# keunwoochoi/torchaudio-contrib

Hardware: AMD Instinct MI355X
Metric: mel frames/sec (higher is better)
Workload: dtype f32; 1 GPU; Melspectrogram+AmplitudeToDb batch=256/GPU x 1ch x 16000Hz x 10s, fft_len=2048 hop=512 128 mel (BASELINE configs[1]); global_batch=256, parallelism=batch-sharded x1, no data-path collective

## Files before the change

include/tac_amd.h:

```cpp
#ifndef TAC_AMD_H
#define TAC_AMD_H

#include <stdint.h>

#ifdef __cplusplus
extern "C" {
#endif

#define TAC_OK 0
#define TAC_E_INVALID (-1)
#define TAC_E_UNSUPPORTED (-2)
#define TAC_E_SHORT_INPUT (-3)
#define TAC_E_LAUNCH (-4)

#define TAC_PAD_CONSTANT 0
#define TAC_PAD_REFLECT 1
#define TAC_PAD_REPLICATE 2
#define TAC_PAD_CIRCULAR 3

const char* tac_strerror(int code);
int tac_last_hip_error(void);
int tac_abi_version(void);

int64_t tac_num_frames(int64_t L, int n_fft, int hop, int center);
int tac_num_bins(int n_fft, int onesided);

typedef struct tac_stft_desc {
    int64_t rows;
    int64_t length;
    int64_t row_stride;
    int32_t n_fft;
    int32_t hop;
    int32_t win_length;
    int32_t center;
    int32_t pad_mode;
    int32_t normalized;
    int32_t onesided;
    int32_t reserved;
} tac_stft_desc;

int tac_stft_f32(const float* wave, const float* window, const tac_stft_desc* d,
                 float* out, void* stream);

int tac_spectrogram_f32(const float* wave, const float* window, const tac_stft_desc* d,
                        float power, int db, float db_ref, float db_amin,
                        float* out, void* stream);

int tac_melspec_f32(const float* wave, const float* window, const tac_stft_desc* d, float power,
                    const float* fb, const int32_t* fb_plan_host, int32_t n_mels,
                    int db, float db_ref, float db_amin, float* out, void* stream);

#define TAC_PACK_PAIRS_2048 (-2048)
int tac_melbank_pack(const float* fb, int32_t n_freqs, int32_t n_mels, int32_t n_fft, float* wpack,
                     int32_t wpack_cap, int32_t* desc, int32_t desc_cap, int32_t* info_host, void* stream);
int tac_melbank_pack_host(const float* fb_host, int32_t n_freqs, int32_t n_mels, int32_t n_fft, float* wpack_host,
                          int32_t wpack_cap, int32_t* desc_host, int32_t desc_cap, int32_t* info_host);
int tac_melbank_plan_pieces_host(const float* fb_host, int32_t n_freqs, int32_t n_mels, int32_t* seg_steps, int32_t* first,
                                 int32_t* band, int32_t* index, float* weights, int32_t weights_cap);
int tac_melspec_sparse_f32(const float* wave, const float* window, const tac_stft_desc* d, float power,
                           const float* wpack, const int32_t* desc, const int32_t* info_host, int32_t n_mels,
                           int db, float db_ref, float db_amin, float* out, void* stream);

#define TAC_SAMPLES_F32 0
#define TAC_SAMPLES_I16 1
#define TAC_SAMPLES_MULAW_U8 2
#define TAC_SAMPLES_MULAW_I64 3
int tac_melspec_sparse_coded_f32(const void* samples, int32_t sample_format, const float* decode_lut,
                                 const float* window, const tac_stft_desc* d, float power, const float* wpack,
                                 const int32_t* desc, const int32_t* info_host, int32_t n_mels, int db,
                                 float db_ref, float db_amin, float* out, void* stream);
int tac_pcm16_to_f32(const int16_t* x, int64_t n, float* out, void* stream);

int tac_melspec_supported(const tac_stft_desc* d, float power, const int32_t* fb_plan_host,
                          int32_t n_mels);

int tac_filterbank_plan(const float* fb, int32_t n_freqs, int32_t n_mels, int32_t* plan,
                        int32_t* plan_host, void* stream);

int tac_apply_filterbank_f32(const float* spec, int64_t rows, int32_t n_freqs, int64_t n_frames,
                             int64_t stride_r, int64_t stride_f, int64_t stride_t,
                             const float* fb, const int32_t* fb_plan, int32_t n_mels,
                             float* out, void* stream);

int tac_apply_filterbank_sparse_f32(const float* spec, int64_t rows, int32_t n_freqs, int64_t n_frames,
                                    int64_t stride_r, int64_t stride_t, const float* wpack,
                                    const int32_t* desc, const int32_t* info_host, int32_t n_mels,
                                    float* out, void* stream);
int tac_apply_filterbank_sparse_db_f32(const float* spec, int64_t rows, int32_t n_freqs, int64_t n_frames,
                                       int64_t stride_r, int64_t stride_t, const float* wpack, const int32_t* desc,
                                       const int32_t* info_host, int32_t n_mels, int db, float db_ref, float db_amin,
                                       float* out, void* stream);

int tac_complex_norm_f32(const float* x, int64_t n, float power, float* out, void* stream);

int tac_magphase_f32(const float* x, int64_t n, float power, float* mag, float* phase, void* stream);

int tac_phase_vocoder_f32(const float* spec, int64_t rows, int32_t n_freqs, int64_t n_frames,
                          int64_t stride_r, int64_t stride_f, int64_t stride_t,
                          const float* phase_advance, const int32_t* idx0, const int32_t* idx1,
                          const float* alpha, int64_t n_out, float* out, void* stream);
int tac_phase_vocoder_f64(const double* spec, int64_t rows, int32_t n_freqs, int64_t n_frames,
                          int64_t stride_r, int64_t stride_f, int64_t stride_t,
                          const double* phase_advance, const int32_t* idx0, const int32_t* idx1,
                          const double* alpha, int64_t n_out, double* out, void* stream);
int tac_phase_vocoder_backward_f32(const float* spec, int64_t rows, int32_t n_freqs, int64_t n_frames, int64_t stride_r,
                                   int64_t stride_f, int64_t stride_t, const int32_t* idx0, const int32_t* idx1, const float* alpha,
                                   int64_t n_out, const float* grad_out, float* grad_spec, void* stream);

int tac_stretch_norm_f32(const float* mag, int64_t rows, int32_t n_freqs, int64_t n_frames, int64_t stride_r, int64_t stride_t,
                         const int32_t* idx0, const float* alpha, int64_t n_out, float power, int db, float db_ref, float db_amin,
                         float* out, int32_t* flags, void* stream);
int tac_stretch_mel_f32(const float* mag, int64_t rows, int32_t n_freqs, int64_t n_frames, int64_t stride_r, int64_t stride_t,
                        const int32_t* idx0, const float* alpha, int64_t n_out, float power, const float* wpack, const int32_t* desc,
                        const int32_t* info_host, int32_t n_mels, int db, float db_ref, float db_amin, float* out, int32_t* flags,
                        void* stream);
int tac_stretch_norm_backward_f32(const float* mag, int64_t rows, int32_t n_freqs, int64_t n_frames, int64_t stride_r,
                                  int64_t stride_t, const int32_t* idx0, const float* alpha, const int32_t* bounds, int64_t n_out,
                                  float power, const float* grad_out, float* grad_mag, void* stream);

int tac_stft_f64(const double* wave, const double* window, const tac_stft_desc* d, double* out, void* stream);
int tac_spectrogram_f64(const double* wave, const double* window, const tac_stft_desc* d, double power, int db,
                        double db_ref, double db_amin, double* out, void* stream);
int tac_apply_filterbank_f64(const double* spec, int64_t rows, int32_t n_freqs, int64_t n_frames, int64_t stride_r,
                             int64_t stride_f, int64_t stride_t, const double* fb, int32_t n_mels, int db,
                             double db_ref, double db_amin, double* out, void* stream);
int tac_magphase_f64(const double* z, int64_t n, double power, double* mag, double* phase, void* stream);
int tac_amplitude_to_db_f64(const double* x, int64_t n, double ref, double amin, double* out, void* stream);
int tac_db_to_amplitude_f64(const double* x, int64_t n, double ref, double* out, void* stream);

int tac_amplitude_to_db_f32(const float* x, int64_t n, float ref, float amin, float* out,
                            void* stream);

int tac_db_to_amplitude_f32(const float* x, int64_t n, float ref, float* out, void* stream);

int tac_mulaw_encode_f32_i64(const float* x, int64_t n, int32_t n_quantize,
                             const int32_t* thresholds, int32_t n_pos, int32_t n_neg,
                             int32_t zero_code, int64_t* out, void* stream);

int tac_mulaw_decode_i64_f32(const int64_t* codes, int64_t n, int32_t n_quantize,
                             const float* lut, float* out, void* stream);

int tac_mulaw_decode_f32_f32(const float* codes, int64_t n, int32_t n_quantize, const float* lut,
                             float* out, void* stream);
int tac_mulaw_encode_f64_i64(const double* x, int64_t n, int32_t n_quantize, int64_t* out, void* stream);
int tac_mulaw_decode_f64(const void* codes, int32_t codes_are_i64, int64_t n, int32_t n_quantize, double* out, void* stream);

int tac_stft_backward_f32(const float* grad_spec, const float* window, const tac_stft_desc* d,
                          float* grad_frames, void* stream);
int tac_stft_norm_backward_f32(const float* spec, const float* grad_norm, float power, const float* window,
                               const tac_stft_desc* d, float* grad_frames, void* stream);
int tac_spectrogram_backward_f32(const float* wave, const float* window, const tac_stft_desc* d,
                                 const float* grad_norm, float power, float* grad_frames, void* stream);
int64_t tac_spectrogram_backward_ola_workspace(const tac_stft_desc* d);
int tac_spectrogram_backward_ola_f32(const float* wave, const float* window, const tac_stft_desc* d,
                                     const float* grad_norm, float power, void* workspace, int64_t workspace_bytes,
                                     float* grad_wave, int64_t grad_row_stride, void* stream);
int tac_melspectrogram_backward_ola_f32(const float* wave, const float* window, const tac_stft_desc* d,
                                        const float* grad_mel, int32_t n_mels, const void* adjoint_table,
                                        int32_t n_freqs, float power, void* workspace, int64_t workspace_bytes,
                                        float* grad_wave, int64_t grad_row_stride, void* stream);
int tac_melspectrogram_backward_f32(const float* wave, const float* window, const tac_stft_desc* d,
                                    const float* grad_mel, int32_t n_mels, const void* adjoint_table, int32_t n_freqs,
                                    float power, float* grad_frames, void* stream);
int tac_filterbank_adjoint_pack(const float* fb, int32_t n_freqs, int32_t n_mels, void* table,
                                int32_t* max_nonzeros_host, void* stream);
int tac_apply_filterbank_adjoint_f32(const float* grad_mel, int64_t rows_times_frames, int32_t n_mels,
                                     const void* table, int32_t n_freqs, float* grad_spec, void* stream);
int tac_overlap_add_f32(const float* grad_frames, const tac_stft_desc* d, float* grad_wave,
                        int64_t grad_row_stride, void* stream);
int tac_complex_norm_backward_f32(const float* z, const float* grad_out, int64_t n, float power,
                                  float* grad_z, void* stream);
int tac_fold_twosided_f32(const float* grad, int64_t n_frames_total, int32_t n_fft, int32_t width, float* out,
                          void* stream);
int64_t tac_window_grad_partials(const tac_stft_desc* d);
int tac_window_grad_f32(const float* grad_frames_unwindowed, const float* wave, const tac_stft_desc* d,
                        float* partial, int64_t n_partials, void* stream);
int tac_sum_slabs_f32(const float* x, int64_t n_slabs, int64_t slab_elems, float* out, void* stream);
int tac_amplitude_to_db_backward_f32(const float* x, const float* grad_out, int64_t n, float amin,
                                     float* grad_x, void* stream);
int tac_magphase_backward_f32(const float* z, const float* grad_mag, const float* grad_phase, int64_t n, float power,
                              float* grad_z, void* stream);
int tac_db_to_amplitude_backward_f32(const float* x, const float* grad_out, int64_t n, float ref, float* grad_x, void* stream);

int tac_hpss_f32(const float* mag, int64_t rows, int32_t n_freqs, int32_t n_frames, int64_t stride_r,
                 int64_t stride_f, int64_t stride_t, int32_t kernel_f, int32_t kernel_t, float power,
                 int hard, float* harm, float* perc, float* mask_harm, float* mask_perc, void* stream);
int tac_hpss_backward_f32(const float* mag, int64_t rows, int32_t n_freqs, int32_t n_frames, int64_t stride_r, int64_t stride_f,
                          int64_t stride_t, int32_t kernel_f, int32_t kernel_t, float power, int hard, const float* grad_harm,
                          const float* grad_perc, const float* grad_mask_harm, const float* grad_mask_perc, float* grad_mag,
                          void* stream);

const char* tac_last_route(void);
int tac_debug_clock_probe(uint64_t* buf, int32_t capacity_pairs);

int tac_set_fft_pipe(int mode);

int64_t tac_istft_workspace(const tac_stft_desc* d, int64_t n_frames);
int tac_istft_envelope_f32(const float* window, const tac_stft_desc* d, int64_t n_frames, float* inv_env, float* env,
                           void* stream);
int tac_istft_f32(const float* spec, int64_t stride_r, int64_t stride_t, int64_t n_frames, const float* window,
                  const float* inv_env, const tac_stft_desc* d, void* workspace, int64_t workspace_bytes, float* out,
                  void* stream);
int tac_istft_grad_input_f32(const float* grad_out, int64_t grad_stride, const float* inv_env, const tac_stft_desc* d,
                             int64_t n_frames, float* padded, void* stream);
int tac_istft_grad_bins_f32(float* spec, int64_t n_frames_total, int n_fft, int normalized, void* stream);

int tac_dct_rows_f32(const float* x, int64_t rows, int32_t n_in, int64_t n_frames,
                     int64_t stride_r, int64_t stride_m, int64_t stride_t,
                     const float* mat, int32_t n_out, float* out, void* stream);

int tac_polyphase_f32(const float* x, int64_t rows, int64_t l_in, int64_t stride_r, const float* bank, const int32_t* table,
                      int32_t phases, int32_t taps, int32_t taps_min, int32_t step, int32_t off_min, int32_t off_max,
                      int64_t l_out, float* out, void* stream);

int32_t tac_lfilter_chunk(void);
int tac_lfilter_supported(const double* b, const double* a, int32_t n_coeffs);
int tac_lfilter_f32(const float* x, int64_t rows, int64_t length, int64_t stride_r, const double* b, const double* a,
                    int32_t n_coeffs, int clamp, int reverse, float* out, void* stream);

int32_t tac_spectral_mac_tile(int32_t n_parts);
int tac_spectral_mac_f32(const float* X, const float* H, const int32_t* hrow, int64_t rows, int64_t n_frames, int32_t n_bins,
                         int32_t n_parts, int32_t h_rows, int conj, float* Y, void* stream);
int32_t tac_fftconvolve_default_n_fft(int64_t m);
int tac_fftconvolve_supported(int64_t l_in, int64_t m, int32_t n_fft);
int64_t tac_fftconvolve_spectra_workspace(int64_t h_rows, int64_t m, int32_t n_fft);
int tac_fftconvolve_spectra_f32(const float* y, int64_t h_rows, int64_t m, int64_t stride_r, int32_t n_fft, int reverse,
                                void* workspace, int64_t workspace_bytes, float* H, void* stream);
int64_t tac_fftconvolve_workspace(int64_t rows, int64_t l_in, int64_t m, int32_t n_fft, int64_t offset, int64_t l_out);
int tac_fftconvolve_f32(const float* x, int64_t rows, int64_t l_in, int64_t stride_r, const float* H, const int32_t* hrow,
                        int32_t h_rows, int64_t m, int32_t n_fft, int conj, int64_t offset, int64_t l_out, void* workspace,
                        int64_t workspace_bytes, float* out, int64_t out_stride, void* stream);
int tac_fftconvolve_direct_f32(const float* x, int64_t rows, int64_t l_in, int64_t stride_r, const float* bank, const int32_t* table,
                               int64_t m, int64_t offset, int64_t l_out, float* out, void* stream);

#define TAC_KALDI_SNIP_EDGES 1
#define TAC_KALDI_REMOVE_DC 2
#define TAC_KALDI_RAW_ENERGY 4
#define TAC_KALDI_USE_ENERGY 8
#define TAC_KALDI_HTK 16
#define TAC_KALDI_LOG 32
#define TAC_KALDI_POWER 64
int64_t tac_kaldi_num_frames(int64_t length, int32_t win_length, int32_t shift, int snip_edges);
int tac_kaldi_fbank_f32(const float* x, int64_t rows, int64_t length, int64_t stride_r, const float* window, const float* weights,
                        const int32_t* table, int32_t n_fft, int32_t win_length, int32_t shift, int32_t n_mels, int32_t w_total,
                        int32_t flags, float preemph, float energy_floor, float* out, void* stream);

int64_t tac_kaldi_mfcc_table_limit(int32_t n_fft, int32_t n_mels, int32_t w_total);
int tac_kaldi_mfcc_f32(const float* x, int64_t rows, int64_t length, int64_t stride_r, const float* window, const float* weights,
                       const int32_t* table, const float* dct, int32_t n_fft, int32_t win_length, int32_t shift, int32_t n_mels,
                       int32_t w_total, int32_t n_ceps, int32_t flags, float preemph, float energy_floor, float* out, void* stream);
int tac_kaldi_spectrogram_f32(const float* x, int64_t rows, int64_t length, int64_t stride_r, const float* window, int32_t n_fft,
                              int32_t win_length, int32_t shift, int32_t flags, float preemph, float energy_floor, float* out,
                              void* stream);

int64_t tac_sliding_cmn_chunk(int64_t rows, int64_t n_frames, int64_t n_feats, int64_t cmn_window, int64_t min_cmn_window);
int tac_sliding_cmn_f32(const float* x, int64_t rows, int64_t n_frames, int64_t n_feats, int64_t stride_r, int64_t stride_t,
                        int64_t stride_f, int64_t cmn_window, int64_t min_cmn_window, int center, int norm_vars, int adjoint,
                        float* out, void* stream);

#define TAC_DELTAS_REPLICATE 0
#define TAC_DELTAS_CONSTANT 1
#define TAC_DELTAS_REFLECT 2
#define TAC_DELTAS_CIRCULAR 3
int tac_deltas_supported(int64_t n_frames, int32_t win_length, int32_t mode, int adjoint);
int tac_deltas_f32(const float* x, int64_t rows, int64_t n_feats, int64_t n_frames, int64_t stride_r, int64_t stride_f,
                   int64_t stride_t, int32_t win_length, int32_t mode, int adjoint, float* out, void* stream);

#ifdef __cplusplus
}
#endif
#endif
```

torchaudio-contrib_amd/_hip.py:

```python
import ctypes
import itertools
import math
import os
import threading
import weakref

import torch

from . import _kaldi
from . import _native
from . import _resample

_lock = threading.Lock()

launches = {}


def _count(name, *filled):
    launches[name] = launches.get(name, 0) + 1
    check_written(name, *filled)


_epoch = 0
_CACHE_ATTRS = ('_tac_pack', '_tac_plan', '_tac_T', '_tac_adj', '_tac_dft', '_tac_dftT', '_tac_finite', '_tac_istft', '_tac_dct', '_tac_coef', '_tac_conv')
# ... 154 lines not shown
    return g


def _rows_of(wave, g):
    return wave.reshape(-1, g.length).contiguous() if g.flatten else wave


def _dft_matrix(window, n_fft, win_length, onesided, normalized):
    cache = getattr(window, '_tac_dft', None)
    key = (_stamp(window), n_fft, win_length, bool(onesided), bool(normalized))
    if cache is not None and cache[0] == key:
        return cache[1]
    dev = window.device
    w = torch.zeros(n_fft, dtype=torch.float64, device=dev)
    off = (n_fft - win_length) // 2
    w[off:off + win_length] = window.detach().double()
    if normalized:
        w = w / math.sqrt(n_fft)
    n_bins = n_fft // 2 + 1 if onesided else n_fft
    n = torch.arange(n_fft, dtype=torch.int64, device=dev)[:, None]
    k = torch.arange(n_bins, dtype=torch.int64, device=dev)[None, :]
    ang = ((n * k) % n_fft).double() * (2.0 * math.pi / n_fft)
    mat = torch.stack([torch.cos(ang) * w[:, None], -torch.sin(ang) * w[:, None]], dim=-1)
    mat = mat.to(torch.float32).reshape(n_fft, 2 * n_bins).contiguous()
    try:
        window._tac_dft = (key, mat)
    except Exception:
        pass
    return mat


def _stft_dft(wave, window, g):
    x = wave.reshape(-1, g.length)
    if g.center:
        pad = g.n_fft // 2
        x = torch.nn.functional.pad(x.unsqueeze(1), (pad, pad), mode=g.pad_mode).squeeze(1)
    x = x.contiguous()
    mat = _dft_matrix(window, g.n_fft, g.win_length, g.onesided, g.normalized)
    out = _empty(g.stft_shape, device=x.device)
    with _native.on_device(x.device):
        rc = _native.lib().tac_apply_filterbank_f32(
            _native.ptr(x), x.shape[0], g.n_fft, g.n_frames, x.stride(0), 1, g.hop,
            _native.ptr(mat), None, 2 * g.n_bins, _native.ptr(out), _native.stream_ptr(x.device))
    _native.check(rc, 'tac_apply_filterbank_f32 (DFT matrix)')
    _count('tac_apply_filterbank_f32', out)
    return out.transpose(-3, -2)


def stft(wave, window, n_fft, hop, win_length, center, pad_mode, normalized, onesided):
    g = geometry(wave, n_fft, hop, win_length, center, pad_mode, normalized, onesided)
    if not (g.fft_kernel or (g.mixed_radix and g.onesided)):
        return _stft_dft(wave, window, g)
    src = _rows_of(wave, g)
    out = _empty(g.stft_shape, device=wave.device)
    with _native.on_device(wave.device):
        rc = _native.lib().tac_stft_f32(_native.ptr(src), _native.ptr(window), g.desc, _native.ptr(out),
                                        _native.stream_ptr(wave.device))
    _native.check(rc, 'tac_stft_f32')
    _count('tac_stft_f32', out)
    return out.transpose(-3, -2)


def spectrogram(wave, window, n_fft, hop, win_length, center, pad_mode, normalized, onesided, power, db, ref, amin):
    g = geometry(wave, n_fft, hop, win_length, center, pad_mode, normalized, onesided)
    if not (g.fft_kernel or (g.mixed_radix and g.onesided and power in (1.0, 2.0))):
        mag = complex_norm(_stft_dft(wave, window, g), power)
        return amplitude_to_db(mag, ref, amin) if db else mag
    src = _rows_of(wave, g)
    out = _empty(g.spec_shape, device=wave.device)
    with _native.on_device(wave.device):
        rc = _native.lib().tac_spectrogram_f32(
            _native.ptr(src), _native.ptr(window), g.desc, float(power), 1 if db else 0, float(ref), float(amin),
            _native.ptr(out), _native.stream_ptr(wave.device))
    _native.check(rc, 'tac_spectrogram_f32')
    _count('tac_spectrogram_f32', out)
    return out.transpose(-2, -1)


istft_layout = {'in_place': 0, 'copied': 0}


def istft_covers(n_fft):
    return bool(fft_kernel_size(n_fft) or mixed_radix_size(n_fft) or smooth_fft_size(n_fft) or n_fft == 8192)


def istft_full_length(n_frames, n_fft, hop, center):
    return hop * (n_frames - 1) + n_fft - (2 * (n_fft // 2) if center else 0)


def _istft_desc(rows, out_len, row_stride, n_fft, hop, win_length, center, normalized):
    return _native.StftDesc(rows=rows, length=out_len, row_stride=row_stride, n_fft=n_fft, hop=hop, win_length=win_length,
                            center=1 if center else 0, pad_mode=0, normalized=1 if normalized else 0, onesided=1, reserved=0)


def istft_envelope(window, n_fft, hop, win_length, center, n_frames, kept):
    cache = getattr(window, '_tac_istft', None)
    stamp = _stamp(window)
    if cache is None or cache[0] != stamp:
        cache = (stamp, {})
        try:
            window._tac_istft = cache
        except Exception:
            pass
    key = (n_fft, hop, win_length, bool(center), n_frames)
    entry = cache[1].get(key)
    if entry is None:
        n_pos = hop * (n_frames - 1) + n_fft
        with torch.inference_mode(False):
            inv_env = torch.empty(n_pos, dtype=torch.float32, device=window.device)
        desc = _istft_desc(1, 1, 1, n_fft, hop, win_length, center, False)
        with _native.on_device(window.device):
            rc = _native.lib().tac_istft_envelope_f32(_native.ptr(window), desc, n_frames, _native.ptr(inv_env),
                                                      None, _native.stream_ptr(window.device))
        _native.check(rc, 'tac_istft_envelope_f32')
        launches['tac_istft_envelope_f32'] = launches.get('tac_istft_envelope_f32', 0) + 1
        if len(cache[1]) > 64:
            cache[1].clear()
        entry = cache[1][key] = (inv_env, set())
    if kept not in entry[1]:
        pad = n_fft // 2 if center else 0
        peak = float(entry[0][pad:pad + kept].max().item())
        lowest = 1.0 / peak if peak > 0.0 else float('inf')
        if not lowest >= 1e-11:
            raise RuntimeError('istft: window overlap add min: %g is below 1e-11 (fft_length=%d, hop_length=%d, center=%s): '
                               'the window does not satisfy the NOLA condition' % (lowest, n_fft, hop, bool(center)))
        entry[1].add(kept)
    return entry[0]


def _istft_rows(spec):
    sp = spec.transpose(-3, -2)
    if sp.is_contiguous() and sp.data_ptr() % 16 == 0:
        istft_layout['in_place'] += 1
    else:
        istft_layout['copied'] += 1
        sp = sp.contiguous()
    return sp.reshape((-1,) + tuple(sp.shape[-3:]))


def istft(spec, window, n_fft, hop, win_length, center, normalized, length, route=None):
    n_frames = int(spec.shape[-2])
    full = istft_full_length(n_frames, n_fft, hop, center)
    if full <= 0:
        raise RuntimeError('istft: %d frame(s) of fft_length %d leave no samples after removing the centre padding'
                           % (n_frames, n_fft))
    out_len = full if length is None else int(length)
    inv_env = istft_envelope(window, n_fft, hop, win_length, center, n_frames, min(full + (n_fft // 2 if center else 0), out_len))
    lead = tuple(int(s) for s in spec.shape[:-3])
    rows = _istft_rows(spec)
    n_rows = int(rows.shape[0])
    out = _empty(lead + (out_len,), device=spec.device)
    desc = _istft_desc(n_rows, out_len, out_len, n_fft, hop, win_length, center, normalized)
    need = int(_native.lib().tac_istft_workspace(desc, n_frames))
    if need < 0:
        _native.check(need, 'tac_istft_workspace')

    def launch(work, nbytes):
        with _native.on_device(spec.device):
            return _native.lib().tac_istft_f32(_native.ptr(rows), rows.stride(0), rows.stride(1), n_frames, _native.ptr(window),
                                               _native.ptr(inv_env), desc, None if work is None else _native.ptr(work), nbytes,
                                               _native.ptr(out), _native.stream_ptr(spec.device))

    rc = _native.TAC_E_UNSUPPORTED
    if need == 0 and route != 'general':
        rc = launch(None, 0)
    if rc == _native.TAC_E_UNSUPPORTED:
        need = n_rows * n_frames * n_fft * 4
        work = torch.empty(need // 4, dtype=torch.float32, device=spec.device)
        rc = launch(work, need)
    _native.check(rc, 'tac_istft_f32')
    _count('tac_istft_f32', out)
    return out


def istft_backward(grad_out, window, n_fft, hop, win_length, center, normalized, n_frames):
    out_len = int(grad_out.shape[-1])
    full = istft_full_length(n_frames, n_fft, hop, center)
    inv_env = istft_envelope(window, n_fft, hop, win_length, center, n_frames, min(full + (n_fft // 2 if center else 0), out_len))
    lead = tuple(int(s) for s in grad_out.shape[:-1])
    go = grad_out.reshape(-1, out_len)
    go = go if go.is_contiguous() else go.contiguous()
    n_rows, n_pos, n_bins = int(go.shape[0]), hop * (n_frames - 1) + n_fft, n_fft // 2 + 1
    padded = _empty((n_rows, n_pos), device=go.device)
    gspec = _empty(lead + (n_frames, n_bins, 2), device=go.device)
    with _native.on_device(go.device):
        stream = _native.stream_ptr(go.device)
        rc = _native.lib().tac_istft_grad_input_f32(
            _native.ptr(go), out_len, _native.ptr(inv_env),
            _istft_desc(n_rows, out_len, out_len, n_fft, hop, win_length, center, normalized), n_frames, _native.ptr(padded), stream)
        _native.check(rc, 'tac_istft_grad_input_f32')
        _count('tac_istft_grad_input_f32', padded)
        fwd = _native.StftDesc(rows=n_rows, length=n_pos, row_stride=n_pos, n_fft=n_fft, hop=hop, win_length=win_length, center=0,
                               pad_mode=0, normalized=0, onesided=1, reserved=0)
        rc = _native.lib().tac_stft_f32(_native.ptr(padded), _native.ptr(window), fwd, _native.ptr(gspec), stream)
        _native.check(rc, 'tac_stft_f32')
        _count('tac_stft_f32', gspec)
        rc = _native.lib().tac_istft_grad_bins_f32(_native.ptr(gspec), n_rows * n_frames, n_fft, 1 if normalized else 0, stream)
        _native.check(rc, 'tac_istft_grad_bins_f32')
        _count('tac_istft_grad_bins_f32', gspec)
    return gspec.transpose(-3, -2)


POISON_OUTPUTS = False

POISON_BITS = {torch.float32: 0x7FC0DEAD, torch.float64: 0x7FF80000DEADBEEF, torch.int64: -0x21524111DEADBEEF,
               torch.int32: -0x21524111}
_BIT_VIEW = {torch.float32: torch.int32, torch.float64: torch.int64, torch.int64: torch.int64, torch.int32: torch.int32}
_poison_hits = {}


def set_poison_outputs(on):
    global POISON_OUTPUTS
    POISON_OUTPUTS = bool(on)
    ext = _native.ext()
    if ext is not None:
        ext.set_poison(POISON_OUTPUTS)


def poison_fill(t):
    if t.numel():
        t.view(_BIT_VIEW[t.dtype]).fill_(POISON_BITS[t.dtype])
    return t


def poison_count(t):
    if not t.numel():
        return torch.zeros((), dtype=torch.int64, device=t.device)
    return (t.view(_BIT_VIEW[t.dtype]) == POISON_BITS[t.dtype]).sum()


def _poisoning(t):
    return POISON_OUTPUTS and not (t.is_cuda and torch.cuda.is_current_stream_capturing())


def _empty(shape, dtype=torch.float32, device=None):
    out = torch.empty(shape, dtype=dtype, device=device)
    return poison_fill(out) if _poisoning(out) else out


def _empty_strided(shape, stride, dtype=torch.float32, device=None):
    out = torch.empty_strided(shape, stride, dtype=dtype, device=device)
    return poison_fill(out) if _poisoning(out) else out


def _empty_like(x):
    out = torch.empty_like(x)
    return poison_fill(out) if _poisoning(out) else out


def check_written(name, *parts):
    if not POISON_OUTPUTS:
        return
    for t in parts:
        if t is None or not t.numel() or not _poisoning(t):
            continue
        key = (name, t.device.index)
        acc = _poison_hits.get(key)
        if acc is None:
            with torch.inference_mode(False):
                acc = _poison_hits[key] = torch.zeros((), dtype=torch.int64, device=t.device)
        acc += poison_count(t)


def poison_report(reset=True):
    bad = {}
    for (name, _), acc in list(_poison_hits.items()):
        n = int(acc.item())
        if n:
            bad[name] = bad.get(name, 0) + n
    if reset:
        _poison_hits.clear()
    return bad

MEL_PATH = os.environ.get('TAC_MEL_PATH', 'auto')


def _melbank_pack(fb, n_fft):
    cache = getattr(fb, '_tac_pack', None)
    if cache is None or cache[0] != _stamp(fb):
        cache = (_stamp(fb), {})
        try:
            fb._tac_pack = cache
        except Exception:
            pass
    if n_fft in cache[1]:
        return cache[1][n_fft]
    n_freqs, n_mels = fb.shape
    wpack = torch.empty(24576, dtype=torch.float32, device=fb.device)
    desc = torch.empty(8192, dtype=torch.int32, device=fb.device)
    info = (ctypes.c_int32 * 8)()
    with _native.on_device(fb.device):
        rc = _native.lib().tac_melbank_pack(_native.ptr(fb), n_freqs, n_mels, n_fft, _native.ptr(wpack), 24576,
                                            _native.ptr(desc), 8192, ctypes.cast(info, ctypes.c_void_p),
                                            _native.stream_ptr(fb.device))
    if rc == _native.TAC_E_UNSUPPORTED:
        result = None
    else:
        _native.check(rc, 'tac_melbank_pack')
        result = (wpack, desc, info)
    cache[1][n_fft] = result
    return result


PAIR_LAYOUT = True
PACK_PAIRS_2048 = -2048


def _fused_pack(fb, n_fft):
    if PAIR_LAYOUT and n_fft == 2048 and tuple(fb.shape) == (1025, 128):
        pack = _melbank_pack(fb, PACK_PAIRS_2048)
        if pack is not None:
            return pack
    return _melbank_pack(fb, n_fft)


def _filterbank_plan(fb):
    hit = getattr(fb, '_tac_plan', None)
    if hit is not None and hit[0] == _stamp(fb) and hit[1].device == fb.device:
        return hit[1], hit[2]
    n_freqs, n_mels = fb.shape
    n_ints = 2 * ((n_mels + 15) // 16)
    plan = torch.empty(n_ints, dtype=torch.int32, device=fb.device)
    host = (ctypes.c_int32 * n_ints)()
    with _native.on_device(fb.device):
        rc = _native.lib().tac_filterbank_plan(_native.ptr(fb), n_freqs, n_mels, _native.ptr(plan),
                                               ctypes.cast(host, ctypes.c_void_p), _native.stream_ptr(fb.device))
    _native.check(rc, 'tac_filterbank_plan')
    try:
        fb._tac_plan = (_stamp(fb), plan, host)
    except Exception:
        pass
    return plan, host


def _fused_mel_route(g, fb, power):
    if not ((g.pow2_kernel or g.mixed_radix) and g.onesided and g.n_fft <= 4096 and fb.dim() == 2 and
            fb.shape[0] == g.n_bins and 0 < fb.shape[1] <= 512 and fb.is_contiguous()):
        return None
    if g.mixed_radix:
        ok = power in (1.0, 2.0) and MEL_PATH != 'mfma' and _melbank_pack(fb, g.n_fft) is not None
        return 'sparse' if ok else None
    if power in (1.0, 2.0) and MEL_PATH != 'mfma' and _melbank_pack(fb, g.n_fft) is not None:
        return 'sparse'
    if MEL_PATH == 'sparse' or g.n_fft > 2048:
        return None
    _, host = _filterbank_plan(fb)
    rc = _native.lib().tac_melspec_supported(g.desc, float(power), ctypes.cast(host, ctypes.c_void_p), fb.shape[1])
    return 'mfma' if rc == _native.TAC_OK else None


class MelPlan(object):
    __slots__ = ('fn', 'win_ptr', 'desc', 'power', 'wpack', 'dsc', 'info', 'wpack_ptr', 'dsc_ptr', 'info_ptr', 'n_mels',
                 'db', 'ref', 'amin', 'shape', 'device', 'dev_index', 'window', 'fb', 'win_stamp', 'fb_stamp', 'layout', 'cplan',
                 'last_rc')

    def run(self, wave):
        c = self.cplan
        if c is not None:
            v = c.launch(wave)
            if v is not None:
                launches['tac_melspec_sparse_f32'] = launches.get('tac_melspec_sparse_f32', 0) + 1
                if POISON_OUTPUTS:
                    check_written('tac_melspec_sparse_f32', v)
            else:
                self.last_rc = c.last_rc
            return v
        return self.launch(wave) if self.matches(wave) else None

    def launch(self, wave):
        out = _empty(self.shape, device=self.device)
        rc = self.fn(wave.data_ptr(), self.win_ptr, self.desc, self.power, self.wpack_ptr, self.dsc_ptr, self.info_ptr,
                     self.n_mels, self.db, self.ref, self.amin, out.data_ptr(),
                     torch._C._cuda_getCurrentRawStream(self.dev_index))
        if rc != _native.TAC_OK:
            self.last_rc = rc
            return None
        launches['tac_melspec_sparse_f32'] = launches.get('tac_melspec_sparse_f32', 0) + 1
        if POISON_OUTPUTS:
            check_written('tac_melspec_sparse_f32', out)
        return out.transpose(-2, -1)

    def matches(self, wave):
        return (wave.shape, wave.stride(), wave.dtype) == self.layout and torch._C._cuda_getDevice() == self.dev_index \
            and _stamp(self.window) == self.win_stamp and _stamp(self.fb) == self.fb_stamp


def mel_plan(wave, window, fb, n_fft, hop, win_length, center, pad_mode, normalized, onesided, power, db, ref, amin):
    if not (type(wave) is torch.Tensor and wave.dtype == torch.float32 and window.dtype == torch.float32
            and window.is_contiguous() and fb.dtype == torch.float32 and fb.dim() == 2 and wave.is_cuda
            and window.device == wave.device and fb.device == wave.device and not window.is_inference()
            and not fb.is_inference()):
        return None
    g = geometry(wave, n_fft, hop, win_length, center, pad_mode, normalized, onesided)
    if g.flatten or g.desc is None or fb.shape[0] != g.n_bins or _fused_mel_route(g, fb, power) != 'sparse':
        return None
    wpack, dsc, info = _fused_pack(fb, g.n_fft)
    p = MelPlan()
    p.fn = _native.lib().tac_melspec_sparse_f32
    p.window, p.fb, p.win_stamp, p.fb_stamp = window, fb, _stamp(window), _stamp(fb)
    p.win_ptr, p.desc, p.power = window.data_ptr(), g.desc, float(power)
    p.wpack, p.dsc, p.info = wpack, dsc, info
    p.wpack_ptr, p.dsc_ptr, p.info_ptr = wpack.data_ptr(), dsc.data_ptr(), ctypes.cast(info, ctypes.c_void_p)
    p.n_mels, p.db, p.ref, p.amin = int(fb.shape[1]), 1 if db else 0, float(ref), float(amin)
    p.shape = g.lead + (g.n_frames, int(fb.shape[1]))
    p.device, p.dev_index = wave.device, wave.device.index
    p.layout = (wave.shape, wave.stride(), wave.dtype)
    p.cplan = None
    p.last_rc = 0
    ext = _native.ext()
    if ext is not None:
        try:
            p.cplan = ext.MelPlan(ctypes.cast(p.fn, ctypes.c_void_p).value, wave, window, fb, wpack, dsc, bytes(g.desc),
                                  [int(v) for v in info], p.power, p.n_mels, bool(db), p.ref, p.amin, [int(n) for n in p.shape],
                                  _epoch)
        except Exception:
            p.cplan = None
    return p


def melspectrogram(wave, window, fb, n_fft, hop, win_length, center, pad_mode, normalized, onesided, power, db, ref,
                   amin):
    g = geometry(wave, n_fft, hop, win_length, center, pad_mode, normalized, onesided)
    if fb.dim() != 2 or fb.shape[0] != g.n_bins:
        raise RuntimeError('apply_filterbank: size mismatch, spectrogram has %d bins, filterbank %s'
                           % (g.n_bins, tuple(fb.shape)))
    rkey = (id(fb), _stamp(fb), power, MEL_PATH)
    hit = g.routes.get(rkey)
    if hit is not None and hit[0]() is fb:
        route = hit[1]
    else:
        if len(g.routes) > 16:
            g.routes.clear()
        route = _fused_mel_route(g, fb, power)
        g.routes[rkey] = (weakref.ref(fb), route)
    if route is None:
        spec = spectrogram(wave, window, n_fft, hop, win_length, center, pad_mode, normalized, onesided, power,
                           False, 1.0, 1e-7)
        return apply_filterbank(spec, fb, db=(ref, amin) if db else None)
    n_mels = fb.shape[1]
    src = _rows_of(wave, g)
    out = _empty(g.lead + (g.n_frames, n_mels), device=wave.device)
    if route == 'sparse':
        wpack, desc, info = _fused_pack(fb, g.n_fft)
        with _native.on_device(wave.device):
            rc = _native.lib().tac_melspec_sparse_f32(
                _native.ptr(src), _native.ptr(window), g.desc, float(power), _native.ptr(wpack), _native.ptr(desc),
                ctypes.cast(info, ctypes.c_void_p), n_mels, 1 if db else 0, float(ref), float(amin),
                _native.ptr(out), _native.stream_ptr(wave.device))
        if rc == _native.TAC_E_UNSUPPORTED:
            spec = spectrogram(wave, window, n_fft, hop, win_length, center, pad_mode, normalized, onesided, power,
                               False, 1.0, 1e-7)
            return apply_filterbank(spec, fb, db=(ref, amin) if db else None)
        _native.check(rc, 'tac_melspec_sparse_f32')
        _count('tac_melspec_sparse_f32', out)
        return out.transpose(-2, -1)
    _, plan_host = _filterbank_plan(fb)
    with _native.on_device(wave.device):
        rc = _native.lib().tac_melspec_f32(
            _native.ptr(src), _native.ptr(window), g.desc, float(power), _native.ptr(fb),
            ctypes.cast(plan_host, ctypes.c_void_p), n_mels, 1 if db else 0, float(ref), float(amin),
            _native.ptr(out), _native.stream_ptr(wave.device))
    _native.check(rc, 'tac_melspec_f32')
    _count('tac_melspec_f32', out)
    return out.transpose(-2, -1)


def apply_filterbank(spec, fb, allow_sparse=True, db=None):
    fb = fb if fb.is_contiguous() else fb.contiguous()
    n_freqs, n_frames = spec.shape[-2], spec.shape[-1]
    lead = tuple(spec.shape[:-2])
    n_mels = fb.shape[1]
    out = _empty(lead + (n_frames, n_mels), device=spec.device)
    if out.numel():
        rows = spec.reshape(-1, n_freqs, n_frames)
        pack = _melbank_pack(fb, 0) if (allow_sparse and rows.stride(1) == 1 and MEL_PATH != 'mfma') else None
        if pack is not None:
            wpack, desc, info = pack
            with _native.on_device(spec.device):
                if db is None:
                    name = 'tac_apply_filterbank_sparse_f32'
                    rc = _native.lib().tac_apply_filterbank_sparse_f32(
                        _native.ptr(rows), rows.shape[0], n_freqs, n_frames, rows.stride(0) if rows.shape[0] > 1 else 0,
                        rows.stride(2), _native.ptr(wpack), _native.ptr(desc), ctypes.cast(info, ctypes.c_void_p), n_mels,
                        _native.ptr(out), _native.stream_ptr(spec.device))
                else:
                    name = 'tac_apply_filterbank_sparse_db_f32'
                    rc = _native.lib().tac_apply_filterbank_sparse_db_f32(
                        _native.ptr(rows), rows.shape[0], n_freqs, n_frames, rows.stride(0) if rows.shape[0] > 1 else 0,
                        rows.stride(2), _native.ptr(wpack), _native.ptr(desc), ctypes.cast(info, ctypes.c_void_p), n_mels,
                        1, float(db[0]), float(db[1]), _native.ptr(out), _native.stream_ptr(spec.device))
            if rc != _native.TAC_E_UNSUPPORTED:
                _native.check(rc, name)
                _count(name, out)
                return out.transpose(-2, -1)
        plan, _ = _filterbank_plan(fb)
        with _native.on_device(spec.device):
            rc = _native.lib().tac_apply_filterbank_f32(
                _native.ptr(rows), rows.shape[0], n_freqs, n_frames, rows.stride(0), rows.stride(1),
                rows.stride(2), _native.ptr(fb), _native.ptr(plan), n_mels, _native.ptr(out),
                _native.stream_ptr(spec.device))
        _native.check(rc, 'tac_apply_filterbank_f32')
        _count('tac_apply_filterbank_f32', out)
    out = out.transpose(-2, -1)
    return out if db is None else amplitude_to_db(out, db[0], db[1])


DCT_MAX_DIM, DCT_MAX_MATRIX = 256, 32768


def dct_covers(n_in, n_out):
    return 1 <= n_in <= DCT_MAX_DIM and 1 <= n_out <= DCT_MAX_DIM and n_in * n_out <= DCT_MAX_MATRIX


def _dct_matrix(mat, transposed):
    if not transposed and mat.dtype == torch.float32 and mat.is_contiguous():
        return mat.detach()
    hit = getattr(mat, '_tac_dct', None)
    if hit is None or hit[0] != _stamp(mat):
        hit = (_stamp(mat), {})
        try:
            mat._tac_dct = hit
        except Exception:
            pass
    m = hit[1].get(transposed)
    if m is None:
        src = mat.detach().t() if transposed else mat.detach()
        m = hit[1][transposed] = src.to(torch.float32).contiguous()
    return m


def dct_rows(x, mat, transposed=False):
    m = _dct_matrix(mat, transposed)
    n_in, n_out = m.shape
    n_frames = x.shape[-1]
    lead = tuple(x.shape[:-2])
    out = _empty(lead + (n_frames, n_out), device=x.device)
    if out.numel():
        rows = x.reshape(-1, n_in, n_frames)
        if any(st <= 0 for st, n in zip(rows.stride(), rows.shape) if n > 1):
            rows = rows.contiguous()
        with _native.on_device(x.device):
            rc = _native.lib().tac_dct_rows_f32(
                _native.ptr(rows), rows.shape[0], n_in, n_frames, rows.stride(0), rows.stride(1), rows.stride(2),
                _native.ptr(m), n_out, _native.ptr(out), _native.stream_ptr(x.device))
        _native.check(rc, 'tac_dct_rows_f32')
        _count('tac_dct_rows_f32', out)
    return out.transpose(-2, -1)


RESAMPLE_MAX_BANK = 20480
RESAMPLE_MAX_PHASES = 2048
RESAMPLE_TILE = 1024
_RS_SPAN_WIDE, _RS_SPAN_MAX = 8192, 14336


def _rs_span_cap(b, tile, off_min, off_max):
    return (3 + ((b.phases - 1 + tile - 1) // b.phases) * b.step + (off_max - off_min) + b.K + 3) & ~3


def resample_tile(b):
    if b.phases > RESAMPLE_MAX_PHASES or b.phases * b.K > RESAMPLE_MAX_BANK:
        return None
    off_min, off_max = min(b.off), max(b.off)
    for tile in (1024, 512, 256):
        if _rs_span_cap(b, tile, off_min, off_max) <= (_RS_SPAN_MAX if tile == 256 else _RS_SPAN_WIDE):
            return tile
    return None


def resample_covers(orig, new, lpw, rolloff, method, beta):
    return resample_tile(_resample.bank(orig, new, lpw, rolloff, method, beta)) is not None and \
        resample_tile(_resample.adjoint_bank(orig, new, lpw, rolloff, method, beta)) is not None


_resample_tables = {}


def _resample_device_bank(key, adjoint, device):
    hit = _resample_tables.get((key, adjoint, device))
    if hit is None:
        b = (_resample.adjoint_bank if adjoint else _resample.bank)(*key)
        taps = b.taps.t().contiguous().to(torch.float32).to(device)
        table = torch.tensor([b.off, b.run], dtype=torch.int32).to(device)
        if len(_resample_tables) > 64:
            _resample_tables.clear()
        hit = _resample_tables[(key, adjoint, device)] = (b, taps, table, min(b.off), max(b.off), min(b.run))
    return hit


def polyphase(x, key, n_out, adjoint=False):
    b, taps, table, off_min, off_max, run_min = _resample_device_bank(key, adjoint, x.device)
    length = x.shape[-1]
    out = _empty(tuple(x.shape[:-1]) + (n_out,), device=x.device)
    if out.numel():
        if length == 0:
            return out.zero_()
        rows = x.reshape(-1, length)
        if (length > 1 and rows.stride(1) != 1) or (rows.shape[0] > 1 and rows.stride(0) <= 0):
            rows = rows.contiguous()
        with _native.on_device(x.device):
            rc = _native.lib().tac_polyphase_f32(
                _native.ptr(rows), rows.shape[0], length, rows.stride(0), _native.ptr(taps), _native.ptr(table), b.phases, b.K,
                run_min, b.step, off_min, off_max, n_out, _native.ptr(out), _native.stream_ptr(x.device))
        _native.check(rc, 'tac_polyphase_f32')
        _count('tac_polyphase_f32', out)
    return out


LFILTER_C = 16
LFILTER_TILE = 1024 * LFILTER_C
LFILTER_MAX_COEFFS = 3

_lfilter_ok = {}
_lfilter_chunk_checked = False

# ... 1187 lines not shown
```

torchaudio-contrib_amd/csrc/lane_placement.hpp:

```cpp
#pragma once
#include <algorithm>
#include <functional>
#include <vector>

namespace tac {

inline std::vector<int> place_band_starts(int nslot, const int* steps, const std::vector<int>& lo, const std::vector<int>& len) {
    std::vector<int> start(lo);
    static const int kGroup[2][16] = {{0, 1, 2, 3, 12, 13, 14, 15, 20, 21, 22, 23, 24, 25, 26, 27},
                                      {4, 5, 6, 7, 8, 9, 10, 11, 16, 17, 18, 19, 28, 29, 30, 31}};
    for (int s = 0; s < nslot; ++s)
        for (int gi = 0; gi < 4; ++gi) {
            int lanes[16];
            for (int i = 0; i < 16; ++i) lanes[i] = kGroup[gi & 1][i] + 32 * (gi >> 1);
            std::vector<int> cand[16];
            for (int i = 0; i < 16; ++i) {
                const int m = s * 64 + lanes[i];
                const int slack = std::max(0, std::min(steps[s] - (len[m] + 3) / 4, lo[m] / 4));
                for (int d = 0; d <= slack; ++d) cand[i].push_back(lo[m] - 4 * d);
            }
            for (int cap = 1; cap <= 16; ++cap) {
                std::vector<int> load[16];
                int choice[16];
                unsigned seen = 0;
                std::function<bool(int)> place = [&](int i) -> bool {
                    for (int c : cand[i]) {
                        const int r = (c / 4) & 15;
                        if (seen & (1u << r)) continue;
                        seen |= 1u << r;
                        if ((int)load[r].size() < cap) { load[r].push_back(i); choice[i] = c; return true; }
                        for (size_t q = 0; q < load[r].size(); ++q) {
                            const int other = load[r][q];
                            if (place(other)) {
                                load[r].erase(std::find(load[r].begin(), load[r].end(), other));
                                load[r].push_back(i);
                                choice[i] = c;
                                return true;
                            }
                        }
                    }
                    return false;
                };
                bool ok = true;
                for (int i = 0; i < 16 && ok; ++i) {
                    seen = 0;
                    ok = place(i);
                }
                if (ok) {
                    for (int i = 0; i < 16; ++i) start[s * 64 + lanes[i]] = choice[i];
                    break;
                }
            }
        }
    return start;
}

inline int row_read_cycles(int nslot, const int* steps, const std::vector<int>& first) {
    static const int kGroup[2][16] = {{0, 1, 2, 3, 12, 13, 14, 15, 20, 21, 22, 23, 24, 25, 26, 27},
                                      {4, 5, 6, 7, 8, 9, 10, 11, 16, 17, 18, 19, 28, 29, 30, 31}};
    int total = 0;
    for (int s = 0; s < nslot; ++s)
        for (int gi = 0; gi < 4; ++gi) {
            std::vector<int> quads[16];
            int worst = 1;
            for (int i = 0; i < 16; ++i) {
                const int q = first[s * 64 + kGroup[gi & 1][i] + 32 * (gi >> 1)] / 4;
                std::vector<int>& v = quads[q & 15];
                if (std::find(v.begin(), v.end(), q) == v.end()) v.push_back(q);
                worst = std::max(worst, (int)v.size());
            }
            total += steps[s] * worst;
        }
    return total;
}

}
```

torchaudio-contrib_amd/csrc/melspec_sparse.hip:

```cpp
#include "mel_common.hpp"
#include "mel_lanes.hpp"
#include "fb_lanes.hpp"

#include <algorithm>
#include <cstdlib>
#include <functional>
#include <atomic>
#include <vector>


#include "sparse_phase.hpp"
#include "melspec_stream.hpp"
#include "melspec_stream3.hpp"
#include "melspec_mfma.hpp"
#include "mel_pieces.hpp"
#include "lane_placement.hpp"

namespace tac {

int launch_n400_mel(const FrameGeom& g, float power, const float* wpack, const int* desc, const int32_t* info_host,
                    int n_mels, int db, float amin, float log10_ref, float* out, hipStream_t stream, int fmt = FMT_F32,
                    const void* samples = nullptr, const float* lut = nullptr);
int pack_n400(const std::vector<float>& h, int n_freqs, int n_mels, float* wpack, int wpack_cap, int32_t* desc,
              int desc_cap, int32_t* info_host, hipStream_t stream, bool to_host = false);
int launch_small_mel_entry(int n_fft, const FrameGeom& g, const Tables& tb, float power, const float* wpack, const int* desc,
                           const int32_t* info_host, int n_mels, int db, float amin, float log10_ref, float* out,
                           hipStream_t stream, int fmt = FMT_F32, const void* samples = nullptr, const float* lut = nullptr);
int pack_small(int n_fft, const std::vector<float>& h, int n_freqs, int n_mels, float* wpack, int wpack_cap, int32_t* desc,
               int desc_cap, int32_t* info_host, hipStream_t stream, bool to_host = false);
int launch_n4096_mel(const FrameGeom& g, float power, const float* wpack, const int32_t* desc, const int32_t* info_host, int n_mels,
                     int db, float amin, float log10_ref, float* out, hipStream_t stream);
int pack_n4096_mel(const std::vector<float>& h, int n_freqs, int n_mels, float* wpack, int wpack_cap, int32_t* desc, int desc_cap,
                   int32_t* info_host, hipStream_t stream, bool to_host = false);

constexpr int SP_TILE = 16;
constexpr int SP_MAX_W = 3072;

struct SparseArgs {
    const float* wpack;
    const int* desc;
    int wtot;
    int dstride;
    int n_mels;
    int db;
    float amin;
    float log10_ref;
    float* out;
    int out_vec4;
};

__host__ __device__ inline int sparse_ostr(int n_mels, int out_vec4) { return out_vec4 ? n_mels + 4 : (n_mels | 1); }


template <int NT>
__device__ __forceinline__ void sparse_phase_c(const float* otile, int ostr, int th, int tile_frames, const SparseArgs& m,
                                               const FrameGeom& g, int row, long long f0) {
    if (m.out_vec4) {
        typedef float f4 __attribute__((ext_vector_type(4)));
        const int q4 = m.n_mels >> 2;
        const int c4_df = NT / q4, c4_db = NT % q4;
        int fo = th / q4, b4 = th % q4;
        for (int idx = th; idx < tile_frames * q4; idx += NT) {
            f4 v = *reinterpret_cast<const f4*>(otile + fo * ostr + 4 * b4);
            if (m.db) {
                v.x = amp_to_db(v.x, m.amin, m.log10_ref);
                v.y = amp_to_db(v.y, m.amin, m.log10_ref);
                v.z = amp_to_db(v.z, m.amin, m.log10_ref);
                v.w = amp_to_db(v.w, m.amin, m.log10_ref);
            }
            const long long frame = f0 + fo;
            if (frame < g.n_frames)
                *reinterpret_cast<f4*>(m.out + (row * g.n_frames + frame) * m.n_mels + 4 * b4) = v;
            b4 += c4_db;
            fo += c4_df;
            if (b4 >= q4) { b4 -= q4; ++fo; }
        }
    } else {
        const int c_df = NT / m.n_mels, c_dband = NT % m.n_mels;
        int fo = th / m.n_mels, band = th % m.n_mels;
        for (int idx = th; idx < tile_frames * m.n_mels; idx += NT) {
            float v = otile[fo * ostr + band];
            if (m.db) v = amp_to_db(v, m.amin, m.log10_ref);
            const long long frame = f0 + fo;
            if (frame < g.n_frames) m.out[(row * g.n_frames + frame) * m.n_mels + band] = v;
            band += c_dband;
            fo += c_df;
            if (band >= m.n_mels) { band -= m.n_mels; ++fo; }
        }
    }
}

template <int NC, int E, bool POW2>
__global__ void __launch_bounds__((MelCfg<NC, E, SP_TILE>::WAVES * 64), (MelCfg<NC, E, SP_TILE>::WAVES / 4))
melspec_sparse_kernel(FrameGeom g, Tables tb, SparseArgs m) {
    using C = MelCfg<NC, E, SP_TILE>;
    using F = typename C::F;
    constexpr int WAVES = C::WAVES, PROW = C::PROW, TILE = SP_TILE;
    extern __shared__ __attribute__((aligned(16))) unsigned char smem_raw[];
    cf* bufs = reinterpret_cast<cf*>(smem_raw);
    float* wlds = reinterpret_cast<float*>(bufs + C::NBUF * F::PADDED);
    const int ostr = sparse_ostr(m.n_mels, m.out_vec4);
    float* otile = wlds + m.wtot;
    int* dlds = reinterpret_cast<int*>(otile + ((TILE * ostr + 3) & ~3));

    const int tid = threadIdx.x;
    const int lane = tid & 63;
    const int w = __builtin_amdgcn_readfirstlane(tid >> 6);
    const int sub = lane / F::LPF;
    const int t = lane % F::LPF;

    for (int i = tid; i < m.wtot; i += WAVES * 64) wlds[i] = m.wpack[i];
    for (int i = tid; i < WAVES * 4 * m.dstride; i += WAVES * 64) dlds[i] = m.desc[i];

    MelFftConsts<F, true, true> fftk;
    fftk.load(tb, g, t);
    __syncthreads();

    const int tiles_per_row = (int)((g.n_frames + TILE - 1) / TILE);
    const int total_tiles = (int)g.rows * tiles_per_row;
    const int chunk = (total_tiles + (int)gridDim.x - 1) / (int)gridDim.x;
    const int begin = (int)blockIdx.x * chunk;
    const int end = begin + chunk < total_tiles ? begin + chunk : total_tiles;

    const int fr = tid & 15;
    const int* dg = dlds + (tid >> 4) * m.dstride;
    const float* prow = reinterpret_cast<const float*>(bufs) + fr * PROW;
    const int c_f0 = tid / m.n_mels, c_band0 = tid % m.n_mels;
    const int c_df = (WAVES * 64) / m.n_mels, c_dband = (WAVES * 64) % m.n_mels;
    const int q4 = m.n_mels >> 2;
    const int c4_f0 = q4 ? tid / q4 : 0, c4_b0 = q4 ? tid % q4 : 0;
    const int c4_df = q4 ? (WAVES * 64) / q4 : 0, c4_db = q4 ? (WAVES * 64) % q4 : 0;

    cf raw[F::E];
    bool pre_ok = false;
    if (begin < end) {
        const int r0 = begin / tiles_per_row;
        const long long fr0 = (long long)(begin - r0 * tiles_per_row) * TILE + (long long)w * C::GPW * F::G + sub;
        pre_ok = prefetch_frame_raw_x<F>(raw, g, r0, fr0, t);
    }
    __builtin_amdgcn_s_waitcnt(0x0F70);

    NoStamp st;
    for (int tile = begin; tile < end; ++tile) {
        const int row = tile / tiles_per_row;
        const long long f0 = (long long)(tile - row * tiles_per_row) * TILE;
        st.mark(0);

        {
            const int nt = tile + 1;
            const int nr = nt / tiles_per_row;
            const long long nf0 = nt < end ? (long long)(nt - nr * tiles_per_row) * TILE : -1;
            mel_phase_a<C, POW2, true, decltype(st), true>(g, bufs, fftk, w, sub, t, row, f0, raw, &pre_ok, &st, nr, nf0);
        }
        __syncthreads();
        st.mark(1);

        sparse_phase_b(dg, prow, wlds, otile + fr * ostr);
        st.mark(7);
        __syncthreads();
        st.mark(11);

        sparse_phase_c<WAVES * 64>(otile, ostr, tid, TILE, m, g, row, f0);
    }
}

constexpr int FBS_WAVES = 8, FBS_TILE = 16, FBS_CHUNKS = 9;

__global__ void __launch_bounds__(FBS_WAVES * 64, 2)
fb_sparse_kernel(const float* __restrict__ spec, long long rows, int n_freqs, long long n_frames, long long stride_r,
                 long long stride_t, int prow_stride, SparseArgs m) {
    extern __shared__ __attribute__((aligned(16))) unsigned char smem_raw[];
    float* ptile = reinterpret_cast<float*>(smem_raw);
    float* wlds = ptile + FBS_TILE * prow_stride;
    const int ostr = sparse_ostr(m.n_mels, m.out_vec4);
    float* otile = wlds + m.wtot;
    int* dlds = reinterpret_cast<int*>(otile + ((FBS_TILE * ostr + 3) & ~3));
    const int tid = threadIdx.x;
    for (int i = tid; i < m.wtot; i += FBS_WAVES * 64) wlds[i] = m.wpack[i];
    for (int i = tid; i < FBS_WAVES * 4 * m.dstride; i += FBS_WAVES * 64) dlds[i] = m.desc[i];

    FrameGeom g{};
    g.n_frames = n_frames;
    const int tiles_per_row = (int)((n_frames + FBS_TILE - 1) / FBS_TILE);
    const int total_tiles = (int)rows * tiles_per_row;
    const int chunk = (total_tiles + (int)gridDim.x - 1) / (int)gridDim.x;
    const int begin = (int)blockIdx.x * chunk;
    const int end = begin + chunk < total_tiles ? begin + chunk : total_tiles;
    const int fr = tid & 15;
    const int* dg = dlds + (tid >> 4) * m.dstride;
    const float* prow = ptile + fr * prow_stride;

    const bool packed = (stride_t == n_freqs);
    typedef float fbs_f4 __attribute__((ext_vector_type(4)));
    fbs_f4 nxt[FBS_CHUNKS];
    auto request = [&](int tile) {
        const int row = tile / tiles_per_row;
        const long long f0 = (long long)(tile - row * tiles_per_row) * FBS_TILE;
        const float* base = spec + row * stride_r;
        const long long row_floats = packed ? n_frames * n_freqs : 0;
#pragma unroll
        for (int j = 0; j < FBS_CHUNKS; ++j) {
            const int c = tid + FBS_WAVES * 64 * j;
            if (packed) {
                const long long e = f0 * n_freqs + 4LL * c;
                if (e + 4 <= row_floats) {
                    nxt[j] = *reinterpret_cast<const fbs_f4*>(base + e);
                } else {
                    fbs_f4 v;
                    const long long lastel = row_floats - 1;
                    v.x = base[e < lastel ? e : lastel];
                    v.y = base[e + 1 < lastel ? e + 1 : lastel];
                    v.z = base[e + 2 < lastel ? e + 2 : lastel];
                    v.w = base[e + 3 < lastel ? e + 3 : lastel];
                    nxt[j] = v;
                }
            } else {
                const int q4r = (n_freqs + 3) >> 2;
                const int fi = c / q4r, b0 = 4 * (c - fi * q4r);
                long long frame = f0 + fi;
                frame = frame < n_frames ? frame : n_frames - 1;
                const float* src = base + frame * stride_t;
                fbs_f4 v;
                v.x = src[b0 < n_freqs ? b0 : n_freqs - 1];
                v.y = src[b0 + 1 < n_freqs ? b0 + 1 : n_freqs - 1];
                v.z = src[b0 + 2 < n_freqs ? b0 + 2 : n_freqs - 1];
                v.w = src[b0 + 3 < n_freqs ? b0 + 3 : n_freqs - 1];
                nxt[j] = v;
            }
        }
    };
    auto deposit = [&](int tile) {
        const int row = tile / tiles_per_row;
        const long long f0 = (long long)(tile - row * tiles_per_row) * FBS_TILE;
        const int live = (int)((n_frames - f0) < FBS_TILE ? (n_frames - f0) : FBS_TILE);
#pragma unroll
        for (int j = 0; j < FBS_CHUNKS; ++j) {
            const int c = tid + FBS_WAVES * 64 * j;
            int fi, bin;
            if (packed) {
                fi = (4 * c) / n_freqs;
                bin = 4 * c - fi * n_freqs;
            } else {
                const int q4r = (n_freqs + 3) >> 2;
                fi = c / q4r;
                bin = 4 * (c - fi * q4r);
            }
            const float vals[4] = {nxt[j].x, nxt[j].y, nxt[j].z, nxt[j].w};
#pragma unroll
            for (int i = 0; i < 4; ++i) {
                if (packed && bin >= n_freqs) { bin -= n_freqs; ++fi; }
                if (fi < FBS_TILE && bin < n_freqs) ptile[fi * prow_stride + bin] = fi < live ? vals[i] : 0.0f;
                ++bin;
            }
        }
    };
    for (int i = tid; i < FBS_TILE * 8; i += FBS_WAVES * 64) {
        const int col = n_freqs + (i & 7);
        if (col < prow_stride) ptile[(i >> 3) * prow_stride + col] = 0.0f;
    }
    if (begin < end) request(begin);
    for (int tile = begin; tile < end; ++tile) {
        const int row = tile / tiles_per_row;
        const long long f0 = (long long)(tile - row * tiles_per_row) * FBS_TILE;
        deposit(tile);
        __syncthreads();
        if (tile + 1 < end) request(tile + 1);
        sparse_phase_b(dg, prow, wlds, otile + fr * ostr);
        __syncthreads();
        sparse_phase_c<FBS_WAVES * 64>(otile, ostr, tid, FBS_TILE, m, g, row, f0);
    }
}

template <int NC, int E>
static int sparse_groups() { return MelCfg<NC, E, SP_TILE>::WAVES * 4; }

static int sparse_groups_for(int n_fft) {
    switch (n_fft) {
        case 32: return sparse_groups<16, 16>();
        case 64: return sparse_groups<32, 16>();
        case 128: return sparse_groups<64, 16>();
        case 256: return sparse_groups<128, 16>();
        case 512: return sparse_groups<256, 16>();
        case 1024: return sparse_groups<512, 16>();
        case 2048: return 64;
        case 400: return LM_MARK + 8;
        case 4096: return LM_MARK + 4096;
        default: return 0;
    }
}

template <int NC, int E>
static int launch_sparse(const FrameGeom& g, const Tables& tb, const SparseArgs& m, float power, hipStream_t stream) {
    using C = MelCfg<NC, E, SP_TILE>;
    const int ostr = sparse_ostr(m.n_mels, m.out_vec4);
    const size_t lds_bytes = (size_t)C::NBUF * C::F::PADDED * sizeof(cf) + (size_t)m.wtot * 4 +
                             (size_t)((SP_TILE * ostr + 3) & ~3) * 4 + (size_t)C::WAVES * 4 * m.dstride * 4;
    if (lds_bytes > 160 * 1024) return TAC_E_UNSUPPORTED;
    const long long tiles = g.rows * ((g.n_frames + SP_TILE - 1) / SP_TILE);
    if (tiles >= 0x7fffffffLL) return TAC_E_UNSUPPORTED;
    int per_cu = (int)(160 * 1024 / lds_bytes);
    if (per_cu > 2) per_cu = 2;
    if (per_cu < 1) per_cu = 1;
    const bool pow2 = (power == 2.0f);
    return launch_kernel(pow2 ? melspec_sparse_kernel<NC, E, true> : melspec_sparse_kernel<NC, E, false>,
                         persistent_blocks(tiles, 1, (long long)device_cu_count() * per_cu), C::WAVES * 64, lds_bytes, stream, g, tb, m);
}

template <int NC, int E, int FMT>
static int launch_stream(FrameGeom g, const Tables& tb, const SparseArgs& sm, const int32_t* info_host, float power,
                         hipStream_t stream, const void* samples, const float* lut) {
    const long long total = g.rows * g.n_frames;
    if (total >= 0x7fffffffLL) return TAC_E_UNSUPPORTED;
    if (g.length < 2 * NC) return TAC_E_UNSUPPORTED;
    if (info_host[2] & ST_PAIR_MARK) {
        int shape = -1;
        for (int i = 0; i < ST_PAIR_SHAPES; ++i)
            if (info_host[4] == ST_PAIR_SHAPE[i][0] && info_host[5] == ST_PAIR_SHAPE[i][1] && info_host[6] == ST_PAIR_SHAPE[i][2]) shape = i;
        const int c1 = info_host[7];
        if (FMT != FMT_F32 || NC != 1024 || shape < 0 || info_host[1] != 3 || sm.n_mels != 128 || info_host[0] != 256 * info_host[3] ||
            (c1 != ST_FAST_STEPS1 && c1 != ST_FAST_STEPS1_SHORT))
            return TAC_E_INVALID;
        if constexpr (FMT == FMT_F32 && NC == 1024) {
            static const bool rotation = getenv("TAC_STREAM2") != nullptr;
            if (fft_pipe_mfma() || rotation) {
                const int32_t classic[8] = {256 * (ST_FAST_STEPS0 + c1), 2, 64, ST_FAST_STEPS0 + c1, ST_FAST_STEPS0, c1, 0, 0};
                SparseArgs cm = sm;
                cm.wpack = sm.wpack + info_host[0];
                cm.desc = sm.desc + 192;
                cm.wtot = classic[0];
                cm.dstride = classic[1];
                return launch_stream<NC, E, FMT>(g, tb, cm, classic, power, stream, samples, lut);
            }
            const size_t ldsp = stream3_lds_bytes<NC, E>(sm.wtot, S3_WAVES, false) + S3_TW2L_BYTES;
            StreamArgs m{sm.wpack, sm.desc, 3, {info_host[4], info_host[5], info_host[6], 0}, sm.wtot,
                         sm.n_mels, sm.db, sm.amin, sm.log10_ref, sm.out, total, samples, lut, 0, nullptr, 0};
            const bool pow2 = (power == 2.0f);
            void (*kp)(FrameGeom, Tables, StreamArgs);
#define TAC_S3_PAIR(I) (pow2 ? melspec_stream3_kernel<NC, E, true, FMT, ST_PAIR_SHAPE[I][1] + ST_PAIR_SHAPE[I][2], S3_WAVES, ST_PAIR_SHAPE[I][0], ST_PAIR_SHAPE[I][2]> \
                             : melspec_stream3_kernel<NC, E, false, FMT, ST_PAIR_SHAPE[I][1] + ST_PAIR_SHAPE[I][2], S3_WAVES, ST_PAIR_SHAPE[I][0], ST_PAIR_SHAPE[I][2]>)
            kp = shape == 0 ? TAC_S3_PAIR(0) : (shape == 1 ? TAC_S3_PAIR(1) : TAC_S3_PAIR(2));
#undef TAC_S3_PAIR
            static_assert(ST_PAIR_SHAPES == 3, "one instantiation per shape");
            const long long bp = persistent_blocks(total, S3_WAVES, device_cu_count());
            m.chunk = (total + bp - 1) / bp;
            m.probe = (g_clock_probe && g_clock_probe_pairs >= bp) ? g_clock_probe : nullptr;
            set_last_route("melspec_stream3_kernel<%d, %d, %s, %d, %d, %d, %d, %d>", NC, E, pow2 ? "true" : "false", FMT,
                           info_host[5] + info_host[6], S3_WAVES, info_host[4], info_host[6]);
            return launch_kernel(kp, bp, S3_WAVES * 64, ldsp, stream, g, tb, m);
        }
    }
    const size_t lds_bytes = stream_lds_bytes<NC, E>(sm.wtot);
    if (info_host[1] < 1 || info_host[1] > ST_MAX_SLOTS) return TAC_E_UNSUPPORTED;
    if (FMT != FMT_F32) g.vec2_ok = coded_pairs_aligned(g, samples, FMT);
    StreamArgs m{sm.wpack, sm.desc, info_host[1], {info_host[4], info_host[5], info_host[6], info_host[7]}, sm.wtot,
                 sm.n_mels, sm.db, sm.amin, sm.log10_ref, sm.out, total, samples, lut, 0, nullptr, (info_host[2] & ST_REV_MARK) ? 1 : 0};
    const bool pow2 = (power == 2.0f);
    const bool fullm = FMT == FMT_F32 && (sm.n_mels % 64) == 0;
    const bool fast2 = fullm && info_host[1] == 2 && info_host[4] == ST_FAST_STEPS0 &&
                       (info_host[5] == ST_FAST_STEPS1 || info_host[5] == ST_FAST_STEPS1_SHORT);
    const bool fshort = info_host[5] == ST_FAST_STEPS1_SHORT;
    static const bool two_waves = getenv("TAC_STREAM2") != nullptr;
    constexpr bool coded = FMT != FMT_F32;
    constexpr int waves3 = S3_WAVES;
    if constexpr (FMT == FMT_F32 && NC == 1024) {
        const bool use_mfma = fft_pipe_mfma();
        constexpr int WM = 12;
        const size_t ldsm = mfma_lds_bytes<NC, E>(sm.wtot, WM);
        if (use_mfma && !two_waves && ldsm <= 160 * 1024) {
            void (*km)(FrameGeom, Tables, StreamArgs);
            if (fast2 && fshort) km = pow2 ? melspec_mfma_kernel<true, ST_FAST_STEPS1_SHORT, WM> : melspec_mfma_kernel<false, ST_FAST_STEPS1_SHORT, WM>;
            else if (fast2) km = pow2 ? melspec_mfma_kernel<true, ST_FAST_STEPS1, WM> : melspec_mfma_kernel<false, ST_FAST_STEPS1, WM>;
            else km = pow2 ? melspec_mfma_kernel<true, 0, WM> : melspec_mfma_kernel<false, 0, WM>;
            const long long bm = persistent_blocks(total, WM, device_cu_count());
            m.chunk = (total + bm - 1) / bm;
            m.probe = (g_clock_probe && g_clock_probe_pairs >= bm) ? g_clock_probe : nullptr;
            set_last_route("melspec_mfma_kernel<%s, %d, %d>", pow2 ? "true" : "false", fast2 ? (fshort ? ST_FAST_STEPS1_SHORT : ST_FAST_STEPS1) : 0, WM);
            return launch_kernel(km, bm, WM * 64, ldsm, stream, g, tb, m);
        }
    }
    const size_t lds3 = stream3_lds_bytes<NC, E>(sm.wtot, waves3, coded) + ((FMT == FMT_F32 && fast2) ? S3_TW2L_BYTES : 0);
    if (!two_waves && lds3 <= 160 * 1024) {
        void (*k3)(FrameGeom, Tables, StreamArgs);
        if constexpr (FMT == FMT_F32) {
            {
                constexpr int W = S3_WAVES;
                if (fast2 && fshort) k3 = pow2 ? melspec_stream3_kernel<NC, E, true, FMT, ST_FAST_STEPS1_SHORT, W> : melspec_stream3_kernel<NC, E, false, FMT, ST_FAST_STEPS1_SHORT, W>;
                else if (fast2) k3 = pow2 ? melspec_stream3_kernel<NC, E, true, FMT, ST_FAST_STEPS1, W> : melspec_stream3_kernel<NC, E, false, FMT, ST_FAST_STEPS1, W>;
                else k3 = pow2 ? melspec_stream3_kernel<NC, E, true, FMT, 0, W> : melspec_stream3_kernel<NC, E, false, FMT, 0, W>;
            }
        } else {
            k3 = pow2 ? melspec_stream3_kernel<NC, E, true, FMT, 0, S3_WAVES> : melspec_stream3_kernel<NC, E, false, FMT, 0, S3_WAVES>;
        }
        const long long b3 = persistent_blocks(total, waves3, device_cu_count());
        m.chunk = (total + b3 - 1) / b3;
        m.probe = (g_clock_probe && g_clock_probe_pairs >= b3) ? g_clock_probe : nullptr;
        {
            const int fast1 = (FMT == FMT_F32 && fast2) ? (fshort ? ST_FAST_STEPS1_SHORT : ST_FAST_STEPS1) : 0;
            set_last_route("melspec_stream3_kernel<%d, %d, %s, %d, %d, %d>", NC, E, pow2 ? "true" : "false", FMT, fast1, waves3);
        }
        return launch_kernel(k3, b3, waves3 * 64, lds3, stream, g, tb, m);
    }
    void (*kern)(FrameGeom, Tables, StreamArgs);
    if constexpr (FMT == FMT_F32) {
        if (fast2 && fshort)
            kern = pow2 ? melspec_stream_kernel<NC, E, true, true, FMT, ST_FAST_STEPS1_SHORT> : melspec_stream_kernel<NC, E, false, true, FMT, ST_FAST_STEPS1_SHORT>;
        else if (fast2)
            kern = pow2 ? melspec_stream_kernel<NC, E, true, true, FMT, ST_FAST_STEPS1> : melspec_stream_kernel<NC, E, false, true, FMT, ST_FAST_STEPS1>;
        else
            kern = pow2 ? (fullm ? melspec_stream_kernel<NC, E, true, true, FMT, 0> : melspec_stream_kernel<NC, E, true, false, FMT, 0>)
                        : (fullm ? melspec_stream_kernel<NC, E, false, true, FMT, 0> : melspec_stream_kernel<NC, E, false, false, FMT, 0>);
    } else {
        kern = pow2 ? melspec_stream_kernel<NC, E, true, false, FMT, 0> : melspec_stream_kernel<NC, E, false, false, FMT, 0>;
    }
    if (lds_bytes > 160 * 1024) return TAC_E_UNSUPPORTED;
    return launch_kernel(kern, persistent_blocks(total, 2 * ST_WAVES, device_cu_count()), ST_WAVES * 64, lds_bytes, stream, g, tb, m);
}


template <int S, int CHUNKS, int FBL_WAVES, int FBL_FLY>
__global__ void __launch_bounds__(FBL_WAVES * 64, FBL_WAVES / 4)
fb_lanes_kernel(const float* __restrict__ spec, long long rows, int n_freqs, long long n_frames, long long stride_r,
                long long stride_t, LaneMel mel) {
    typedef float f4 __attribute__((ext_vector_type(4)));
    extern __shared__ __attribute__((aligned(16))) unsigned char smem_raw[];
    const int lane = threadIdx.x & 63;
    const int w = __builtin_amdgcn_readfirstlane(threadIdx.x >> 6);
    const int pitch = fbl_pitch(n_freqs);
    float* const srow = reinterpret_cast<float*>(smem_raw) + (size_t)w * (pitch + LM_MAX_MELS + 4);
    float* const mbuf = srow + pitch;
    unsigned* const next_frame = reinterpret_cast<unsigned*>(reinterpret_cast<float*>(smem_raw) +
                                                             (size_t)FBL_WAVES * (pitch + LM_MAX_MELS + 4));
    int* const mlo = reinterpret_cast<int*>(next_frame + 4);
    float* const mwl = reinterpret_cast<float*>(mlo + lm_desc_ints(64));
    lane_mel_load_tables<S, 64, FBL_FLY>(mlo, mwl, mel, threadIdx.x, FBL_WAVES * 64);

    const long long total = rows * n_frames;
    const long long chunk = (total + gridDim.x - 1) / gridDim.x;
    const long long begin = (long long)blockIdx.x * chunk;
    const long long endl = begin + chunk < total ? begin + chunk : total;
    const int nloc = endl > begin ? (int)(endl - begin) : 0;
    if (threadIdx.x == 0) *next_frame = FBL_WAVES;
    __syncthreads();
    auto grab = [&]() -> int {
        unsigned v = 0;
        if (lane == 0) v = __hip_atomic_fetch_add(next_frame, 1u, __ATOMIC_RELAXED, __HIP_MEMORY_SCOPE_WORKGROUP);
        return (int)__builtin_amdgcn_readfirstlane(v);
    };
    const int nch = (n_freqs + 3) >> 2, lastc = (n_freqs >> 2) - 1;
    f4 nxt[CHUNKS];
    float tail[3];
    auto request = [&](int i) {
        const long long gf = begin + i;
        const long long r = gf / n_frames;
        const float* src = spec + r * stride_r + (gf - r * n_frames) * stride_t;
#pragma unroll
        for (int u = 0; u < CHUNKS; ++u) {
            const int c = lane + 64 * u;
            nxt[u] = *reinterpret_cast<const f4*>(src + 4 * (c < lastc ? c : lastc));
        }
#pragma unroll
        for (int u = 0; u < 3; ++u) tail[u] = src[n_freqs - 1 - u];
    };
    auto deposit = [&]() {
#pragma unroll
        for (int u = 0; u < CHUNKS; ++u) {
            const int c = lane + 64 * u;
            if (c <= lastc) *reinterpret_cast<f4*>(srow + 4 * c) = nxt[u];
        }
        if (lane < 3 && n_freqs - 1 - lane > 4 * lastc + 3) srow[n_freqs - 1 - lane] = tail[lane == 0 ? 0 : (lane == 1 ? 1 : 2)];
    };
    int i = w;
    if (i < nloc) request(i);
    while (i < nloc) {
        const int nx = grab();
        wave_lds_fence();
        deposit();
        wave_lds_fence();
        if (nx < nloc) request(nx);
        const long long g0 = (begin + i) * (long long)mel.n_mels;
        const int am = (int)(g0 & 3);
        lane_mel_contract<S, 64, FBL_FLY>(srow, n_freqs, mlo, mwl, lane, mel, mbuf + am);
        wave_lds_fence();
        lane_mel_store<1>(mbuf + am, am, mel.n_mels, mel.out + g0, lane);
        i = nx;
    }
}

template <int S, int CHUNKS>
static int launch_fb_lanes(const float* spec, long long rows, int n_freqs, long long n_frames, long long stride_r,
                           long long stride_t, const LaneMel& mel, hipStream_t stream) {
    constexpr int FBL_WAVES = CHUNKS == FBL_CHUNKS_WIDE ? 8 : 16, FBL_FLY = CHUNKS == FBL_CHUNKS_WIDE ? 16 : 8;
    const size_t bytes = fbl_base_lds(n_freqs) + lm_lds_bytes(64, mel.wtot);
    if (bytes > 160 * 1024) return TAC_E_UNSUPPORTED;
    const long long total = rows * n_frames;
    if (total >= 0x7fffffffLL) return TAC_E_UNSUPPORTED;
    return launch_kernel(fb_lanes_kernel<S, CHUNKS, FBL_WAVES, FBL_FLY>, persistent_blocks(total, FBL_WAVES, device_cu_count()),
                         FBL_WAVES * 64, bytes, stream, spec, rows, n_freqs, n_frames, stride_r, stride_t, mel);
}

static int pack_lanes(const std::vector<float>& h, int n_freqs, int n_mels, float* wpack, int wpack_cap, int32_t* desc,
                      int desc_cap, int32_t* info_host, hipStream_t stream, bool to_host = false) {
    const int nslot = (n_mels + 63) / 64;
    if (nslot > ST_MAX_SLOTS || nslot * 64 > desc_cap) return TAC_E_UNSUPPORTED;
    const int limit = StreamCfg<1024, 16>::PROW;
    std::vector<int> blo(n_mels, 0), blen(n_mels, 0);
    for (int m = 0; m < n_mels; ++m) {
        int l0 = n_freqs, h0 = 0;
        for (int f = 0; f < n_freqs; ++f)
            if (h[(size_t)f * n_mels + m] != 0.0f) { l0 = f < l0 ? f : l0; h0 = f + 1; }
        if (h0 > l0) {
            blo[m] = l0 & ~3;
            blen[m] = h0 - blo[m];
        }
    }
    const bool rev = (n_mels % 64) != 0 && blen[n_mels - 1] > blen[0];
    auto band_of = [&](int c) { return rev ? n_mels - 1 - c : c; };
    std::vector<int> lo(nslot * 64, 0), len(nslot * 64, 0);
    int steps[ST_MAX_SLOTS] = {0, 0, 0, 0};
    for (int c = 0; c < n_mels; ++c) {
        lo[c] = blo[band_of(c)];
        len[c] = blen[band_of(c)];
        steps[c / 64] = std::max(steps[c / 64], (len[c] + 3) / 4);
    }
    const bool fast_shape = nslot == 2 && (n_mels % 64) == 0 && steps[0] <= ST_FAST_STEPS0 && steps[1] <= ST_FAST_STEPS1;
    if (fast_shape) {
        steps[0] = ST_FAST_STEPS0;
        steps[1] = steps[1] <= ST_FAST_STEPS1_SHORT ? ST_FAST_STEPS1_SHORT : ST_FAST_STEPS1;
    }
    int total_steps = 0;
    for (int s = 0; s < nslot; ++s) {
        if (!fast_shape) steps[s] = std::max(4, (steps[s] + 3) & ~3);
        if (4 * steps[s] > limit) return TAC_E_UNSUPPORTED;
        total_steps += steps[s];
    }
    const long long wtot = 256LL * total_steps;
    if (wtot > wpack_cap || stream3_lds_bytes<1024, 16>((int)wtot, S3_WAVES, true) > 160 * 1024) return TAC_E_UNSUPPORTED;
    std::vector<float> wp((size_t)wtot, 0.0f);
    const std::vector<int> start = place_band_starts(nslot, steps, lo, len);
    int base = 0;
    for (int s = 0; s < nslot; ++s) {
        for (int l = 0; l < 64; ++l) {
            const int c = s * 64 + l, m = c < n_mels ? band_of(c) : 0;
            int first = start[c];
            if (first + 4 * steps[s] > limit) first = (limit - 4 * steps[s]) & ~3;
            for (int j = 0; j < steps[s]; ++j)
                for (int u = 0; u < 4; ++u) {
                    const int bin = first + 4 * j + u;
                    const bool live = c < n_mels && bin >= lo[c] && bin < lo[c] + len[c] && bin < n_freqs;
                    wp[((size_t)(base + j) * 64 + l) * 4 + u] = live ? h[(size_t)bin * n_mels + m] : 0.0f;
                }
            lo[c] = first;
        }
        base += steps[s];
    }
    if (to_host) {
        std::copy(wp.begin(), wp.end(), wpack);
        std::copy(lo.begin(), lo.end(), desc);
    } else {
        TAC_HIP(hipMemcpyAsync(wpack, wp.data(), wp.size() * sizeof(float), hipMemcpyHostToDevice, stream));
        TAC_HIP(hipMemcpyAsync(desc, lo.data(), lo.size() * sizeof(int32_t), hipMemcpyHostToDevice, stream));
        TAC_HIP(hipStreamSynchronize(stream));
    }
    info_host[0] = (int32_t)wtot;
    info_host[1] = nslot;
    info_host[2] = 64 + (rev ? ST_REV_MARK : 0);
    info_host[3] = total_steps;
    for (int s = 0; s < ST_MAX_SLOTS; ++s) info_host[4 + s] = steps[s];
    return TAC_OK;
}

static int pack_pairs(const std::vector<float>& h, int n_freqs, int n_mels, float* wpack, int wpack_cap, int32_t* desc,
                      int desc_cap, int32_t* info_host, hipStream_t stream, bool to_host = false) {
    if (n_mels != 128 || n_freqs != 1025 || desc_cap < 192 + 128) return TAC_E_UNSUPPORTED;
    const int limit = StreamCfg<1024, 16>::PROW;
    std::vector<int> blo(n_mels, 0), bq(n_mels, 0), bend(n_mels, 0);
    for (int m = 0; m < n_mels; ++m) {
        int l0 = n_freqs, h0 = 0;
        for (int f = 0; f < n_freqs; ++f)
            if (h[(size_t)f * n_mels + m] != 0.0f) { l0 = f < l0 ? f : l0; h0 = f + 1; }
        if (h0 > l0) {
            blo[m] = l0 & ~3;
            bend[m] = h0;
            bq[m] = (h0 - blo[m] + 3) / 4;
        }
    }
    int need_a = 0, need_b = 0, need_w = 0;
    for (int m = 0; m < 64; ++m) need_a = std::max(need_a, bq[m]);
    for (int m = 64; m < 96; ++m) need_b = std::max(need_b, bq[m]);
    for (int m = 96; m < 128; ++m) need_w = std::max(need_w, bq[m]);
    int steps[3] = {0, 0, 0}, best_cycles = 0;
    std::vector<int> best_first, best_lo, best_hi, best_band;
    for (int i = 0; i < ST_PAIR_SHAPES; ++i) {
        const int* shp = ST_PAIR_SHAPE[i];
        if (need_a > shp[0] || need_b > shp[1] || need_w > shp[1] + 2 * shp[2]) continue;
        if (!best_first.empty() && shp[0] + shp[1] + shp[2] > steps[0] + steps[1] + steps[2]) continue;
        const int keep[3] = {steps[0], steps[1], steps[2]};
        steps[0] = shp[0]; steps[1] = shp[1]; steps[2] = shp[2];
        const int B = steps[1], C = steps[2];
        std::vector<int> band(192, 0), lo(192, 0), len(192, 0), first(192, 0);
        std::vector<int> live_lo(192, 0), live_hi(192, 0);
        auto must = [&](int c, int m, int q0, int q1) {
            band[c] = m;
            lo[c] = blo[m] + 4 * q0;
            len[c] = q1 > q0 ? std::min(bend[m], blo[m] + 4 * q1) - lo[c] : 0;
            if (len[c] < 0) len[c] = 0;
        };
        auto place = [&](int c0, int c1) {
            const std::vector<int> st = place_band_starts(3, steps, lo, len);
            for (int c = c0; c < c1; ++c) {
                first[c] = st[c];
                const int n = steps[c / 64];
                if (first[c] + 4 * n > limit) first[c] = (limit - 4 * n) & ~3;
            }
        };
        auto end_quad = [&](int c) { return (first[c] + 4 * steps[c / 64] - blo[band[c]]) / 4; };
        for (int l = 0; l < 64; ++l) {
            must(l, l, 0, bq[l]);
            if (l < 32) must(64 + l, 64 + l, 0, bq[64 + l]);
            else must(64 + l, 64 + l, 0, std::max(1, bq[64 + l] - 2 * C));
            band[128 + l] = l >= 32 ? 64 + l : 96 + l;
        }
        place(0, 128);
        for (int l = 32; l < 64; ++l) {
            const int e1 = std::min(end_quad(64 + l), bq[64 + l]);
            must(128 + l, 64 + l, e1, std::max(e1, bq[64 + l] - C));
        }
        place(160, 192);
        for (int l = 0; l < 32; ++l) {
            const int m = 96 + l, e2 = std::min(std::max(end_quad(64 + 32 + l), end_quad(128 + 32 + l)), bq[m]);
            must(128 + l, m, e2, bq[m]);
        }
        place(128, 160);
        for (int l = 0; l < 64; ++l) {
            live_lo[l] = blo[l];
            live_hi[l] = bend[l];
            live_lo[64 + l] = blo[64 + l];
            live_hi[64 + l] = l < 32 ? bend[64 + l] : std::min(bend[64 + l], first[64 + l] + 4 * B);
            if (l >= 32) {
                const int up = 128 + l, down = 128 + l - 32;
                live_lo[up] = live_hi[64 + l];
                live_hi[up] = std::max(live_lo[up], std::min(bend[64 + l], first[up] + 4 * C));
                live_lo[down] = live_hi[up];
                live_hi[down] = std::max(live_lo[down], bend[64 + l]);
            }
        }
        const int cycles = row_read_cycles(3, steps, first);
        if (best_first.empty() || cycles < best_cycles) {
            best_cycles = cycles; best_first = first; best_lo = live_lo; best_hi = live_hi; best_band = band;
        } else {
            steps[0] = keep[0]; steps[1] = keep[1]; steps[2] = keep[2];
        }
    }
    if (best_first.empty()) return TAC_E_UNSUPPORTED;
    const int A = steps[0], B = steps[1], C = steps[2], total_steps = A + B + C;
    const int wtot = 256 * total_steps;
    std::vector<int> first = best_first, live_lo = best_lo, live_hi = best_hi, band = best_band, lo;
    std::vector<float> wp((size_t)wtot, 0.0f);
    int base = 0;
    for (int s = 0; s < 3; ++s) {
        for (int l = 0; l < 64; ++l) {
            const int c = s * 64 + l;
            if (live_hi[c] > first[c] + 4 * steps[s] || (live_hi[c] > live_lo[c] && live_lo[c] < first[c])) return TAC_E_UNSUPPORTED;
            for (int j = 0; j < steps[s]; ++j)
                for (int u = 0; u < 4; ++u) {
                    const int bin = first[c] + 4 * j + u;
                    const bool live = bin >= live_lo[c] && bin < live_hi[c];
                    wp[((size_t)(base + j) * 64 + l) * 4 + u] = live ? h[(size_t)bin * n_mels + band[c]] : 0.0f;
                }
        }
        base += steps[s];
    }
    lo = first;
    int32_t classic[8] = {0, 0, 0, 0, 0, 0, 0, 0};
    if (wtot >= wpack_cap) return TAC_E_UNSUPPORTED;
    const int rc = pack_lanes(h, n_freqs, n_mels, wpack + wtot, wpack_cap - wtot, desc + 192, desc_cap - 192, classic, stream, to_host);
    if (rc != TAC_OK) return rc;
    if (classic[1] != 2 || classic[2] != 64 || classic[4] != ST_FAST_STEPS0 ||
        (classic[5] != ST_FAST_STEPS1 && classic[5] != ST_FAST_STEPS1_SHORT))
        return TAC_E_UNSUPPORTED;
    if (to_host) {
        std::copy(wp.begin(), wp.end(), wpack);
        std::copy(lo.begin(), lo.end(), desc);
    } else {
        TAC_HIP(hipMemcpyAsync(wpack, wp.data(), wp.size() * sizeof(float), hipMemcpyHostToDevice, stream));
        TAC_HIP(hipMemcpyAsync(desc, lo.data(), lo.size() * sizeof(int32_t), hipMemcpyHostToDevice, stream));
        TAC_HIP(hipStreamSynchronize(stream));
    }
    info_host[0] = wtot;
    info_host[1] = 3;
    info_host[2] = 64 + ST_PAIR_MARK;
    info_host[3] = total_steps;
    info_host[4] = A;
    info_host[5] = B;
    info_host[6] = C;
    info_host[7] = classic[5];
    return TAC_OK;
}

}

extern "C" {

int tac_melbank_plan_pieces_host(const float* fb_host, int32_t n_freqs, int32_t n_mels, int32_t* seg_steps, int32_t* first,
                                 int32_t* band, int32_t* index, float* weights, int32_t weights_cap) {
    using namespace tac;
    if (!fb_host || !seg_steps || !first || !band || !index || !weights || n_freqs <= 0 || n_mels <= 0) return TAC_E_INVALID;
    PiecePlan p;
    if (!plan_pieces(fb_host, n_freqs, n_mels, StreamCfg<1024, 16>::PROW, &p)) return TAC_E_UNSUPPORTED;
    if ((long long)p.w.size() > weights_cap) return TAC_E_INVALID;
    for (int s = 0; s < MP_SEGS; ++s) seg_steps[s] = p.L[s];
    for (int e = 0; e < MP_SEGS * 64; ++e) {
        first[e] = p.first[e];
        band[e] = p.band[e];
        index[e] = p.index[e];
    }
    std::copy(p.w.begin(), p.w.end(), weights);
    return TAC_OK;
}

int tac_melbank_pack_host(const float* fb_host, int32_t n_freqs, int32_t n_mels, int32_t n_fft, float* wpack_host, int32_t wpack_cap,
                          int32_t* desc_host, int32_t desc_cap, int32_t* info_host) {
    using namespace tac;
    if (!fb_host || !wpack_host || !desc_host || !info_host || n_freqs <= 0 || n_mels <= 0) return TAC_E_INVALID;
    const bool lanes = n_fft == 256 || n_fft == 400 || n_fft == 512 || n_fft == 1024;
    if (n_fft == TAC_PACK_PAIRS_2048) {
        if (n_freqs != 1025) return TAC_E_UNSUPPORTED;
        const std::vector<float> hp(fb_host, fb_host + (size_t)n_freqs * n_mels);
        return pack_pairs(hp, n_freqs, n_mels, wpack_host, wpack_cap, desc_host, desc_cap, info_host, nullptr, true);
    }
    if ((n_fft != 2048 && n_fft != 4096 && !lanes) || n_freqs != n_fft / 2 + 1) return TAC_E_UNSUPPORTED;
    const std::vector<float> h(fb_host, fb_host + (size_t)n_freqs * n_mels);
    if (n_fft == 400) return pack_n400(h, n_freqs, n_mels, wpack_host, wpack_cap, desc_host, desc_cap, info_host, nullptr, true);
    if (lanes) return pack_small(n_fft, h, n_freqs, n_mels, wpack_host, wpack_cap, desc_host, desc_cap, info_host, nullptr, true);
    return n_fft == 2048 ? pack_lanes(h, n_freqs, n_mels, wpack_host, wpack_cap, desc_host, desc_cap, info_host, nullptr, true)
                         : pack_n4096_mel(h, n_freqs, n_mels, wpack_host, wpack_cap, desc_host, desc_cap, info_host, nullptr, true);
}

int tac_melbank_pack(const float* fb, int32_t n_freqs, int32_t n_mels, int32_t n_fft, float* wpack,
                     int32_t wpack_cap, int32_t* desc, int32_t desc_cap, int32_t* info_host, void* stream) {
    using namespace tac;
    if (!fb || !wpack || !desc || !info_host || n_freqs <= 0 || n_mels <= 0) return TAC_E_INVALID;
    if (n_fft == TAC_PACK_PAIRS_2048) {
        if (n_freqs != 1025) return TAC_E_UNSUPPORTED;
        std::vector<float> hp((size_t)n_freqs * n_mels);
        TAC_HIP(hipMemcpyAsync(hp.data(), fb, hp.size() * sizeof(float), hipMemcpyDeviceToHost, (hipStream_t)stream));
        TAC_HIP(hipStreamSynchronize((hipStream_t)stream));
        return pack_pairs(hp, n_freqs, n_mels, wpack, wpack_cap, desc, desc_cap, info_host, (hipStream_t)stream);
    }
    if (n_fft < 0) return TAC_E_UNSUPPORTED;
    const int groups = n_fft == 0 ? FBS_WAVES * 4 : sparse_groups_for(n_fft);
    if (groups == 0 || (n_fft != 0 && n_freqs != n_fft / 2 + 1)) return TAC_E_UNSUPPORTED;
    std::vector<float> h((size_t)n_freqs * n_mels);
    TAC_HIP(hipMemcpyAsync(h.data(), fb, h.size() * sizeof(float), hipMemcpyDeviceToHost, (hipStream_t)stream));
    TAC_HIP(hipStreamSynchronize((hipStream_t)stream));
    if (n_fft == 2048)
        return pack_lanes(h, n_freqs, n_mels, wpack, wpack_cap, desc, desc_cap, info_host, (hipStream_t)stream);
    if (n_fft == 4096)
        return pack_n4096_mel(h, n_freqs, n_mels, wpack, wpack_cap, desc, desc_cap, info_host, (hipStream_t)stream);
    if (n_fft == 0 && n_freqs >= 8 && (n_freqs + 3) / 4 <= FBL_CHUNKS_WIDE * 64) {
        const int rc = pack_lane_mel(h, n_freqs, n_mels, 64, fbl_pitch(n_freqs), 2, fbl_fly(n_freqs), LM_MAX_STEPS_WAVE, fbl_base_lds(n_freqs),
                                     wpack, wpack_cap, desc, desc_cap, info_host, (hipStream_t)stream);
        if (rc != TAC_E_UNSUPPORTED) return rc;
    }
    if (n_fft == 400) return pack_n400(h, n_freqs, n_mels, wpack, wpack_cap, desc, desc_cap, info_host, (hipStream_t)stream);
    if (n_fft == 256 || n_fft == 512 || n_fft == 1024) {
        const int rc = pack_small(n_fft, h, n_freqs, n_mels, wpack, wpack_cap, desc, desc_cap, info_host, (hipStream_t)stream);
        if (rc != TAC_E_UNSUPPORTED) return rc;
    }
    struct Band { int m, lo, len; };
    std::vector<Band> bands(n_mels);
    long long total = 0;
    for (int m = 0; m < n_mels; ++m) {
        int lo = n_freqs, hi = 0;
        for (int f = 0; f < n_freqs; ++f)
            if (h[(size_t)f * n_mels + m] != 0.0f) { lo = f < lo ? f : lo; hi = f + 1; }
        lo &= ~1;
        bands[m] = {m, hi > lo ? lo : 0, hi > lo ? hi - lo : 0};
        total += (bands[m].len + 7) & ~7;
    }
    if (total > SP_MAX_W || total > wpack_cap) return TAC_E_UNSUPPORTED;
    std::stable_sort(bands.begin(), bands.end(), [](const Band& a, const Band& b) { return a.len > b.len; });
    std::vector<std::vector<Band>> per(groups);
    std::vector<int> load(groups, 0);
    for (const Band& b : bands) {
        int best = 0;
        for (int gI = 1; gI < groups; ++gI)
            if (load[gI] < load[best] || (load[gI] == load[best] && per[gI].size() < per[best].size())) best = gI;
        per[best].push_back(b);
        load[best] += ((b.len + 7) & ~7) + 4;
    }
    size_t maxnb = 0;
    for (auto& v : per) maxnb = std::max(maxnb, v.size());
    const int dstride = 4 + 4 * (int)maxnb;
    if ((long long)groups * dstride > desc_cap) return TAC_E_UNSUPPORTED;
    std::vector<float> wp((size_t)total, 0.0f);
    std::vector<int32_t> dd((size_t)groups * dstride, 0);
    int woff = 0, maxload = 0;
    for (int gI = 0; gI < groups; ++gI) {
        dd[(size_t)gI * dstride] = (int)per[gI].size();
        int gl = 0;
        for (size_t bI = 0; bI < per[gI].size(); ++bI) {
            const Band& b = per[gI][bI];
            const int n8 = (b.len + 7) / 8;
            int32_t* e = &dd[(size_t)gI * dstride + 4 + 4 * bI];
            e[0] = b.m; e[1] = b.lo; e[2] = n8; e[3] = woff;
            for (int j = 0; j < b.len; ++j) wp[woff + j] = h[(size_t)(b.lo + j) * n_mels + b.m];
            woff += 8 * n8;
            gl += 8 * n8;
        }
        maxload = std::max(maxload, gl);
    }
    TAC_HIP(hipMemcpyAsync(wpack, wp.data(), wp.size() * sizeof(float), hipMemcpyHostToDevice, (hipStream_t)stream));
    TAC_HIP(hipMemcpyAsync(desc, dd.data(), dd.size() * sizeof(int32_t), hipMemcpyHostToDevice, (hipStream_t)stream));
    TAC_HIP(hipStreamSynchronize((hipStream_t)stream));
    info_host[0] = (int32_t)total;
    info_host[1] = dstride;
    info_host[2] = groups;
    info_host[3] = maxload;
    return TAC_OK;
}

int tac_melspec_sparse_f32(const float* wave, const float* window, const tac_stft_desc* d, float power,
                           const float* wpack, const int32_t* desc, const int32_t* info_host, int32_t n_mels,
                           int db, float db_ref, float db_amin, float* out, void* stream) {
    using namespace tac;
    if (!wpack || !desc || !info_host || !out || !d || n_mels <= 0) return TAC_E_INVALID;
    if (!d->onesided || d->n_fft > 4096) return TAC_E_UNSUPPORTED;
    if (power != 2.0f && power != 1.0f) return TAC_E_UNSUPPORTED;
    if (d->n_fft == 4096) {
        FrameGeom g4;
        int64_t T4 = 0;
        const int rc4 = make_geometry(wave, window, d, &g4, &T4);
        if (rc4 != TAC_OK) return rc4;
        return launch_n4096_mel(g4, power, wpack, desc, info_host, n_mels, db ? 1 : 0, db_amin, db ? log10f(db_ref) : 0.0f, out,
                                (hipStream_t)stream);
    }
    const bool lanes_pack = info_host[2] >= LM_MARK;
    if (!lanes_pack && (info_host[2] & ~(d->n_fft == 2048 ? (ST_REV_MARK | ST_PAIR_MARK) : 0)) != sparse_groups_for(d->n_fft)) return TAC_E_INVALID;
    FrameGeom g;
    int64_t T = 0;
    int rc = make_geometry(wave, window, d, &g, &T);
    if (rc != TAC_OK) return rc;
    if (lanes_pack && (d->n_fft == 256 || d->n_fft == 512 || d->n_fft == 1024)) {
        Tables tbs;
        rc = get_tables(d->n_fft, &tbs);
        if (rc != TAC_OK) return rc;
        return launch_small_mel_entry(d->n_fft, g, tbs, power, wpack, desc, info_host, n_mels, db ? 1 : 0, db_amin,
                                      db ? log10f(db_ref) : 0.0f, out, (hipStream_t)stream);
    }
    if (lanes_pack && d->n_fft != 400) return TAC_E_INVALID;
    if (d->n_fft == 400)
        return launch_n400_mel(g, power, wpack, desc, info_host, n_mels, db ? 1 : 0, db_amin, db ? log10f(db_ref) : 0.0f, out,
                               (hipStream_t)stream);
    Tables tb;
    rc = get_tables(d->n_fft, &tb);
    if (rc != TAC_OK) return rc;
    const int out_vec4 = ((n_mels & 3) == 0) && ((reinterpret_cast<uintptr_t>(out) & 15u) == 0);
    SparseArgs m{wpack, desc, info_host[0], info_host[1], n_mels, db ? 1 : 0, db_amin, db ? log10f(db_ref) : 0.0f, out, out_vec4};
    hipStream_t s = (hipStream_t)stream;
    switch (d->n_fft) {
        case 32: return launch_sparse<16, 16>(g, tb, m, power, s);
        case 64: return launch_sparse<32, 16>(g, tb, m, power, s);
        case 128: return launch_sparse<64, 16>(g, tb, m, power, s);
        case 256: return launch_sparse<128, 16>(g, tb, m, power, s);
        case 512: return launch_sparse<256, 16>(g, tb, m, power, s);
        case 1024: return launch_sparse<512, 16>(g, tb, m, power, s);
        case 2048: return launch_stream<1024, 16, FMT_F32>(g, tb, m, info_host, power, s, wave, nullptr);
        default: return TAC_E_UNSUPPORTED;
    }
}

int tac_melspec_sparse_coded_f32(const void* samples, int32_t sample_format, const float* decode_lut, const float* window,
                                 const tac_stft_desc* d, float power, const float* wpack, const int32_t* desc,
                                 const int32_t* info_host, int32_t n_mels, int db, float db_ref, float db_amin, float* out,
                                 void* stream) {
    using namespace tac;
    if (!samples || !wpack || !desc || !info_host || !out || !d || n_mels <= 0) return TAC_E_INVALID;
    if (sample_format < TAC_SAMPLES_F32 || sample_format > TAC_SAMPLES_MULAW_I64) return TAC_E_INVALID;
    if (sample_format >= TAC_SAMPLES_MULAW_U8 && !decode_lut) return TAC_E_INVALID;
    const bool small = d->n_fft == 256 || d->n_fft == 512 || d->n_fft == 1024 || d->n_fft == 400;
    if (!d->onesided || (d->n_fft != 2048 && !small)) return TAC_E_UNSUPPORTED;
    if (power != 2.0f && power != 1.0f) return TAC_E_UNSUPPORTED;
    if (small ? info_host[2] < LM_MARK : (info_host[2] & ~ST_REV_MARK) != sparse_groups_for(d->n_fft)) return small ? TAC_E_UNSUPPORTED : TAC_E_INVALID;
    FrameGeom g;
    int64_t T = 0;
    int rc = make_geometry(static_cast<const float*>(samples), window, d, &g, &T);
    if (rc != TAC_OK) return rc;
    Tables tb;
    rc = get_tables(d->n_fft, &tb);
    if (rc != TAC_OK) return rc;
    if (small) {
        if (sample_format == TAC_SAMPLES_F32) return TAC_E_UNSUPPORTED;
        if (d->n_fft == 400)
            return launch_n400_mel(g, power, wpack, desc, info_host, n_mels, db ? 1 : 0, db_amin, db ? log10f(db_ref) : 0.0f, out,
                                   (hipStream_t)stream, sample_format, samples, decode_lut);
        return launch_small_mel_entry(d->n_fft, g, tb, power, wpack, desc, info_host, n_mels, db ? 1 : 0, db_amin,
                                      db ? log10f(db_ref) : 0.0f, out, (hipStream_t)stream, sample_format, samples, decode_lut);
    }
    SparseArgs m{wpack, desc, info_host[0], info_host[1], n_mels, db ? 1 : 0, db_amin, db ? log10f(db_ref) : 0.0f, out, 0};
    hipStream_t s = (hipStream_t)stream;
    switch (sample_format) {
        case TAC_SAMPLES_F32: return launch_stream<1024, 16, FMT_F32>(g, tb, m, info_host, power, s, samples, nullptr);
        case TAC_SAMPLES_I16: return launch_stream<1024, 16, FMT_I16>(g, tb, m, info_host, power, s, samples, nullptr);
        case TAC_SAMPLES_MULAW_U8: return launch_stream<1024, 16, FMT_MULAW_U8>(g, tb, m, info_host, power, s, samples, decode_lut);
        default: return launch_stream<1024, 16, FMT_MULAW_I64>(g, tb, m, info_host, power, s, samples, decode_lut);
    }
}

int tac_apply_filterbank_sparse_f32(const float* spec, int64_t rows, int32_t n_freqs, int64_t n_frames,
                                    int64_t stride_r, int64_t stride_t, const float* wpack, const int32_t* desc,
                                    const int32_t* info_host, int32_t n_mels, float* out, void* stream) {
    return tac_apply_filterbank_sparse_db_f32(spec, rows, n_freqs, n_frames, stride_r, stride_t, wpack, desc, info_host, n_mels, 0,
                                              1.0f, 1e-7f, out, stream);
}

int tac_apply_filterbank_sparse_db_f32(const float* spec, int64_t rows, int32_t n_freqs, int64_t n_frames,
                                       int64_t stride_r, int64_t stride_t, const float* wpack, const int32_t* desc,
                                       const int32_t* info_host, int32_t n_mels, int db, float db_ref, float db_amin,
                                       float* out, void* stream) {
    using namespace tac;
    if (rows == 0 || n_frames == 0) return TAC_OK;
    if (!spec || !wpack || !desc || !info_host || !out) return TAC_E_INVALID;
    if (rows < 0 || n_freqs <= 0 || n_frames < 0 || n_mels <= 0) return TAC_E_INVALID;
    if (db && !(db_ref > 0.0f)) return TAC_E_INVALID;
    const float log10_ref = db ? log10f(db_ref) : 0.0f;
    if (info_host[2] == LM_MARK + 64) {
        if (!lane_mel_info_ok(info_host, 64, fbl_fly(n_freqs), LM_MAX_STEPS_WAVE)) return TAC_E_INVALID;
        const int chunks = (n_freqs + 3) / 4;
        if (n_mels < LM_MIN_MELS || n_mels > LM_MAX_MELS || chunks > FBL_CHUNKS_WIDE * 64) return TAC_E_UNSUPPORTED;
        const LaneMel lm{wpack, desc, info_host[1], info_host[0], n_mels, db ? 1 : 0, db_amin, log10_ref, out, info_host[5] ? 1 : 0};
        const long long sr = rows > 1 ? stride_r : 0;
        const bool wide = chunks > FBL_CHUNKS * 64;
        switch (info_host[4]) {
#define TAC_FBL_CASE(SS)                                                                                                    \
    case SS:                                                                                                               \
        return wide ? launch_fb_lanes<SS, FBL_CHUNKS_WIDE>(spec, rows, n_freqs, n_frames, sr, stride_t, lm, (hipStream_t)stream) \
                    : launch_fb_lanes<SS, FBL_CHUNKS>(spec, rows, n_freqs, n_frames, sr, stride_t, lm, (hipStream_t)stream);
            TAC_FBL_CASE(2) TAC_FBL_CASE(4) TAC_FBL_CASE(6) TAC_FBL_CASE(8) TAC_FBL_CASE(10) TAC_FBL_CASE(12) TAC_FBL_CASE(14)
            TAC_FBL_CASE(16) TAC_FBL_CASE(18) TAC_FBL_CASE(20) TAC_FBL_CASE(22) TAC_FBL_CASE(24) TAC_FBL_CASE(26) TAC_FBL_CASE(28)
            TAC_FBL_CASE(30) TAC_FBL_CASE(32) TAC_FBL_CASE(34) TAC_FBL_CASE(36)
#undef TAC_FBL_CASE
            default: return TAC_E_INVALID;
        }
    }
    if (info_host[2] != FBS_WAVES * 4) return TAC_E_INVALID;
    if ((long long)FBS_TILE * ((n_freqs + 3) / 4) > (long long)FBS_CHUNKS * FBS_WAVES * 64) return TAC_E_UNSUPPORTED;
    int prow = n_freqs + 7;
    prow += (34 - (prow & 31)) & 31;
    const int out_vec4 = ((n_mels & 3) == 0) && ((reinterpret_cast<uintptr_t>(out) & 15u) == 0);
    SparseArgs m{wpack, desc, info_host[0], info_host[1], n_mels, db ? 1 : 0, db_amin, log10_ref, out, out_vec4};
    const int ostr = sparse_ostr(n_mels, out_vec4);
    const size_t lds_bytes = (size_t)FBS_TILE * prow * 4 + (size_t)m.wtot * 4 + (size_t)((FBS_TILE * ostr + 3) & ~3) * 4 +
                             (size_t)FBS_WAVES * 4 * m.dstride * 4;
    if (lds_bytes > 160 * 1024) return TAC_E_UNSUPPORTED;
    const long long tiles = rows * ((n_frames + FBS_TILE - 1) / FBS_TILE);
    if (tiles >= 0x7fffffffLL) return TAC_E_UNSUPPORTED;
    int per_cu = (int)(160 * 1024 / lds_bytes);
    if (per_cu > 2) per_cu = 2;
    return launch_kernel(fb_sparse_kernel, persistent_blocks(tiles, 1, (long long)device_cu_count() * per_cu), FBS_WAVES * 64, lds_bytes,
                         (hipStream_t)stream, spec, (long long)rows, (int)n_freqs, (long long)n_frames, (long long)stride_r,
                         (long long)stride_t, prow, m);
}

}
```

torchaudio-contrib_amd/csrc/melspec_stream.hpp:

```cpp
#pragma once
#include "mel_common.hpp"


namespace tac {

#ifndef TAC_ST_WAVES
#define TAC_ST_WAVES 8
#endif
constexpr int ST_WAVES = TAC_ST_WAVES;
constexpr int ST_MAX_SLOTS = 4;
constexpr int ST_TW_STRIDE = 36;
constexpr int ST_TW_BYTES = 16 * ST_TW_STRIDE * 4;
constexpr int ST_FAST_STEPS0 = 4, ST_FAST_STEPS1 = 16;
constexpr int ST_FAST_STEPS1_SHORT = 14;
constexpr int ST_RIDE1 = 6;
constexpr int ST_BATCH = 4;
constexpr int ST_RIDE = ST_FAST_STEPS0 + ST_RIDE1;

struct StreamArgs {
    const float* wl;
    const int* lo;
    int nslot;
    int steps[ST_MAX_SLOTS];
    int wtot;
    int n_mels;
    int db;
    float amin;
    float log10_ref;
    float* out;
    long long total;
    const void* samples;
    const float* lut;
    long long chunk;
    unsigned long long* probe;
    int rev;
};
constexpr int ST_REV_MARK = 256;
constexpr int ST_PAIR_MARK = 512;
constexpr int ST_PAIR_SHAPES = 3;
constexpr int ST_PAIR_SHAPE[ST_PAIR_SHAPES][3] = {{4, 6, 4}, {4, 7, 3}, {3, 7, 5}};


template <int NC, int E>
struct StreamCfg {
    using F = WaveFft<NC, E>;
    static constexpr int NBINS = NC + 1;
    static constexpr int PROW0 = NBINS + 7;
    static constexpr int PROW = (PROW0 + 3) & ~3;
    static_assert(F::G == 1, "one frame per wave-pass");
};

template <int NC, int E>
__host__ __device__ inline size_t stream_lds_bytes(int wtot) {
    using C = StreamCfg<NC, E>;
    size_t b = (size_t)ST_WAVES * ((C::F::PADDED * sizeof(cf) + 15) & ~(size_t)15);
    b += (size_t)ST_WAVES * 2 * C::PROW * 4;
    b += ((size_t)wtot * 4 + 15) & ~(size_t)15;
    return b + 1024 + ST_TW_BYTES + 16;
}

template <int NC, int E, bool POW2, bool FULLM, int FMT, int FAST2>
__global__ void __launch_bounds__(ST_WAVES * 64, 2)
melspec_stream_kernel(FrameGeom g, Tables tb, StreamArgs m) {
    using C = StreamCfg<NC, E>;
    using F = typename C::F;
    constexpr int PROW = C::PROW, NBINS = C::NBINS, SLOTS = 2 * ST_WAVES;
    constexpr int XA_BYTES = (F::PADDED * sizeof(cf) + 15) & ~15;
    extern __shared__ __attribute__((aligned(16))) unsigned char smem_raw[];
    const int tid = threadIdx.x;
    const int lane = tid & 63;
    const int w = __builtin_amdgcn_readfirstlane(tid >> 6);
    cf* xa = reinterpret_cast<cf*>(smem_raw + (size_t)w * XA_BYTES);
    float* const rows_all = reinterpret_cast<float*>(smem_raw + (size_t)ST_WAVES * XA_BYTES);
    float* rowA = rows_all + (size_t)(2 * w) * PROW;
    float* rowB = rowA + PROW;
    float* wlds = rows_all + (size_t)ST_WAVES * 2 * PROW;

    float* lutlds = wlds + ((m.wtot + 3) & ~3);
    for (int i = tid; i < m.wtot; i += ST_WAVES * 64) wlds[i] = m.wl[i];
    if (FMT >= FMT_MULAW_U8 && tid < 256) lutlds[tid] = m.lut[tid];
    float* twlds = lutlds + 256;
    if (FAST2 && tid < 16 * 16) {
        const int js = tid >> 4, q = tid & 15;
        const cf wv = q ? tb.w_nc[js * q * (NC / 256)] : mkc(1.0f, 0.0f);
        twlds[js * ST_TW_STRIDE + 2 * (q ? q - 1 : 15)] = wv.x;
        twlds[js * ST_TW_STRIDE + 2 * (q ? q - 1 : 15) + 1] = wv.y;
    }
    unsigned* const next_frame = reinterpret_cast<unsigned*>(twlds + ST_TW_BYTES / 4);
    if (tid == 0) *next_frame = SLOTS;
    for (int i = tid; i < ST_WAVES * 2 * (PROW - NBINS); i += ST_WAVES * 64) {
        const int r = i / (PROW - NBINS), c2 = i - r * (PROW - NBINS);
        rows_all[(size_t)r * PROW + NBINS + c2] = 0.0f;
    }

    const long long chunk = (m.total + gridDim.x - 1) / gridDim.x;
    const long long begin = (long long)blockIdx.x * chunk;
    const long long endl = begin + chunk < m.total ? begin + chunk : m.total;
    const int nloc = endl > begin ? (int)(endl - begin) : 0;
    const unsigned T = (unsigned)g.n_frames;

    const int t = lane;
    cf tw[FAST2 ? 3 : F::NTW];
    if constexpr (FAST2) {
        cf all[F::NTW];
        F::load_twiddles(all, tb.w_nc, t);
#pragma unroll
        for (int q = 0; q < 3; ++q) tw[q] = all[twiddles_before(NC, E, 2) + q];
    } else {
        F::load_twiddles(tw, tb.w_nc, t);
    }
    const cf w0 = tb.w_n[t];
    constexpr bool FULLPTW = FAST2 != 0;
    cf ptw[FULLPTW ? F::NPAIR : 1];
    if constexpr (FULLPTW) {
#pragma unroll
        for (int p = 0; p < F::NPAIR; ++p) ptw[p] = tb.w_n[t + p * F::LPF];
    }
    cf win[E];
    load_window_regs<F>(win, g, t);
    const float half = 0.5f * g.scale;
    const float win_scale = FMT == FMT_I16 ? half * (1.0f / 32768.0f) : half;
#pragma unroll
    for (int e = 0; e < E; ++e) win[e] = cscale(win[e], win_scale);
    int lo_s[ST_MAX_SLOTS];
#pragma unroll
    for (int s = 0; s < ST_MAX_SLOTS; ++s) lo_s[s] = s < m.nslot ? m.lo[s * 64 + lane] : 0;
    __syncthreads();

#define ST_MARK(k) do { } while (0)
    cf vA[E], vB[E];
    cf zmA[F::NPAIR], zmB[F::NPAIR], zmidA = mkc(0.f, 0.f), zmidB = mkc(0.f, 0.f);

    auto grab_ask = [&]() -> unsigned {
        unsigned v = 0;
        if (lane == 0) v = __hip_atomic_fetch_add(next_frame, 1u, __ATOMIC_RELAXED, __HIP_MEMORY_SCOPE_WORKGROUP);
        return v;
    };
    auto grab = [&]() -> int { return (int)__builtin_amdgcn_readfirstlane(grab_ask()); };
    auto request = [&](cf (&raw)[E], int i, int& mode, int& row, long long& fr) {
        i = i < nloc ? i : nloc - 1;
        const unsigned gf = (unsigned)(begin + i);
        const unsigned r = gf / T;
        row = (int)r;
        fr = (long long)(gf - r * T);
        const long long start = fr * (long long)g.hop - g.center_pad;
        const bool ok = g.vec2_ok && start >= 0 && start + F::N <= g.length;
        mode = ok ? 1 : 2;
        long long cs = start < 0 ? 0 : start;
        cs = cs + F::N <= g.length ? cs : g.length - F::N;
        const long long off = (long long)row * g.row_stride + cs;
        {
            if constexpr (FMT == FMT_F32) {
                const cf* src = reinterpret_cast<const cf*>(static_cast<const float*>(m.samples) + off);
#pragma unroll
                for (int q = 0; q < E; ++q) raw[q] = src[t + q * F::LPF];
            } else if constexpr (FMT == FMT_I16) {
                const unsigned* src = reinterpret_cast<const unsigned*>(static_cast<const short*>(m.samples) + off);
#pragma unroll
                for (int q = 0; q < E; ++q) raw[q].x = __uint_as_float(src[t + q * F::LPF]);
            } else if constexpr (FMT == FMT_MULAW_U8) {
                const unsigned short* src =
                    reinterpret_cast<const unsigned short*>(static_cast<const unsigned char*>(m.samples) + off);
#pragma unroll
                for (int q = 0; q < E; ++q) raw[q].x = __uint_as_float((unsigned)src[t + q * F::LPF]);
            } else {
                const int* src = reinterpret_cast<const int*>(static_cast<const long long*>(m.samples) + off);
#pragma unroll
                for (int q = 0; q < E; ++q) {
                    raw[q].x = __int_as_float(src[4 * (t + q * F::LPF)]);
                    raw[q].y = __int_as_float(src[4 * (t + q * F::LPF) + 2]);
                }
            }
        }
    };
    auto decode = [&](cf (&v)[E]) {
        if constexpr (FMT == FMT_I16) {
#pragma unroll
            for (int q = 0; q < E; ++q) {
                const int bits = __float_as_int(v[q].x);
                v[q] = mkc((float)(short)(bits & 0xffff), (float)(bits >> 16));
            }
        } else if constexpr (FMT == FMT_MULAW_U8) {
#pragma unroll
            for (int q = 0; q < E; ++q) {
                const unsigned bits = __float_as_uint(v[q].x);
                v[q] = mkc(lutlds[bits & 0xffu], lutlds[(bits >> 8) & 0xffu]);
            }
        } else if constexpr (FMT == FMT_MULAW_I64) {
#pragma unroll
            for (int q = 0; q < E; ++q) v[q] = mkc(lutlds[__float_as_uint(v[q].x) & 0xffu], lutlds[__float_as_uint(v[q].y) & 0xffu]);
        }
    };
    struct Fetch {
        const void* base;
        const float* lut;
        __device__ __forceinline__ float operator()(long long row_offset, int j) const {
            if constexpr (FMT == FMT_F32) return static_cast<const float*>(base)[row_offset + j];
            else if constexpr (FMT == FMT_I16) return (float)static_cast<const short*>(base)[row_offset + j];
            else if constexpr (FMT == FMT_MULAW_U8) return lut[static_cast<const unsigned char*>(base)[row_offset + j]];
            else return lut[(unsigned)static_cast<const long long*>(base)[row_offset + j] & 0xffu];
        }
    };
    auto s0 = [&](cf (&v)[E], int mode, int row, long long fr) {
        if (mode == 1) {
            decode(v);
        } else {
            int tz;
            asm volatile("v_mov_b32 %0, %1" : "=v"(tz) : "v"(t));
            load_frame<F, true, true>(v, g, win, xa, row, fr, tz, Fetch{m.samples, lutlds});
#pragma unroll
            for (int e = 0; e < E; ++e) v[e] = cscale(v[e], win_scale);
        }
    };
    typedef float f4 __attribute__((ext_vector_type(4)));
    auto s0b = [&](cf (&v)[E], int mode, auto&& before_writes) {
        if (mode == 1) Dft<16>::run_windowed(v, win);
        else F::template pass_butterflies<0>(v);
        wave_lds_fence();
        before_writes();
        F::template pass_write<0, true>(v, xa, t, t);
        wave_lds_fence();
        F::template pass_readback<1>(v, xa, t);
    };
    auto tw1_issue = [&](cf (&tw1)[16]) {
        if constexpr (FAST2) {
            const f4* tl = reinterpret_cast<const f4*>(twlds + (t & 15) * ST_TW_STRIDE);
#pragma unroll
            for (int u = 0; u < 8; ++u) {
                const f4 x = tl[u];
                tw1[2 * u] = mkc(x.x, x.y);
                tw1[2 * u + 1] = mkc(x.z, x.w);
            }
        }
    };
    auto s12 = [&](cf (&v)[E], cf (&zm)[F::NPAIR], cf& zmid, cf (&tw1)[16], bool reload_tw1) {
        if constexpr (FAST2) F::template pass_twiddle<1, true>(v, tw1);
        else F::template pass_twiddle<1>(v, tw);
        F::template pass_butterflies<1>(v);
        F::exchange_1_2_in_registers(v);
        if constexpr (FAST2) F::template pass_twiddle<2, true>(v, tw);
        else F::template pass_twiddle<2>(v, tw);
        F::template pass_butterflies<2>(v);
        wave_lds_fence();
        F::template pass_write<2, true>(v, xa, t, t);
        wave_lds_fence();
        const cf* const pb = xa + lds_pad(NC - t);
#pragma unroll
        for (int p = 0; p < F::NPAIR; ++p) {
            const cf z = pb[-lds_pad_c(p * F::LPF)];
            zm[p] = (p == 0 && t == 0) ? v[F::reg_of_spectrum(0)] : z;
        }
        zmid = xa[lds_pad(NC / 2)];
    };
    auto s3 = [&](cf (&v)[E], cf (&zm)[F::NPAIR], cf zmid, float* prow) {
        wave_lds_fence();
        static_assert(F::NPAIR % 2 == 0, "R2C pairs are processed two at a time");
#pragma unroll
        for (int p = 0; p < F::NPAIR; p += 2) {
            const int kk = t + p * F::LPF, kk2 = kk + F::LPF;
            cf pw, pw2;
            if constexpr (FULLPTW) {
                r2c_power_pair_x2(v[F::reg_of_spectrum(p)], zm[p], ptw[p], v[F::reg_of_spectrum(p + 1)], zm[p + 1], ptw[p + 1], pw, pw2);
            } else {
                pw = F::r2c_power_factored_x2(v[F::reg_of_spectrum(p)], zm[p], w0, p);
                pw2 = F::r2c_power_factored_x2(v[F::reg_of_spectrum(p + 1)], zm[p + 1], w0, p + 1);
            }
            prow[kk] = POW2 ? pw.x : __builtin_amdgcn_sqrtf(pw.x);
            prow[NC - kk] = POW2 ? pw.y : __builtin_amdgcn_sqrtf(pw.y);
            prow[kk2] = POW2 ? pw2.x : __builtin_amdgcn_sqrtf(pw2.x);
            prow[NC - kk2] = POW2 ? pw2.y : __builtin_amdgcn_sqrtf(pw2.y);
        }
        if (t == 0) {
            const float pm = 4.0f * cnorm2(zmid);
            prow[NC / 2] = POW2 ? pm : __builtin_amdgcn_sqrtf(pm);
        }
        wave_lds_fence();
    };
    auto s3_issue = [&](const float* prow, f4 (&cw)[ST_RIDE], f4 (&cp)[ST_RIDE], bool with_weights) {
        const f4* wp = reinterpret_cast<const f4*>(wlds) + lane;
        const f4* p0 = reinterpret_cast<const f4*>(prow + lo_s[0]);
        const f4* p1 = reinterpret_cast<const f4*>(prow + lo_s[1]);
#pragma unroll
        for (int u = 0; u < ST_FAST_STEPS0; ++u) {
            if (with_weights) cw[u] = wp[u * 64];
            cp[u] = p0[u];
        }
#pragma unroll
        for (int u = 0; u < ST_RIDE1; ++u) {
            if (with_weights) cw[ST_FAST_STEPS0 + u] = wp[(ST_FAST_STEPS0 + u) * 64];
            cp[ST_FAST_STEPS0 + u] = p1[u];
        }
    };
    auto fma4 = [](f4 wv, f4 pv, cf& a0, cf& a1) {
        a0 = __builtin_elementwise_fma(mkc(wv.x, wv.y), mkc(pv.x, pv.y), a0);
        a1 = __builtin_elementwise_fma(mkc(wv.z, wv.w), mkc(pv.z, pv.w), a1);
    };
    const bool fast_db = m.amin >= 1.1754944e-38f;
    const float ten_log10_ref = 10.0f * m.log10_ref;
    auto s4_fast = [&](const float* prow, int i, const f4 (&cw)[ST_RIDE], const f4 (&cp)[ST_RIDE], auto&& after_ride) {
        i = i < nloc ? i : nloc - 1;
        constexpr int REST = (FAST2 ? FAST2 : ST_FAST_STEPS1) - ST_RIDE1;
        constexpr int NB = (REST + ST_BATCH - 1) / ST_BATCH;
        const f4* wp = reinterpret_cast<const f4*>(wlds) + lane + ST_RIDE * 64;
        const f4* p1 = reinterpret_cast<const f4*>(prow + lo_s[1]) + ST_RIDE1;
        cf a0 = mkc(0.f, 0.f), a1 = mkc(0.f, 0.f), b0 = mkc(0.f, 0.f), b1 = mkc(0.f, 0.f);
        f4 w2[ST_BATCH], q2[ST_BATCH];
        auto issue_batch = [&](int c0) {
#pragma unroll
            for (int u = 0; u < ST_BATCH; ++u) {
                if (c0 + u < REST) {
                    w2[u] = wp[(c0 + u) * 64];
                    q2[u] = p1[c0 + u];
                }
            }
        };
        if constexpr (NB > 0) issue_batch(0);
        __builtin_amdgcn_sched_barrier(0);
#pragma unroll
        for (int u = 0; u < ST_FAST_STEPS0; ++u) fma4(cw[u], cp[u], a0, a1);
#pragma unroll
        for (int u = 0; u < ST_RIDE1; ++u) fma4(cw[ST_FAST_STEPS0 + u], cp[ST_FAST_STEPS0 + u], b0, b1);
        asm volatile("" : "+v"(a0), "+v"(a1), "+v"(b0), "+v"(b1) : : "memory");
        __builtin_amdgcn_sched_barrier(0);
        after_ride();
        __builtin_amdgcn_sched_barrier(0);
#pragma unroll
        for (int c = 0; c < NB; ++c) {
#pragma unroll
            for (int u = 0; u < ST_BATCH; ++u)
                if (c * ST_BATCH + u < REST) fma4(w2[u], q2[u], b0, b1);
            __builtin_amdgcn_sched_barrier(0);
            if (c + 1 < NB) issue_batch((c + 1) * ST_BATCH);
            __builtin_amdgcn_sched_barrier(0);
        }
        float v0 = (a0.x + a0.y) + (a1.x + a1.y), v1 = (b0.x + b0.y) + (b1.x + b1.y);
        if (m.db) {
            v0 = fast_db ? amp_to_db_fast(v0, m.amin, ten_log10_ref) : amp_to_db(v0, m.amin, m.log10_ref);
            v1 = fast_db ? amp_to_db_fast(v1, m.amin, ten_log10_ref) : amp_to_db(v1, m.amin, m.log10_ref);
        }
        float* orow = m.out + (begin + i) * (long long)m.n_mels + lane;
        orow[0] = v0;
        orow[64] = v1;
    };
// ... 121 lines not shown
```

torchaudio-contrib_amd/csrc/melspec_stream3.hpp:

```cpp
#pragma once
#include <type_traits>

#include "melspec_stream.hpp"

namespace tac {

constexpr int S3_WAVES = 12;
constexpr int S3_TW2L_BYTES = 64 * 12 * 8;

template <class F>
__host__ __device__ constexpr int s3_xa_bytes() {
    return ((F::NC + F::NC / 16 - 1) * (int)sizeof(cf) + 127) & ~127;
}

template <int NC, int E>
__host__ __device__ inline size_t stream3_lds_bytes(int wtot, int waves, bool coded) {
    using C = StreamCfg<NC, E>;
    size_t xa = (size_t)s3_xa_bytes<typename C::F>();
    return (size_t)waves * xa + (((size_t)wtot * 4 + 15) & ~(size_t)15) + ST_TW_BYTES + 16 + 64 * (C::F::NPAIR + E) * sizeof(cf) + (coded ? 1024 : 0);
}

__device__ __forceinline__ unsigned lds_offset_of(const void* p) { return (unsigned)reinterpret_cast<unsigned long long>(p); }
template <int BYTE_OFF>
__device__ __forceinline__ cf lds_read_b64_single(unsigned addr) {
    cf r;
    asm volatile("ds_read_b64 %0, %1 offset:%2" : "=v"(r) : "v"(addr), "n"(BYTE_OFF) : "memory");
    return r;
}
__device__ __forceinline__ void lds_wait_all(cf (&a)[16]) {
    asm volatile("s_waitcnt lgkmcnt(0)"
                 : "+v"(a[0]), "+v"(a[1]), "+v"(a[2]), "+v"(a[3]), "+v"(a[4]), "+v"(a[5]), "+v"(a[6]), "+v"(a[7]), "+v"(a[8]),
                   "+v"(a[9]), "+v"(a[10]), "+v"(a[11]), "+v"(a[12]), "+v"(a[13]), "+v"(a[14]), "+v"(a[15])
                 :: "memory");
}
__device__ __forceinline__ void lds_wait_all8(cf* a) {
    asm volatile("s_waitcnt lgkmcnt(0)"
                 : "+v"(a[0]), "+v"(a[1]), "+v"(a[2]), "+v"(a[3]), "+v"(a[4]), "+v"(a[5]), "+v"(a[6]), "+v"(a[7])
                 :: "memory");
}
__device__ __forceinline__ void lds_wait_all(cf (&a)[8], cf& b) {
    asm volatile("s_waitcnt lgkmcnt(0)"
                 : "+v"(a[0]), "+v"(a[1]), "+v"(a[2]), "+v"(a[3]), "+v"(a[4]), "+v"(a[5]), "+v"(a[6]), "+v"(a[7]), "+v"(b)
                 :: "memory");
}

struct S3Swz {
    unsigned w0;
    unsigned r[4];
    __device__ __forceinline__ void init(const cf* xa, int t) {
        const unsigned base = lds_offset_of(xa);
        w0 = base + 128u * (unsigned)t + 8u * (unsigned)(t & 15);
        const unsigned a = (unsigned)t >> 4, k0 = (unsigned)t & 15u;
#pragma unroll
        for (unsigned j = 0; j < 4; ++j) r[j] = base + 8u * (16u * a + (k0 ^ (a + 4u * j)));
    }
};
__device__ __forceinline__ void s3_write_pass0_swz(const cf (&v)[16], const S3Swz& z) {
#pragma unroll
    for (int k = 0; k < 16; ++k) {
        const unsigned addr = z.w0 ^ (8u * (unsigned)k);
        asm volatile("ds_write_b64 %0, %1" :: "v"(addr), "v"(v[k]) : "memory");
    }
}
__device__ __forceinline__ void s3_readback_pass1_swz(cf (&v)[16], const S3Swz& z) {
    auto rd = [&](auto qc) { constexpr int q = decltype(qc)::value; v[q] = lds_read_b64_single<512 * q>(z.r[q & 3]); };
    rd(std::integral_constant<int, 0>{}); rd(std::integral_constant<int, 1>{}); rd(std::integral_constant<int, 2>{}); rd(std::integral_constant<int, 3>{});
    rd(std::integral_constant<int, 4>{}); rd(std::integral_constant<int, 5>{}); rd(std::integral_constant<int, 6>{}); rd(std::integral_constant<int, 7>{});
    rd(std::integral_constant<int, 8>{}); rd(std::integral_constant<int, 9>{}); rd(std::integral_constant<int, 10>{}); rd(std::integral_constant<int, 11>{});
    rd(std::integral_constant<int, 12>{}); rd(std::integral_constant<int, 13>{}); rd(std::integral_constant<int, 14>{}); rd(std::integral_constant<int, 15>{});
    lds_wait_all(v);
}
template <class F>
__device__ __forceinline__ void s3_r2c_partners_dense(const cf (&v)[16], cf* xa, cf (&zm)[8], cf& zmid, int t) {
    constexpr int NC = F::NC;
    static_assert(NC == 1024 && F::E == 16 && radix_at(NC, 2) == 4, "16 . 16 . 4 plan");
    wave_lds_fence();
#pragma unroll
    for (int b = 0; b < 4; ++b)
#pragma unroll
        for (int k = 2; k < 4; ++k) xa[t + 64 * b + 256 * k] = v[b * 4 + k];
    wave_lds_fence();
    const unsigned pa = lds_offset_of(xa + (NC - t - 7 * 64));
    auto rd = [&](auto pc) { constexpr int p = decltype(pc)::value; zm[p] = lds_read_b64_single<(7 - p) * 64 * 8>(pa); };
    rd(std::integral_constant<int, 0>{}); rd(std::integral_constant<int, 1>{}); rd(std::integral_constant<int, 2>{}); rd(std::integral_constant<int, 3>{});
    rd(std::integral_constant<int, 4>{}); rd(std::integral_constant<int, 5>{}); rd(std::integral_constant<int, 6>{}); rd(std::integral_constant<int, 7>{});
    zmid = lds_read_b64_single<0>(lds_offset_of(xa + NC / 2));
    lds_wait_all(zm, zmid);
    if (t == 0) zm[0] = v[F::reg_of_spectrum(0)];
}

template <class F>
__device__ __forceinline__ void s3_readback_pass1(cf (&v)[16], const cf* xa, int t) {
    const unsigned ra = lds_offset_of(xa + lds_pad(t));
    auto rd = [&](auto qc) { constexpr int q = decltype(qc)::value; v[q] = lds_read_b64_single<lds_pad_c(q * (F::NC / 16)) * 8>(ra); };
    rd(std::integral_constant<int, 0>{}); rd(std::integral_constant<int, 1>{}); rd(std::integral_constant<int, 2>{}); rd(std::integral_constant<int, 3>{});
    rd(std::integral_constant<int, 4>{}); rd(std::integral_constant<int, 5>{}); rd(std::integral_constant<int, 6>{}); rd(std::integral_constant<int, 7>{});
    rd(std::integral_constant<int, 8>{}); rd(std::integral_constant<int, 9>{}); rd(std::integral_constant<int, 10>{}); rd(std::integral_constant<int, 11>{});
    rd(std::integral_constant<int, 12>{}); rd(std::integral_constant<int, 13>{}); rd(std::integral_constant<int, 14>{}); rd(std::integral_constant<int, 15>{});
    lds_wait_all(v);
}
template <class F>
__device__ __forceinline__ void s3_read_partners(const cf (&v)[16], const cf* xa, cf (&zm)[8], cf& zmid, int t) {
    constexpr int NC = F::NC;
    static_assert(F::NPAIR == 8, "eight partners per lane");
    const unsigned pa = lds_offset_of(xa + lds_pad(NC - t) - lds_pad_c(7 * F::LPF));
    auto rd = [&](auto pc) { constexpr int p = decltype(pc)::value; zm[p] = lds_read_b64_single<lds_pad_c((7 - p) * F::LPF) * 8>(pa); };
    rd(std::integral_constant<int, 0>{}); rd(std::integral_constant<int, 1>{}); rd(std::integral_constant<int, 2>{}); rd(std::integral_constant<int, 3>{});
    rd(std::integral_constant<int, 4>{}); rd(std::integral_constant<int, 5>{}); rd(std::integral_constant<int, 6>{}); rd(std::integral_constant<int, 7>{});
    zmid = lds_read_b64_single<0>(lds_offset_of(xa + lds_pad(NC / 2)));
    lds_wait_all(zm, zmid);
    if (t == 0) zm[0] = v[F::reg_of_spectrum(0)];
}
template <class F>
__device__ __forceinline__ void s3_r2c_partners(const cf (&v)[16], cf* xa, cf (&zm)[8], cf& zmid, int t) {
    s3_r2c_partners_dense<F>(v, xa, zm, zmid, t);
}
template <int N0, int CNT>
__device__ __forceinline__ void s3_read_strided(cf* dst, const cf* first) {
    static_assert(CNT == 8 || CNT == 16, "eight or sixteen values");
    const unsigned ra = lds_offset_of(first);
    auto rd = [&](auto qc) { constexpr int q = decltype(qc)::value; if constexpr (q < CNT) dst[q] = lds_read_b64_single<lds_pad_c((N0 + q) * 64) * 8>(ra); };
    rd(std::integral_constant<int, 0>{}); rd(std::integral_constant<int, 1>{}); rd(std::integral_constant<int, 2>{}); rd(std::integral_constant<int, 3>{});
    rd(std::integral_constant<int, 4>{}); rd(std::integral_constant<int, 5>{}); rd(std::integral_constant<int, 6>{}); rd(std::integral_constant<int, 7>{});
    rd(std::integral_constant<int, 8>{}); rd(std::integral_constant<int, 9>{}); rd(std::integral_constant<int, 10>{}); rd(std::integral_constant<int, 11>{});
    rd(std::integral_constant<int, 12>{}); rd(std::integral_constant<int, 13>{}); rd(std::integral_constant<int, 14>{}); rd(std::integral_constant<int, 15>{});
    if constexpr (CNT == 16) lds_wait_all(*reinterpret_cast<cf(*)[16]>(dst));
    else lds_wait_all8(dst);
}

typedef float pf4 __attribute__((ext_vector_type(4)));
template <class F, int THREADS>
struct S3Setup {
    static constexpr int TOT = S3_IMG_TW1_F4 + S3_IMG_PTW_F4;
    static constexpr int NIMG = (TOT + THREADS - 1) / THREADS;
    static constexpr int NWIN = (64 * F::E + THREADS - 1) / THREADS;
    static_assert(F::N == 2048 && F::E == 16 && F::NPAIR == 8 && S3_IMG_TW_STRIDE == ST_TW_STRIDE, "image layout of get_tables()");
    pf4 img[NIMG];
    cf win[NWIN];
    __device__ __forceinline__ void issue(const FrameGeom& g, const Tables& tb, int tid) {
#pragma unroll
        for (int u = 0; u < NIMG; ++u) {
            const int c = tid + u * THREADS;
            img[u] = reinterpret_cast<const pf4*>(tb.s3img)[c < TOT ? c : TOT - 1];
        }
        if (g.win_length == F::N) {
            const cf* w2 = reinterpret_cast<const cf*>(g.window);
#pragma unroll
            for (int u = 0; u < NWIN; ++u) {
                const int idx = tid + u * THREADS;
                win[u] = w2[idx < 64 * F::E ? idx : 0];
            }
        } else {
#pragma unroll
            for (int u = 0; u < NWIN; ++u) {
                const int idx = tid + u * THREADS;
                win[u] = window_pair(g, idx < 64 * F::E ? idx : 0);
            }
        }
    }
    __device__ __forceinline__ void store(float* twlds, cf* ptwl, cf* winl, float half, int tid) const {
#pragma unroll
        for (int u = 0; u < NIMG; ++u) {
            const int c = tid + u * THREADS;
            if (c < S3_IMG_TW1_F4) reinterpret_cast<pf4*>(twlds)[c] = img[u];
            else if (c < TOT) reinterpret_cast<pf4*>(ptwl)[c - S3_IMG_TW1_F4] = img[u];
        }
#pragma unroll
        for (int u = 0; u < NWIN; ++u) {
            const int idx = tid + u * THREADS;
            const int q = idx >> 6, tt = idx & 63;
            if (idx < 64 * F::E) winl[((q >> 1) * 64 + tt) * 2 + (q & 1)] = cscale(win[u], half);
        }
    }
};

template <int NC, int E, bool POW2, int FMT, int FAST1, int WAVES, int PA = 0, int PC = 0>
__global__ void __launch_bounds__(WAVES * 64, (WAVES + 3) / 4)
melspec_stream3_kernel(FrameGeom g, Tables tb, StreamArgs m) {
    using C = StreamCfg<NC, E>;
    using F = typename C::F;
    constexpr int NBINS = C::NBINS;
    constexpr int XA_BYTES = s3_xa_bytes<F>();
    static_assert(XA_BYTES >= (int)(C::PROW * 4), "the power row fits the exchange area");
    extern __shared__ __attribute__((aligned(16))) unsigned char smem_raw[];
    const int tid = threadIdx.x;
    const int lane = tid & 63;
    const int w = __builtin_amdgcn_readfirstlane(tid >> 6);
    cf* const xa = reinterpret_cast<cf*>(smem_raw + (size_t)w * XA_BYTES);
    float* const prow = reinterpret_cast<float*>(xa);
    const long long chunk = m.chunk;
    const long long begin = (long long)blockIdx.x * chunk;
    const long long endl = begin + chunk < m.total ? begin + chunk : m.total;
    const int nloc = endl > begin ? (int)(endl - begin) : 0;
    const unsigned T = (unsigned)g.n_frames;
    const int t = lane;

    const int deal_shift = nloc >> 1;
    auto place = [&](int i) { const int j = i + deal_shift; return j < nloc ? j : j - nloc; };
    cf v[E];
    int mode = 0, row = 0;
    long long fr = 0;
    auto request = [&](int i) {
        i = i < nloc ? i : nloc - 1;
        const unsigned gf = (unsigned)(begin + place(i));
        const unsigned r = gf / T;
        row = (int)r;
        fr = (long long)(gf - r * T);
        const long long start = fr * (long long)g.hop - g.center_pad;
        const bool ok = g.vec2_ok && start >= 0 && start + F::N <= g.length;
        mode = ok ? 1 : 2;
        long long cs = start < 0 ? 0 : start;
        cs = cs + F::N <= g.length ? cs : g.length - F::N;
        const long long off = (long long)row * g.row_stride + cs;
        if constexpr (FMT == FMT_F32) {
            const cf* src = reinterpret_cast<const cf*>(static_cast<const float*>(m.samples) + off);
#pragma unroll
            for (int q = 0; q < E; ++q) v[q] = src[t + q * F::LPF];
        } else if constexpr (FMT == FMT_I16) {
            const unsigned* src = reinterpret_cast<const unsigned*>(static_cast<const short*>(m.samples) + off);
#pragma unroll
            for (int q = 0; q < E; ++q) v[q].x = __uint_as_float(src[t + q * F::LPF]);
        } else if constexpr (FMT == FMT_MULAW_U8) {
            const unsigned short* src = reinterpret_cast<const unsigned short*>(static_cast<const unsigned char*>(m.samples) + off);
#pragma unroll
            for (int q = 0; q < E; ++q) v[q].x = __uint_as_float((unsigned)src[t + q * F::LPF]);
        } else {
            const int* src = reinterpret_cast<const int*>(static_cast<const long long*>(m.samples) + off);
#pragma unroll
            for (int q = 0; q < E; ++q) {
                v[q].x = __int_as_float(src[4 * (t + q * F::LPF)]);
                v[q].y = __int_as_float(src[4 * (t + q * F::LPF) + 2]);
            }
        }
    };
    float* const wlds = reinterpret_cast<float*>(smem_raw + (size_t)WAVES * XA_BYTES);
    float* const twlds = wlds + ((m.wtot + 3) & ~3);
    unsigned* const next_frame = reinterpret_cast<unsigned*>(twlds + ST_TW_BYTES / 4);
    cf* const ptwl = reinterpret_cast<cf*>(next_frame + 4);
    cf* const winl = ptwl + 64 * F::NPAIR;
    const float half = 0.5f * g.scale * (FMT == FMT_I16 ? (1.0f / 32768.0f) : 1.0f);
    constexpr int WCH = 4;
    const int n4 = (m.wtot + 3) >> 2;
    pf4 wreg[WCH];
#pragma unroll
    for (int u = 0; u < WCH; ++u) {
        const int c = tid + u * WAVES * 64;
        wreg[u] = reinterpret_cast<const pf4*>(m.wl)[c < n4 ? c : n4 - 1];
    }
    S3Setup<F, WAVES * 64> setup;
    setup.issue(g, tb, tid);
    cf tw2[3];
    {
        cf all[F::NTW];
        F::load_twiddles(all, tb.w_nc, t);
#pragma unroll
        for (int q = 0; q < 3; ++q) tw2[q] = all[twiddles_before(NC, E, 2) + q];
    }
    int lo_s[ST_MAX_SLOTS];
#pragma unroll
    for (int s = 0; s < ST_MAX_SLOTS; ++s) lo_s[s] = s < m.nslot ? m.lo[s * 64 + lane] : 0;
    float lutv = 0.0f;
    if (FMT >= FMT_MULAW_U8) lutv = m.lut[tid & 255];
    __builtin_amdgcn_sched_barrier(0);
    if (nloc > 0) request(w);
    __builtin_amdgcn_sched_barrier(0);
#pragma unroll
    for (int u = 0; u < WCH; ++u) {
        const int c = tid + u * WAVES * 64;
        if (c < n4) reinterpret_cast<pf4*>(wlds)[c] = wreg[u];
    }
    for (int c = tid + WCH * WAVES * 64; c < n4; c += WAVES * 64)
        reinterpret_cast<pf4*>(wlds)[c] = reinterpret_cast<const pf4*>(m.wl)[c];
    if (tid == 0) *next_frame = WAVES;
    setup.store(twlds, ptwl, winl, half, tid);
    cf ptw_regs[F::NPAIR];
#pragma unroll
    for (int p = 0; p < F::NPAIR; ++p) ptw_regs[p] = tb.w_n[t + p * F::LPF];
    float* const lutlds = reinterpret_cast<float*>(winl + 64 * E);
    constexpr bool TW2L = FAST1 > 0;
    cf* const tw2l = reinterpret_cast<cf*>(lutlds);
    if constexpr (TW2L) {
        for (int i = tid; i < 64 * 12; i += WAVES * 64) {
            const int tt = i & 63, e = i >> 6, b = e / 3, q = e % 3 + 1;
            tw2l[((e >> 1) * 64 + tt) * 2 + (e & 1)] = tb.w_nc[((tt + 64 * b) * q) & 1023];
        }
    }
    if (FMT >= FMT_MULAW_U8 && tid < 256) lutlds[tid] = lutv;
    __syncthreads();
    if (nloc <= 0) return;

    typedef float f4 __attribute__((ext_vector_type(4)));
    const bool fast_db = m.amin >= 1.1754944e-38f;
    const float ten_log10_ref = 10.0f * m.log10_ref;
    auto decode = [&]() {
        if constexpr (FMT == FMT_I16) {
#pragma unroll
            for (int q = 0; q < E; ++q) {
                const int bits = __float_as_int(v[q].x);
                v[q] = mkc((float)(short)(bits & 0xffff), (float)(bits >> 16));
            }
        } else if constexpr (FMT == FMT_MULAW_U8) {
#pragma unroll
            for (int q = 0; q < E; ++q) {
                const unsigned bits = __float_as_uint(v[q].x);
                v[q] = mkc(lutlds[bits & 0xffu], lutlds[(bits >> 8) & 0xffu]);
            }
        } else if constexpr (FMT == FMT_MULAW_I64) {
#pragma unroll
            for (int q = 0; q < E; ++q) v[q] = mkc(lutlds[__float_as_uint(v[q].x) & 0xffu], lutlds[__float_as_uint(v[q].y) & 0xffu]);
        }
    };
    struct Fetch {
        const void* base;
        const float* lut;
        __device__ __forceinline__ float operator()(long long row_offset, int j) const {
            if constexpr (FMT == FMT_F32) return static_cast<const float*>(base)[row_offset + j];
            else if constexpr (FMT == FMT_I16) return (float)static_cast<const short*>(base)[row_offset + j];
            else if constexpr (FMT == FMT_MULAW_U8) return lut[static_cast<const unsigned char*>(base)[row_offset + j]];
            else return lut[(unsigned)static_cast<const long long*>(base)[row_offset + j] & 0xffu];
        }
    };
    auto fma4 = [](f4 wv, f4 pv, cf& a0, cf& a1) {
        a0 = __builtin_elementwise_fma(mkc(wv.x, wv.y), mkc(pv.x, pv.y), a0);
        a1 = __builtin_elementwise_fma(mkc(wv.z, wv.w), mkc(pv.z, pv.w), a1);
    };
    S3Swz swz;
    swz.init(xa, t);
    int i = w;
    unsigned long long probe_c = 0, probe_w = 0;
    if (m.probe && w == 0) {
        probe_c = __builtin_readcyclecounter();
        probe_w = wall_clock64();
    }
    while (i < nloc) {
        unsigned ask = 0;
        if (lane == 0) ask = __hip_atomic_fetch_add(next_frame, 1u, __ATOMIC_RELAXED, __HIP_MEMORY_SCOPE_WORKGROUP);
        if (mode == 1) {
            decode();
        } else {
            int tz;
            asm volatile("v_mov_b32 %0, %1" : "=v"(tz) : "v"(t));
            load_frame<F, false, true, true>(v, g, nullptr, xa, row, fr, tz, Fetch{m.samples, lutlds});
        }
        {
            cf win[E];
            const f4* wl = reinterpret_cast<const f4*>(winl) + t;
#pragma unroll
            for (int u = 0; u < E / 2; ++u) {
                const f4 x = wl[u * 64];
                win[2 * u] = mkc(x.x, x.y);
                win[2 * u + 1] = mkc(x.z, x.w);
            }
            Dft<16>::run_windowed(v, win);
        }
        wave_lds_fence();
        cf tw1[16];
        {
            const f4* tl = reinterpret_cast<const f4*>(twlds + (t & 15) * ST_TW_STRIDE);
#pragma unroll
            for (int u = 0; u < 8; ++u) {
                const f4 x = tl[u];
                tw1[2 * u] = mkc(x.x, x.y);
                tw1[2 * u + 1] = mkc(x.z, x.w);
            }
        }
        s3_write_pass0_swz(v, swz);
        wave_lds_fence();
        s3_readback_pass1_swz(v, swz);
        F::template pass_twiddle<1, true>(v, tw1);
        F::template pass_butterflies<1>(v);
        F::exchange_1_2_in_registers(v);
        if constexpr (TW2L) {
            const f4* tl2 = reinterpret_cast<const f4*>(tw2l) + t;
            cf w2[12];
#pragma unroll
            for (int u = 0; u < 6; ++u) {
                const f4 x = tl2[u * 64];
                w2[2 * u] = mkc(x.x, x.y);
                w2[2 * u + 1] = mkc(x.z, x.w);
            }
#pragma unroll
            for (int b = 0; b < 4; ++b) {
                cmul_x2(v[4 * b + 1], w2[3 * b], v[4 * b + 2], w2[3 * b + 1]);
                v[4 * b + 3] = cmul(v[4 * b + 3], w2[3 * b + 2]);
            }
        } else {
            F::template pass_twiddle<2, true>(v, tw2);
        }
        F::template pass_butterflies<2>(v);
        cf zm[F::NPAIR], zmid;
        s3_r2c_partners<F>(v, xa, zm, zmid, t);
        cf pw[F::NPAIR];
        const cf (&ptw)[F::NPAIR] = ptw_regs;
#pragma unroll
        for (int p = 0; p < F::NPAIR; p += 2)
            r2c_power_pair_x2(v[F::reg_of_spectrum(p)], zm[p], ptw[p], v[F::reg_of_spectrum(p + 1)], zm[p + 1], ptw[p + 1], pw[p], pw[p + 1]);
        const float pmid = 4.0f * cnorm2(zmid);
        wave_lds_fence();
        {
            float lo[F::NPAIR], hi[F::NPAIR];
#pragma unroll
            for (int p = 0; p < F::NPAIR; ++p) {
                lo[p] = POW2 ? pw[p].x : __builtin_amdgcn_sqrtf(pw[p].x);
                hi[p] = POW2 ? pw[p].y : __builtin_amdgcn_sqrtf(pw[p].y);
            }
            const unsigned alo = lds_offset_of(prow + t), ahi = lds_offset_of(prow + (NC - t - 7 * F::LPF));
            asm volatile("ds_write2st64_b32 %8, %0, %1 offset0:0 offset1:1\n\t"
                         "ds_write2st64_b32 %8, %2, %3 offset0:2 offset1:3\n\t"
                         "ds_write2st64_b32 %8, %4, %5 offset0:4 offset1:5\n\t"
                         "ds_write2st64_b32 %8, %6, %7 offset0:6 offset1:7"
                         :: "v"(lo[0]), "v"(lo[1]), "v"(lo[2]), "v"(lo[3]), "v"(lo[4]), "v"(lo[5]), "v"(lo[6]), "v"(lo[7]), "v"(alo)
                         : "memory");
            asm volatile("ds_write2st64_b32 %8, %0, %1 offset0:7 offset1:6\n\t"
                         "ds_write2st64_b32 %8, %2, %3 offset0:5 offset1:4\n\t"
                         "ds_write2st64_b32 %8, %4, %5 offset0:3 offset1:2\n\t"
                         "ds_write2st64_b32 %8, %6, %7 offset0:1 offset1:0"
                         :: "v"(hi[0]), "v"(hi[1]), "v"(hi[2]), "v"(hi[3]), "v"(hi[4]), "v"(hi[5]), "v"(hi[6]), "v"(hi[7]), "v"(ahi)
                         : "memory");
        }
        if (t == 0) prow[NC / 2] = POW2 ? pmid : __builtin_amdgcn_sqrtf(pmid);
        if (t < C::PROW - NBINS) prow[NBINS + t] = 0.0f;
        wave_lds_fence();
        const int cur = i;
        i = (int)__builtin_amdgcn_readfirstlane(ask);
        request(i);
        if constexpr (FAST1 > 0 && PC > 0) {
            constexpr int SA = PA, SB = FAST1 - PC, SC = PC;
            static_assert(SA > 0 && SB > 0 && FMT == FMT_F32, "three segments, float32 samples");
            const int ci = cur < nloc ? cur : nloc - 1;
            const f4* wp = reinterpret_cast<const f4*>(wlds) + lane;
            const f4* p0 = reinterpret_cast<const f4*>(prow + lo_s[0]);
            const f4* p1 = reinterpret_cast<const f4*>(prow + lo_s[1]);
            const f4* p2 = reinterpret_cast<const f4*>(prow + lo_s[2]);
            cf a0 = mkc(0.f, 0.f), a1 = mkc(0.f, 0.f), b0 = mkc(0.f, 0.f), b1 = mkc(0.f, 0.f), c0 = mkc(0.f, 0.f), c1 = mkc(0.f, 0.f);
            f4 wa[SA], qa[SA], wb[SB], qb[SB];
#pragma unroll
            for (int u = 0; u < SA; ++u) {
                wa[u] = wp[u * 64];
                qa[u] = p0[u];
            }
#pragma unroll
            for (int u = 0; u < SB; ++u) {
                wb[u] = wp[(SA + u) * 64];
                qb[u] = p1[u];
            }
#pragma unroll
            for (int u = 0; u < SA; ++u) fma4(wa[u], qa[u], a0, a1);
            f4 wc[SC], qc[SC];
#pragma unroll
            for (int u = 0; u < SC; ++u) {
                wc[u] = wp[(SA + SB + u) * 64];
                qc[u] = p2[u];
            }
#pragma unroll
            for (int u = 0; u < SB; ++u) fma4(wb[u], qb[u], b0, b1);
#pragma unroll
            for (int u = 0; u < SC; ++u) fma4(wc[u], qc[u], c0, c1);
            float v0 = (a0.x + a0.y) + (a1.x + a1.y);
            const float sb = (b0.x + b0.y) + (b1.x + b1.y), sc = (c0.x + c0.y) + (c1.x + c1.y);
            const auto got = __builtin_amdgcn_permlane32_swap(0u, __float_as_uint(sc), false, false);
            float v1 = (sb + (lane >= 32 ? sc : 0.0f)) + __uint_as_float(got[0]);
            if (m.db) {
                v0 = fast_db ? amp_to_db_fast(v0, m.amin, ten_log10_ref) : amp_to_db(v0, m.amin, m.log10_ref);
                v1 = fast_db ? amp_to_db_fast(v1, m.amin, ten_log10_ref) : amp_to_db(v1, m.amin, m.log10_ref);
            }
            float* orow = m.out + (begin + place(ci)) * (long long)m.n_mels + lane;
            orow[0] = v0;
            orow[64] = v1;
        } else if constexpr (FAST1 > 0) {
            const int ci = cur < nloc ? cur : nloc - 1;
            const f4* wp = reinterpret_cast<const f4*>(wlds) + lane;
            const f4* p0 = reinterpret_cast<const f4*>(prow + lo_s[0]);
            const f4* p1 = reinterpret_cast<const f4*>(prow + lo_s[1]);
            cf a0 = mkc(0.f, 0.f), a1 = mkc(0.f, 0.f), b0 = mkc(0.f, 0.f), b1 = mkc(0.f, 0.f);
            constexpr int B1 = (FAST1 + 1) / 2, B2 = FAST1 - B1;
            f4 w0[ST_FAST_STEPS0], q0[ST_FAST_STEPS0], wa[B1], qa[B1];
#pragma unroll
            for (int u = 0; u < ST_FAST_STEPS0; ++u) {
                w0[u] = wp[u * 64];
                q0[u] = p0[u];
            }
#pragma unroll
            for (int u = 0; u < B1; ++u) {
                wa[u] = wp[(ST_FAST_STEPS0 + u) * 64];
                qa[u] = p1[u];
            }
#pragma unroll
            for (int u = 0; u < ST_FAST_STEPS0; ++u) fma4(w0[u], q0[u], a0, a1);
            f4 wb[B2], qb[B2];
#pragma unroll
            for (int u = 0; u < B2; ++u) {
                wb[u] = wp[(ST_FAST_STEPS0 + B1 + u) * 64];
                qb[u] = p1[B1 + u];
            }
#pragma unroll
            for (int u = 0; u < B1; ++u) fma4(wa[u], qa[u], b0, b1);
#pragma unroll
            for (int u = 0; u < B2; ++u) fma4(wb[u], qb[u], b0, b1);
            float v0 = (a0.x + a0.y) + (a1.x + a1.y), v1 = (b0.x + b0.y) + (b1.x + b1.y);
            if (m.db) {
                v0 = fast_db ? amp_to_db_fast(v0, m.amin, ten_log10_ref) : amp_to_db(v0, m.amin, m.log10_ref);
                v1 = fast_db ? amp_to_db_fast(v1, m.amin, ten_log10_ref) : amp_to_db(v1, m.amin, m.log10_ref);
            }
            float* orow = m.out + (begin + place(ci)) * (long long)m.n_mels + lane;
            orow[0] = v0;
            orow[64] = v1;
        } else {
            const int ci = cur < nloc ? cur : nloc - 1;
            const f4* wp = reinterpret_cast<const f4*>(wlds) + lane;
            float* orow = m.out + (begin + place(ci)) * (long long)m.n_mels + (m.rev ? m.n_mels - 1 - lane : lane);
            const int ostep = m.rev ? -64 : 64;
#pragma unroll
            for (int s = 0; s < ST_MAX_SLOTS; ++s) {
                if (s < m.nslot) {
                    const f4* pp = reinterpret_cast<const f4*>(prow + lo_s[s]);
                    const int n = m.steps[s];
                    cf acc0 = mkc(0.f, 0.f), acc1 = mkc(0.f, 0.f);
                    int j = 0;
#pragma unroll 1
                    for (; j + 8 <= n; j += 8, wp += 512) {
                        f4 wv[8], pv[8];
#pragma unroll
                        for (int u = 0; u < 8; ++u) {
                            wv[u] = wp[u * 64];
                            pv[u] = pp[j + u];
                        }
#pragma unroll
                        for (int u = 0; u < 8; ++u) fma4(wv[u], pv[u], acc0, acc1);
                    }
                    if (j + 4 <= n) {
                        f4 wv[4], pv[4];
#pragma unroll
                        for (int u = 0; u < 4; ++u) {
                            wv[u] = wp[u * 64];
                            pv[u] = pp[j + u];
                        }
#pragma unroll
                        for (int u = 0; u < 4; ++u) fma4(wv[u], pv[u], acc0, acc1);
                        wp += 256;
                        j += 4;
                    }
#pragma unroll 1
                    for (; j < n; ++j, wp += 64) fma4(wp[0], pp[j], acc0, acc1);
                    float val = (acc0.x + acc0.y) + (acc1.x + acc1.y);
                    if (m.db) val = fast_db ? amp_to_db_fast(val, m.amin, ten_log10_ref) : amp_to_db(val, m.amin, m.log10_ref);
                    if (s * 64 + lane < m.n_mels) orow[s * ostep] = val;
                }
            }
        }
        wave_lds_fence();
    }
    if (m.probe && w == 0) {
        const unsigned long long dc = __builtin_readcyclecounter() - probe_c, dw = wall_clock64() - probe_w;
        if (lane == 0) {
            m.probe[2 * blockIdx.x] = dc;
            m.probe[2 * blockIdx.x + 1] = dw;
        }
    }
}

}
```

Measured before the change: 709.5 million frames/s.

## Deal mel bands to lanes with a permuted layout to shorten fused mel-reduction steps

Adds a 'dealt' pack mode for the fused 2048/128-mel stream kernel. Mel bands are assigned to lanes through a searched permutation instead of lane==band, which allows a shorter step shape (3,6,4) and placement with fewer LDS bank conflicts. Each lane's band indices and a swap flag are packed into a descriptor word, and the kernel scatters its two outputs to the permuted mel columns. The cost is scattered output stores and more host-side packing search. The dealt pack is used only when it beats the pair pack on steps or modeled read cycles; otherwise the pair pack is kept.

```diff
diff --git a/include/tac_amd.h b/include/tac_amd.h
--- a/include/tac_amd.h
+++ b/include/tac_amd.h
@@ -51,6 +51,7 @@
                     int db, float db_ref, float db_amin, float* out, void* stream);
 
 #define TAC_PACK_PAIRS_2048 (-2048)
+#define TAC_PACK_DEALT_2048 (-2049)
 int tac_melbank_pack(const float* fb, int32_t n_freqs, int32_t n_mels, int32_t n_fft, float* wpack,
                      int32_t wpack_cap, int32_t* desc, int32_t desc_cap, int32_t* info_host, void* stream);
 int tac_melbank_pack_host(const float* fb_host, int32_t n_freqs, int32_t n_mels, int32_t n_fft, float* wpack_host,
diff --git a/torchaudio-contrib_amd/_hip.py b/torchaudio-contrib_amd/_hip.py
--- a/torchaudio-contrib_amd/_hip.py
+++ b/torchaudio-contrib_amd/_hip.py
@@ -480,15 +480,17 @@
     return result
 
 
-PAIR_LAYOUT = True
+PAIR_LAYOUT = 'dealt'
 PACK_PAIRS_2048 = -2048
+PACK_DEALT_2048 = -2049
 
 
 def _fused_pack(fb, n_fft):
     if PAIR_LAYOUT and n_fft == 2048 and tuple(fb.shape) == (1025, 128):
-        pack = _melbank_pack(fb, PACK_PAIRS_2048)
-        if pack is not None:
-            return pack
+        for selector in ((PACK_DEALT_2048, PACK_PAIRS_2048) if PAIR_LAYOUT == 'dealt' else (PACK_PAIRS_2048,)):
+            pack = _melbank_pack(fb, selector)
+            if pack is not None:
+                return pack
     return _melbank_pack(fb, n_fft)
 
 
diff --git a/torchaudio-contrib_amd/csrc/lane_placement.hpp b/torchaudio-contrib_amd/csrc/lane_placement.hpp
--- a/torchaudio-contrib_amd/csrc/lane_placement.hpp
+++ b/torchaudio-contrib_amd/csrc/lane_placement.hpp
@@ -4,6 +4,95 @@
 #include <vector>
 
 namespace tac {
+
+inline int place_group(const std::vector<int> (&cand)[16], int (&choice)[16], int max_cap = 16) {
+    struct Search {
+        const std::vector<int> (&cand)[16];
+        int (&choice)[16];
+        int cap;
+        int load[16][16], n[16];
+        unsigned seen;
+        bool place(int i) {
+            for (int c : cand[i]) {
+                const int r = (c / 4) & 15;
+                if (seen & (1u << r)) continue;
+                seen |= 1u << r;
+                if (n[r] < cap) { load[r][n[r]++] = i; choice[i] = c; return true; }
+                for (int q = 0; q < n[r]; ++q) {
+                    const int other = load[r][q];
+                    if (place(other)) {
+                        int* at = std::find(load[r], load[r] + n[r], other);
+                        std::copy(at + 1, load[r] + n[r], at);
+                        load[r][n[r] - 1] = i;
+                        choice[i] = c;
+                        return true;
+                    }
+                }
+            }
+            return false;
+        }
+    };
+    for (int cap = 1; cap <= max_cap; ++cap) {
+        Search s{cand, choice, cap, {}, {}, 0};
+        bool ok = true;
+        for (int i = 0; i < 16 && ok; ++i) {
+            s.seen = 0;
+            ok = s.place(i);
+        }
+        if (ok) return cap;
+    }
+    return 0;
+}
+
+inline int read_group_lane(int gi, int i) {
+    static const int kGroup[2][16] = {{0, 1, 2, 3, 12, 13, 14, 15, 20, 21, 22, 23, 24, 25, 26, 27},
+                                      {4, 5, 6, 7, 8, 9, 10, 11, 16, 17, 18, 19, 28, 29, 30, 31}};
+    return kGroup[gi & 1][i] + 32 * (gi >> 1);
+}
+
+inline int group_distance(int steps, int limit, const int* lo, const int* len) {
+    unsigned mask[16];
+    int slack[16], top = 0;
+    for (int i = 0; i < 16; ++i) {
+        slack[i] = std::max(0, std::min(steps - (len[i] + 3) / 4, lo[i] / 4));
+        mask[i] = 0;
+        for (int d = 0; d <= slack[i] && d < 16; ++d) mask[i] |= 1u << ((lo[i] / 4 - d) & 15);
+        top = std::max(top, lo[i]);
+    }
+    int owner[16], unseated = 0;
+    std::fill(owner, owner + 16, -1);
+    struct Seat {
+        const unsigned* mask;
+        int* owner;
+        unsigned seen;
+        bool operator()(int i) {
+            for (unsigned todo = mask[i] & ~seen; todo; todo = mask[i] & ~seen) {
+                const int r = __builtin_ctz(todo);
+                seen |= 1u << r;
+                if (owner[r] < 0 || (*this)(owner[r])) { owner[r] = i; return true; }
+            }
+            return false;
+        }
+    } seat{mask, owner, 0};
+    for (int i = 0; i < 16; ++i) {
+        seat.seen = 0;
+        if (!seat(i)) ++unseated;
+    }
+    if (unseated == 0 && top + 4 * steps <= limit) return 0;
+    std::vector<int> cand[16];
+    for (int i = 0; i < 16; ++i)
+        for (int d = 0; d <= slack[i]; ++d) cand[i].push_back(lo[i] - 4 * d);
+    int choice[16], worst = 1, quads[16][16], n[16] = {};
+    place_group(cand, choice);
+    for (int i = 0; i < 16; ++i) {
+        int f = choice[i];
+        if (f + 4 * steps > limit) f = (limit - 4 * steps) & ~3;
+        const int r = (f / 4) & 15;
+        if (std::find(quads[r], quads[r] + n[r], f / 4) == quads[r] + n[r]) quads[r][n[r]++] = f / 4;
+        worst = std::max(worst, n[r]);
+    }
+    return 100 * (worst - 1) + (worst > 1 ? unseated : 0);
+}
 
 inline std::vector<int> place_band_starts(int nslot, const int* steps, const std::vector<int>& lo, const std::vector<int>& len) {
     std::vector<int> start(lo);
@@ -19,38 +108,9 @@
                 const int slack = std::max(0, std::min(steps[s] - (len[m] + 3) / 4, lo[m] / 4));
                 for (int d = 0; d <= slack; ++d) cand[i].push_back(lo[m] - 4 * d);
             }
-            for (int cap = 1; cap <= 16; ++cap) {
-                std::vector<int> load[16];
-                int choice[16];
-                unsigned seen = 0;
-                std::function<bool(int)> place = [&](int i) -> bool {
-                    for (int c : cand[i]) {
-                        const int r = (c / 4) & 15;
-                        if (seen & (1u << r)) continue;
-                        seen |= 1u << r;
-                        if ((int)load[r].size() < cap) { load[r].push_back(i); choice[i] = c; return true; }
-                        for (size_t q = 0; q < load[r].size(); ++q) {
-                            const int other = load[r][q];
-                            if (place(other)) {
-                                load[r].erase(std::find(load[r].begin(), load[r].end(), other));
-                                load[r].push_back(i);
-                                choice[i] = c;
-                                return true;
-                            }
-                        }
-                    }
-                    return false;
-                };
-                bool ok = true;
-                for (int i = 0; i < 16 && ok; ++i) {
-                    seen = 0;
-                    ok = place(i);
-                }
-                if (ok) {
-                    for (int i = 0; i < 16; ++i) start[s * 64 + lanes[i]] = choice[i];
-                    break;
-                }
-            }
+            int choice[16];
+            if (place_group(cand, choice))
+                for (int i = 0; i < 16; ++i) start[s * 64 + lanes[i]] = choice[i];
         }
     return start;
 }
diff --git a/torchaudio-contrib_amd/csrc/melspec_sparse.hip b/torchaudio-contrib_amd/csrc/melspec_sparse.hip
--- a/torchaudio-contrib_amd/csrc/melspec_sparse.hip
+++ b/torchaudio-contrib_amd/csrc/melspec_sparse.hip
@@ -313,9 +313,13 @@
     if (total >= 0x7fffffffLL) return TAC_E_UNSUPPORTED;
     if (g.length < 2 * NC) return TAC_E_UNSUPPORTED;
     if (info_host[2] & ST_PAIR_MARK) {
+        const bool deal = (info_host[2] & ST_DEAL_MARK) != 0;
+        const int desc_rows = deal ? 256 : 192;
         int shape = -1;
-        for (int i = 0; i < ST_PAIR_SHAPES; ++i)
-            if (info_host[4] == ST_PAIR_SHAPE[i][0] && info_host[5] == ST_PAIR_SHAPE[i][1] && info_host[6] == ST_PAIR_SHAPE[i][2]) shape = i;
+        for (int i = 0; i < (deal ? ST_DEAL_SHAPES : ST_PAIR_SHAPES); ++i) {
+            const int* shp = deal ? ST_DEAL_SHAPE[i] : ST_PAIR_SHAPE[i];
+            if (info_host[4] == shp[0] && info_host[5] == shp[1] && info_host[6] == shp[2]) shape = i;
+        }
         const int c1 = info_host[7];
         if (FMT != FMT_F32 || NC != 1024 || shape < 0 || info_host[1] != 3 || sm.n_mels != 128 || info_host[0] != 256 * info_host[3] ||
             (c1 != ST_FAST_STEPS1 && c1 != ST_FAST_STEPS1_SHORT))
@@ -326,7 +330,7 @@
                 const int32_t classic[8] = {256 * (ST_FAST_STEPS0 + c1), 2, 64, ST_FAST_STEPS0 + c1, ST_FAST_STEPS0, c1, 0, 0};
                 SparseArgs cm = sm;
                 cm.wpack = sm.wpack + info_host[0];
-                cm.desc = sm.desc + 192;
+                cm.desc = sm.desc + desc_rows;
                 cm.wtot = classic[0];
                 cm.dstride = classic[1];
                 return launch_stream<NC, E, FMT>(g, tb, cm, classic, power, stream, samples, lut);
@@ -341,11 +345,16 @@
             kp = shape == 0 ? TAC_S3_PAIR(0) : (shape == 1 ? TAC_S3_PAIR(1) : TAC_S3_PAIR(2));
 #undef TAC_S3_PAIR
             static_assert(ST_PAIR_SHAPES == 3, "one instantiation per shape");
+#define TAC_S3_DEAL(I) (pow2 ? melspec_stream3_kernel<NC, E, true, FMT, ST_DEAL_SHAPE[I][1] + ST_DEAL_SHAPE[I][2], S3_WAVES, ST_DEAL_SHAPE[I][0], ST_DEAL_SHAPE[I][2], true> \
+                             : melspec_stream3_kernel<NC, E, false, FMT, ST_DEAL_SHAPE[I][1] + ST_DEAL_SHAPE[I][2], S3_WAVES, ST_DEAL_SHAPE[I][0], ST_DEAL_SHAPE[I][2], true>)
+            if (deal) kp = shape == 0 ? TAC_S3_DEAL(0) : (shape == 1 ? TAC_S3_DEAL(1) : (shape == 2 ? TAC_S3_DEAL(2) : TAC_S3_DEAL(3)));
+#undef TAC_S3_DEAL
+            static_assert(ST_DEAL_SHAPES == 4, "one instantiation per shape");
             const long long bp = persistent_blocks(total, S3_WAVES, device_cu_count());
             m.chunk = (total + bp - 1) / bp;
             m.probe = (g_clock_probe && g_clock_probe_pairs >= bp) ? g_clock_probe : nullptr;
-            set_last_route("melspec_stream3_kernel<%d, %d, %s, %d, %d, %d, %d, %d>", NC, E, pow2 ? "true" : "false", FMT,
-                           info_host[5] + info_host[6], S3_WAVES, info_host[4], info_host[6]);
+            set_last_route("melspec_stream3_kernel<%d, %d, %s, %d, %d, %d, %d, %d%s>", NC, E, pow2 ? "true" : "false", FMT,
+                           info_host[5] + info_host[6], S3_WAVES, info_host[4], info_host[6], deal ? ", true" : "");
             return launch_kernel(kp, bp, S3_WAVES * 64, ldsp, stream, g, tb, m);
         }
     }
@@ -569,92 +578,111 @@
     return TAC_OK;
 }
 
-static int pack_pairs(const std::vector<float>& h, int n_freqs, int n_mels, float* wpack, int wpack_cap, int32_t* desc,
-                      int desc_cap, int32_t* info_host, hipStream_t stream, bool to_host = false) {
-    if (n_mels != 128 || n_freqs != 1025 || desc_cap < 192 + 128) return TAC_E_UNSUPPORTED;
-    const int limit = StreamCfg<1024, 16>::PROW;
-    std::vector<int> blo(n_mels, 0), bq(n_mels, 0), bend(n_mels, 0);
-    for (int m = 0; m < n_mels; ++m) {
-        int l0 = n_freqs, h0 = 0;
-        for (int f = 0; f < n_freqs; ++f)
-            if (h[(size_t)f * n_mels + m] != 0.0f) { l0 = f < l0 ? f : l0; h0 = f + 1; }
-        if (h0 > l0) {
-            blo[m] = l0 & ~3;
-            bend[m] = h0;
-            bq[m] = (h0 - blo[m] + 3) / 4;
-        }
-    }
+struct PairCells {
+    std::vector<int> first = std::vector<int>(192, 0), live_lo = std::vector<int>(192, 0), live_hi = std::vector<int>(192, 0),
+                     band = std::vector<int>(192, 0);
+    int cycles = 0;
+};
+static PairCells pair_cells(const int* steps, const int* b0, const int* b1, const std::vector<int>& blo, const std::vector<int>& bq,
+                            const std::vector<int>& bend, int limit) {
+    const int B = steps[1], C = steps[2];
+    PairCells out;
+    std::vector<int> lo(192, 0), len(192, 0);
+    std::vector<int>&band = out.band, &first = out.first, &live_lo = out.live_lo, &live_hi = out.live_hi;
+    auto must = [&](int c, int m, int q0, int q1) {
+        band[c] = m;
+        lo[c] = blo[m] + 4 * q0;
+        len[c] = q1 > q0 ? std::min(bend[m], blo[m] + 4 * q1) - lo[c] : 0;
+        if (len[c] < 0) len[c] = 0;
+    };
+    auto place = [&](int c0, int c1) {
+        const std::vector<int> st = place_band_starts(3, steps, lo, len);
+        for (int c = c0; c < c1; ++c) {
+            first[c] = st[c];
+            const int n = steps[c / 64];
+            if (first[c] + 4 * n > limit) first[c] = (limit - 4 * n) & ~3;
+        }
+    };
+    auto end_quad = [&](int c) { return (first[c] + 4 * steps[c / 64] - blo[band[c]]) / 4; };
+    for (int l = 0; l < 64; ++l) {
+        must(l, b0[l], 0, bq[b0[l]]);
+        if (l < 32) must(64 + l, b1[l], 0, bq[b1[l]]);
+        else must(64 + l, b1[l], 0, std::max(1, bq[b1[l]] - 2 * C));
+        band[128 + l] = l >= 32 ? b1[l] : b1[l + 32];
+    }
+    place(0, 128);
+    for (int l = 32; l < 64; ++l) {
+        const int e1 = std::min(end_quad(64 + l), bq[b1[l]]);
+        must(128 + l, b1[l], e1, std::max(e1, bq[b1[l]] - C));
+    }
+    place(160, 192);
+    for (int l = 0; l < 32; ++l) {
+        const int m = b1[32 + l], e2 = std::min(std::max(end_quad(64 + 32 + l), end_quad(128 + 32 + l)), bq[m]);
+        must(128 + l, m, e2, bq[m]);
+    }
+    place(128, 160);
+    for (int l = 0; l < 64; ++l) {
+        live_lo[l] = blo[b0[l]];
+        live_hi[l] = bend[b0[l]];
+        live_lo[64 + l] = blo[b1[l]];
+        live_hi[64 + l] = l < 32 ? bend[b1[l]] : std::min(bend[b1[l]], first[64 + l] + 4 * B);
+        if (l >= 32) {
+            const int up = 128 + l, down = 128 + l - 32;
+            live_lo[up] = live_hi[64 + l];
+            live_hi[up] = std::max(live_lo[up], std::min(bend[b1[l]], first[up] + 4 * C));
+            live_lo[down] = live_hi[up];
+            live_hi[down] = std::max(live_lo[down], bend[b1[l]]);
+        }
+    }
+    out.cycles = row_read_cycles(3, steps, first);
+    return out;
+}
+
+struct PairBands {
+    std::vector<int> blo, bq, bend;
+    PairBands(const std::vector<float>& h, int n_freqs, int n_mels) : blo(n_mels, 0), bq(n_mels, 0), bend(n_mels, 0) {
+        for (int m = 0; m < n_mels; ++m) {
+            int l0 = n_freqs, h0 = 0;
+            for (int f = 0; f < n_freqs; ++f)
+                if (h[(size_t)f * n_mels + m] != 0.0f) { l0 = f < l0 ? f : l0; h0 = f + 1; }
+            if (h0 > l0) {
+                blo[m] = l0 & ~3;
+                bend[m] = h0;
+                bq[m] = (h0 - blo[m] + 3) / 4;
+            }
+        }
+    }
+};
+
+static bool pair_search(const PairBands& pb, int limit, int* steps, PairCells* best) {
+    const std::vector<int>&blo = pb.blo, &bq = pb.bq, &bend = pb.bend;
     int need_a = 0, need_b = 0, need_w = 0;
     for (int m = 0; m < 64; ++m) need_a = std::max(need_a, bq[m]);
     for (int m = 64; m < 96; ++m) need_b = std::max(need_b, bq[m]);
     for (int m = 96; m < 128; ++m) need_w = std::max(need_w, bq[m]);
-    int steps[3] = {0, 0, 0}, best_cycles = 0;
-    std::vector<int> best_first, best_lo, best_hi, best_band;
+    int ident0[64], ident1[64];
+    for (int l = 0; l < 64; ++l) { ident0[l] = l; ident1[l] = 64 + l; }
+    bool found = false;
+    steps[0] = steps[1] = steps[2] = 0;
     for (int i = 0; i < ST_PAIR_SHAPES; ++i) {
         const int* shp = ST_PAIR_SHAPE[i];
         if (need_a > shp[0] || need_b > shp[1] || need_w > shp[1] + 2 * shp[2]) continue;
-        if (!best_first.empty() && shp[0] + shp[1] + shp[2] > steps[0] + steps[1] + steps[2]) continue;
-        const int keep[3] = {steps[0], steps[1], steps[2]};
-        steps[0] = shp[0]; steps[1] = shp[1]; steps[2] = shp[2];
-        const int B = steps[1], C = steps[2];
-        std::vector<int> band(192, 0), lo(192, 0), len(192, 0), first(192, 0);
-        std::vector<int> live_lo(192, 0), live_hi(192, 0);
-        auto must = [&](int c, int m, int q0, int q1) {
-            band[c] = m;
-            lo[c] = blo[m] + 4 * q0;
-            len[c] = q1 > q0 ? std::min(bend[m], blo[m] + 4 * q1) - lo[c] : 0;
-            if (len[c] < 0) len[c] = 0;
-        };
-        auto place = [&](int c0, int c1) {
-            const std::vector<int> st = place_band_starts(3, steps, lo, len);
-            for (int c = c0; c < c1; ++c) {
-                first[c] = st[c];
-                const int n = steps[c / 64];
-                if (first[c] + 4 * n > limit) first[c] = (limit - 4 * n) & ~3;
-            }
-        };
-        auto end_quad = [&](int c) { return (first[c] + 4 * steps[c / 64] - blo[band[c]]) / 4; };
-        for (int l = 0; l < 64; ++l) {
-            must(l, l, 0, bq[l]);
-            if (l < 32) must(64 + l, 64 + l, 0, bq[64 + l]);
-            else must(64 + l, 64 + l, 0, std::max(1, bq[64 + l] - 2 * C));
-            band[128 + l] = l >= 32 ? 64 + l : 96 + l;
-        }
-        place(0, 128);
-        for (int l = 32; l < 64; ++l) {
-            const int e1 = std::min(end_quad(64 + l), bq[64 + l]);
-            must(128 + l, 64 + l, e1, std::max(e1, bq[64 + l] - C));
-        }
-        place(160, 192);
-        for (int l = 0; l < 32; ++l) {
-            const int m = 96 + l, e2 = std::min(std::max(end_quad(64 + 32 + l), end_quad(128 + 32 + l)), bq[m]);
-            must(128 + l, m, e2, bq[m]);
-        }
-        place(128, 160);
-        for (int l = 0; l < 64; ++l) {
-            live_lo[l] = blo[l];
-            live_hi[l] = bend[l];
-            live_lo[64 + l] = blo[64 + l];
-            live_hi[64 + l] = l < 32 ? bend[64 + l] : std::min(bend[64 + l], first[64 + l] + 4 * B);
-            if (l >= 32) {
-                const int up = 128 + l, down = 128 + l - 32;
-                live_lo[up] = live_hi[64 + l];
-                live_hi[up] = std::max(live_lo[up], std::min(bend[64 + l], first[up] + 4 * C));
-                live_lo[down] = live_hi[up];
-                live_hi[down] = std::max(live_lo[down], bend[64 + l]);
-            }
-        }
-        const int cycles = row_read_cycles(3, steps, first);
-        if (best_first.empty() || cycles < best_cycles) {
-            best_cycles = cycles; best_first = first; best_lo = live_lo; best_hi = live_hi; best_band = band;
-        } else {
-            steps[0] = keep[0]; steps[1] = keep[1]; steps[2] = keep[2];
-        }
-    }
-    if (best_first.empty()) return TAC_E_UNSUPPORTED;
+        if (found && shp[0] + shp[1] + shp[2] > steps[0] + steps[1] + steps[2]) continue;
+        PairCells pc = pair_cells(shp, ident0, ident1, blo, bq, bend, limit);
+        if (!found || pc.cycles < best->cycles) {
+            steps[0] = shp[0]; steps[1] = shp[1]; steps[2] = shp[2];
+            *best = std::move(pc);
+            found = true;
+        }
+    }
+    return found;
+}
+
+static int pair_emit(const std::vector<float>& h, int n_freqs, int n_mels, const int* steps, const PairCells& pc, const int32_t* extra,
+                     float* wpack, int wpack_cap, int32_t* desc, int desc_cap, int32_t* info_host, hipStream_t stream, bool to_host) {
     const int A = steps[0], B = steps[1], C = steps[2], total_steps = A + B + C;
-    const int wtot = 256 * total_steps;
-    std::vector<int> first = best_first, live_lo = best_lo, live_hi = best_hi, band = best_band, lo;
+    const int wtot = 256 * total_steps, rows = extra ? 256 : 192;
+    const std::vector<int>&first = pc.first, &live_lo = pc.live_lo, &live_hi = pc.live_hi, &band = pc.band;
     std::vector<float> wp((size_t)wtot, 0.0f);
     int base = 0;
     for (int s = 0; s < 3; ++s) {
@@ -670,10 +698,11 @@
         }
         base += steps[s];
     }
-    lo = first;
+    std::vector<int32_t> lo(first.begin(), first.end());
+    if (extra) lo.insert(lo.end(), extra, extra + 64);
     int32_t classic[8] = {0, 0, 0, 0, 0, 0, 0, 0};
-    if (wtot >= wpack_cap) return TAC_E_UNSUPPORTED;
-    const int rc = pack_lanes(h, n_freqs, n_mels, wpack + wtot, wpack_cap - wtot, desc + 192, desc_cap - 192, classic, stream, to_host);
+    if (wtot >= wpack_cap || desc_cap < rows + 128) return TAC_E_UNSUPPORTED;
+    const int rc = pack_lanes(h, n_freqs, n_mels, wpack + wtot, wpack_cap - wtot, desc + rows, desc_cap - rows, classic, stream, to_host);
     if (rc != TAC_OK) return rc;
     if (classic[1] != 2 || classic[2] != 64 || classic[4] != ST_FAST_STEPS0 ||
         (classic[5] != ST_FAST_STEPS1 && classic[5] != ST_FAST_STEPS1_SHORT))
@@ -688,13 +717,175 @@
     }
     info_host[0] = wtot;
     info_host[1] = 3;
-    info_host[2] = 64 + ST_PAIR_MARK;
+    info_host[2] = 64 + ST_PAIR_MARK + (extra ? ST_DEAL_MARK : 0);
     info_host[3] = total_steps;
     info_host[4] = A;
     info_host[5] = B;
     info_host[6] = C;
     info_host[7] = classic[5];
     return TAC_OK;
+}
+
+static int pack_pairs(const std::vector<float>& h, int n_freqs, int n_mels, float* wpack, int wpack_cap, int32_t* desc,
+                      int desc_cap, int32_t* info_host, hipStream_t stream, bool to_host = false) {
+    if (n_mels != 128 || n_freqs != 1025 || desc_cap < 192 + 128) return TAC_E_UNSUPPORTED;
+    const PairBands pb(h, n_freqs, n_mels);
+    int steps[3];
+    PairCells pc;
+    if (!pair_search(pb, StreamCfg<1024, 16>::PROW, steps, &pc)) return TAC_E_UNSUPPORTED;
+    return pair_emit(h, n_freqs, n_mels, steps, pc, nullptr, wpack, wpack_cap, desc, desc_cap, info_host, stream, to_host);
+}
+
+static bool deal_bands(const PairBands& pb, const int* shp, int limit, int* b0, int* b1) {
+    const std::vector<int>&blo = pb.blo, &bq = pb.bq, &bend = pb.bend;
+    const int A = shp[0], B = shp[1], C = shp[2];
+    std::vector<int> out, in;
+    for (int m = 0; m < 64; ++m) if (bq[m] > A) out.push_back(m);
+    for (int m = 64; m < 128 && in.size() < out.size(); ++m) if (bq[m] <= A) in.push_back(m);
+    if (in.size() < out.size()) return false;
+    int partner[128];
+    std::fill(partner, partner + 128, -1);
+    for (size_t i = 0; i < out.size(); ++i) { partner[out[i]] = in[i]; partner[in[i]] = out[i]; }
+    const auto by_start = [&](int x, int y) { return blo[x] != blo[y] ? blo[x] < blo[y] : x < y; };
+    std::vector<int> v0, v1;
+    for (int m = 0; m < 128; ++m) ((m < 64) == (partner[m] < 0) ? v0 : v1).push_back(m);
+    std::sort(v1.begin(), v1.end(), [&](int x, int y) { return bq[x] != bq[y] ? bq[x] > bq[y] : x > y; });
+    std::vector<int> heavy(v1.begin(), v1.begin() + 32), light(v1.begin() + 32, v1.end());
+    for (int m : heavy) if (bq[m] > B + 2 * C) return false;
+    for (int m : light) if (bq[m] > B) return false;
+    std::sort(v0.begin(), v0.end(), by_start);
+    std::sort(light.begin(), light.end(), by_start);
+    std::sort(heavy.begin(), heavy.end(), by_start);
+    int mem0[4][16], mem1[4][16], group1[128];
+    for (int i = 0; i < 64; ++i) mem0[i / 16][i % 16] = v0[i];
+    for (int i = 0; i < 32; ++i) {
+        mem1[i / 16][i % 16] = light[i];
+        mem1[2 + i / 16][i % 16] = heavy[i];
+        group1[light[i]] = i / 16;
+        group1[heavy[i]] = 2 + i / 16;
+    }
+    for (int x : in) {
+        const int want = group1[partner[x]];
+        int g = 0, i = 0, j = -1;
+        for (int gg = 0; gg < 4; ++gg)
+            for (int ii = 0; ii < 16; ++ii) if (mem0[gg][ii] == x) { g = gg; i = ii; }
+        if (g == want) continue;
+        for (int jj = 0; jj < 16; ++jj)
+            if (partner[mem0[want][jj]] < 0 && (j < 0 || by_start(mem0[want][j], mem0[want][jj]))) j = jj;
+        if (j < 0) return false;
+        std::swap(mem0[g][i], mem0[want][j]);
+    }
+    const auto distance = [&](const int* bands, int cls) {
+        int lo[16], len[16];
+        for (int i = 0; i < 16; ++i) {
+            const int m = bands[i], q = cls == 2 ? std::max(1, bq[m] - 2 * C) : bq[m];
+            lo[i] = blo[m];
+            len[i] = std::max(0, std::min(bend[m], blo[m] + 4 * q) - blo[m]);
+        }
+        return group_distance(cls == 0 ? A : B, limit, lo, len);
+    };
+    const auto settle = [&](int (*mem)[16], int g_lo, int g_hi, int cls) {
+        int cost[4] = {0, 0, 0, 0};
+        for (int g = g_lo; g < g_hi; ++g) cost[g] = distance(mem[g], cls);
+        for (int pass = 0, before = -1; pass < 8 && cost[0] + cost[1] + cost[2] + cost[3] != before; ++pass) {
+            before = cost[0] + cost[1] + cost[2] + cost[3];
+            for (int ga = g_lo; ga < g_hi; ++ga)
+                for (int gb = ga + 1; gb < g_hi; ++gb)
+                    for (int i = 0; i < 16; ++i)
+                        for (int j = 0; j < 16 && cost[ga] + cost[gb] > 0; ++j) {
+                            if (partner[mem[ga][i]] >= 0 || partner[mem[gb][j]] >= 0) continue;
+                            std::swap(mem[ga][i], mem[gb][j]);
+                            const int ca = distance(mem[ga], cls), cb = distance(mem[gb], cls);
+                            if (ca + cb < cost[ga] + cost[gb]) {
+                                cost[ga] = ca;
+                                cost[gb] = cb;
+                            } else {
+                                std::swap(mem[ga][i], mem[gb][j]);
+                            }
+                        }
+        }
+    };
+    settle(mem0, 0, 4, 0);
+    settle(mem1, 0, 2, 1);
+    const auto to_lanes = [&]() {
+        for (int g = 0; g < 4; ++g) {
+            std::sort(mem0[g], mem0[g] + 16, by_start);
+            std::sort(mem1[g], mem1[g] + 16, by_start);
+            bool taken[16] = {};
+            for (int i = 0; i < 16; ++i) {
+                b1[read_group_lane(g, i)] = mem1[g][i];
+                if (partner[mem1[g][i]] >= 0) {
+                    b0[read_group_lane(g, i)] = partner[mem1[g][i]];
+                    taken[i] = true;
+                }
+            }
+            int i = 0;
+            for (int k = 0; k < 16; ++k) {
+                if (partner[mem0[g][k]] >= 0) continue;
+                while (taken[i]) ++i;
+                b0[read_group_lane(g, i++)] = mem0[g][k];
+            }
+        }
+    };
+    to_lanes();
+    if (distance(mem1[2], 2) + distance(mem1[3], 2) > 0) {
+        int keep[2][16], k0[64], k1[64];
+        std::copy(&mem1[2][0], &mem1[2][0] + 32, &keep[0][0]);
+        std::copy(b0, b0 + 64, k0);
+        std::copy(b1, b1 + 64, k1);
+        const int before = pair_cells(shp, b0, b1, blo, bq, bend, limit).cycles;
+        settle(mem1, 2, 4, 2);
+        to_lanes();
+        if (pair_cells(shp, b0, b1, blo, bq, bend, limit).cycles >= before) {
+            std::copy(&keep[0][0], &keep[0][0] + 32, &mem1[2][0]);
+            std::copy(k0, k0 + 64, b0);
+            std::copy(k1, k1 + 64, b1);
+        }
+    }
+    return true;
+}
+
+static int pack_dealt(const std::vector<float>& h, int n_freqs, int n_mels, float* wpack, int wpack_cap, int32_t* desc,
+                      int desc_cap, int32_t* info_host, hipStream_t stream, bool to_host = false) {
+    if (n_mels != 128 || n_freqs != 1025 || desc_cap < 256 + 128) return TAC_E_UNSUPPORTED;
+    const int limit = StreamCfg<1024, 16>::PROW;
+    const PairBands pb(h, n_freqs, n_mels);
+    int psteps[3], steps[3] = {0, 0, 0}, lane0[64], lane1[64];
+    PairCells ppc, best;
+    const bool have_pair = pair_search(pb, limit, psteps, &ppc);
+    bool found = false;
+    for (int i = 0; i < ST_DEAL_SHAPES; ++i) {
+        const int* shp = ST_DEAL_SHAPE[i];
+        if (found && shp[0] + shp[1] + shp[2] > steps[0] + steps[1] + steps[2]) continue;
+        int b0[64], b1[64];
+        if (!deal_bands(pb, shp, limit, b0, b1)) continue;
+        PairCells pc = pair_cells(shp, b0, b1, pb.blo, pb.bq, pb.bend, limit);
+        if (!found || pc.cycles < best.cycles) {
+            steps[0] = shp[0]; steps[1] = shp[1]; steps[2] = shp[2];
+            std::copy(b0, b0 + 64, lane0);
+            std::copy(b1, b1 + 64, lane1);
+            best = std::move(pc);
+            found = true;
+        }
+    }
+    if (!found) return TAC_E_UNSUPPORTED;
+    if (have_pair) {
+        const int total = steps[0] + steps[1] + steps[2], ptotal = psteps[0] + psteps[1] + psteps[2];
+        if (total > ptotal || (total == ptotal && best.cycles >= ppc.cycles)) return TAC_E_UNSUPPORTED;
+    }
+    int32_t words[64], holder[128];
+    std::fill(holder, holder + 128, -1);
+    for (int l = 0; l < 64; ++l) {
+        const bool swap = lane0[l] >= 64;
+        const int u0 = swap ? lane1[l] : lane0[l], u1 = swap ? lane0[l] : lane1[l];
+        if (u0 >= 64 || u1 < 64 || holder[u0] >= 0 || holder[u1] >= 0) return TAC_E_UNSUPPORTED;
+        holder[u0] = holder[u1] = l;
+    }
+    for (int l = 0; l < 64; ++l) {
+        const bool swap = lane0[l] >= 64;
+        words[l] = holder[l] | (holder[64 + l] << 8) | (swap ? 1 << 16 : 0) | ((swap ? lane1[l] : lane0[l]) << 18) | (((swap ? lane0[l] : lane1[l]) - 64) << 24);
+    }
+    return pair_emit(h, n_freqs, n_mels, steps, best, words, wpack, wpack_cap, desc, desc_cap, info_host, stream, to_host);
 }
 
 }
@@ -723,10 +914,11 @@
     using namespace tac;
     if (!fb_host || !wpack_host || !desc_host || !info_host || n_freqs <= 0 || n_mels <= 0) return TAC_E_INVALID;
     const bool lanes = n_fft == 256 || n_fft == 400 || n_fft == 512 || n_fft == 1024;
-    if (n_fft == TAC_PACK_PAIRS_2048) {
+    if (n_fft == TAC_PACK_PAIRS_2048 || n_fft == TAC_PACK_DEALT_2048) {
         if (n_freqs != 1025) return TAC_E_UNSUPPORTED;
         const std::vector<float> hp(fb_host, fb_host + (size_t)n_freqs * n_mels);
-        return pack_pairs(hp, n_freqs, n_mels, wpack_host, wpack_cap, desc_host, desc_cap, info_host, nullptr, true);
+        return (n_fft == TAC_PACK_DEALT_2048 ? pack_dealt : pack_pairs)(hp, n_freqs, n_mels, wpack_host, wpack_cap, desc_host, desc_cap,
+                                                                       info_host, nullptr, true);
     }
     if ((n_fft != 2048 && n_fft != 4096 && !lanes) || n_freqs != n_fft / 2 + 1) return TAC_E_UNSUPPORTED;
     const std::vector<float> h(fb_host, fb_host + (size_t)n_freqs * n_mels);
@@ -740,12 +932,13 @@
                      int32_t wpack_cap, int32_t* desc, int32_t desc_cap, int32_t* info_host, void* stream) {
     using namespace tac;
     if (!fb || !wpack || !desc || !info_host || n_freqs <= 0 || n_mels <= 0) return TAC_E_INVALID;
-    if (n_fft == TAC_PACK_PAIRS_2048) {
+    if (n_fft == TAC_PACK_PAIRS_2048 || n_fft == TAC_PACK_DEALT_2048) {
         if (n_freqs != 1025) return TAC_E_UNSUPPORTED;
         std::vector<float> hp((size_t)n_freqs * n_mels);
         TAC_HIP(hipMemcpyAsync(hp.data(), fb, hp.size() * sizeof(float), hipMemcpyDeviceToHost, (hipStream_t)stream));
         TAC_HIP(hipStreamSynchronize((hipStream_t)stream));
-        return pack_pairs(hp, n_freqs, n_mels, wpack, wpack_cap, desc, desc_cap, info_host, (hipStream_t)stream);
+        return (n_fft == TAC_PACK_DEALT_2048 ? pack_dealt : pack_pairs)(hp, n_freqs, n_mels, wpack, wpack_cap, desc, desc_cap, info_host,
+                                                                       (hipStream_t)stream, false);
     }
     if (n_fft < 0) return TAC_E_UNSUPPORTED;
     const int groups = n_fft == 0 ? FBS_WAVES * 4 : sparse_groups_for(n_fft);
@@ -836,7 +1029,7 @@
                                 (hipStream_t)stream);
     }
     const bool lanes_pack = info_host[2] >= LM_MARK;
-    if (!lanes_pack && (info_host[2] & ~(d->n_fft == 2048 ? (ST_REV_MARK | ST_PAIR_MARK) : 0)) != sparse_groups_for(d->n_fft)) return TAC_E_INVALID;
+    if (!lanes_pack && (info_host[2] & ~(d->n_fft == 2048 ? (ST_REV_MARK | ST_PAIR_MARK | ST_DEAL_MARK) : 0)) != sparse_groups_for(d->n_fft)) return TAC_E_INVALID;
     FrameGeom g;
     int64_t T = 0;
     int rc = make_geometry(wave, window, d, &g, &T);
diff --git a/torchaudio-contrib_amd/csrc/melspec_stream.hpp b/torchaudio-contrib_amd/csrc/melspec_stream.hpp
--- a/torchaudio-contrib_amd/csrc/melspec_stream.hpp
+++ b/torchaudio-contrib_amd/csrc/melspec_stream.hpp
@@ -39,6 +39,9 @@
 constexpr int ST_PAIR_MARK = 512;
 constexpr int ST_PAIR_SHAPES = 3;
 constexpr int ST_PAIR_SHAPE[ST_PAIR_SHAPES][3] = {{4, 6, 4}, {4, 7, 3}, {3, 7, 5}};
+constexpr int ST_DEAL_MARK = 128;
+constexpr int ST_DEAL_SHAPES = 4;
+constexpr int ST_DEAL_SHAPE[ST_DEAL_SHAPES][3] = {{3, 6, 4}, {4, 6, 4}, {4, 7, 3}, {3, 7, 5}};
 
 
 template <int NC, int E>
diff --git a/torchaudio-contrib_amd/csrc/melspec_stream3.hpp b/torchaudio-contrib_amd/csrc/melspec_stream3.hpp
--- a/torchaudio-contrib_amd/csrc/melspec_stream3.hpp
+++ b/torchaudio-contrib_amd/csrc/melspec_stream3.hpp
@@ -174,7 +174,7 @@
     }
 };
 
-template <int NC, int E, bool POW2, int FMT, int FAST1, int WAVES, int PA = 0, int PC = 0>
+template <int NC, int E, bool POW2, int FMT, int FAST1, int WAVES, int PA = 0, int PC = 0, bool DEAL = false>
 __global__ void __launch_bounds__(WAVES * 64, (WAVES + 3) / 4)
 melspec_stream3_kernel(FrameGeom g, Tables tb, StreamArgs m) {
     using C = StreamCfg<NC, E>;
@@ -259,6 +259,10 @@
     int lo_s[ST_MAX_SLOTS];
 #pragma unroll
     for (int s = 0; s < ST_MAX_SLOTS; ++s) lo_s[s] = s < m.nslot ? m.lo[s * 64 + lane] : 0;
+    if constexpr (DEAL) {
+        const int word = m.lo[3 * 64 + lane];
+        lo_s[2] |= (((word >> 18) & 63) | (((word >> 24) & 63) << 6) | (((word >> 16) & 1) << 12)) << 16;
+    }
     float lutv = 0.0f;
     if (FMT >= FMT_MULAW_U8) lutv = m.lut[tid & 255];
     __builtin_amdgcn_sched_barrier(0);
@@ -431,7 +435,7 @@
             const f4* wp = reinterpret_cast<const f4*>(wlds) + lane;
             const f4* p0 = reinterpret_cast<const f4*>(prow + lo_s[0]);
             const f4* p1 = reinterpret_cast<const f4*>(prow + lo_s[1]);
-            const f4* p2 = reinterpret_cast<const f4*>(prow + lo_s[2]);
+            const f4* p2 = reinterpret_cast<const f4*>(prow + (DEAL ? (lo_s[2] & 0xffff) : lo_s[2]));
             cf a0 = mkc(0.f, 0.f), a1 = mkc(0.f, 0.f), b0 = mkc(0.f, 0.f), b1 = mkc(0.f, 0.f), c0 = mkc(0.f, 0.f), c1 = mkc(0.f, 0.f);
             f4 wa[SA], qa[SA], wb[SB], qb[SB];
 #pragma unroll
@@ -460,13 +464,25 @@
             const float sb = (b0.x + b0.y) + (b1.x + b1.y), sc = (c0.x + c0.y) + (c1.x + c1.y);
             const auto got = __builtin_amdgcn_permlane32_swap(0u, __float_as_uint(sc), false, false);
             float v1 = (sb + (lane >= 32 ? sc : 0.0f)) + __uint_as_float(got[0]);
+            if constexpr (DEAL) {
+                const bool swap = (lo_s[2] & (0x1000 << 16)) != 0;
+                const float u0 = swap ? v1 : v0, u1 = swap ? v0 : v1;
+                v0 = u0;
+                v1 = u1;
+            }
             if (m.db) {
                 v0 = fast_db ? amp_to_db_fast(v0, m.amin, ten_log10_ref) : amp_to_db(v0, m.amin, m.log10_ref);
                 v1 = fast_db ? amp_to_db_fast(v1, m.amin, ten_log10_ref) : amp_to_db(v1, m.amin, m.log10_ref);
             }
-            float* orow = m.out + (begin + place(ci)) * (long long)m.n_mels + lane;
-            orow[0] = v0;
-            orow[64] = v1;
+            if constexpr (DEAL) {
+                float* orow = m.out + (begin + place(ci)) * (long long)m.n_mels;
+                orow[(lo_s[2] >> 16) & 63] = v0;
+                orow[64 + ((lo_s[2] >> 22) & 63)] = v1;
+            } else {
+                float* orow = m.out + (begin + place(ci)) * (long long)m.n_mels + lane;
+                orow[0] = v0;
+                orow[64] = v1;
+            }
         } else if constexpr (FAST1 > 0) {
             const int ci = cur < nloc ? cur : nloc - 1;
             const f4* wp = reinterpret_cast<const f4*>(wlds) + lane;
```

Result: no change. 714.4 million frames/s, median of 6 (+0.7%).
